# huangnengCSU/longcallR

Measured on AMD Instinct MI355X. Metric: candidate_sites_per_sec, higher is better.
Workload: dtype u8 in, u32 counts, f64 likelihoods, i64 fixed-point phase scores

## Files before the change

### include/lcr.h

```cpp
#ifndef LCR_H
#define LCR_H
#include <stddef.h>
#include <stdint.h>
#ifdef __cplusplus
extern "C" {
#endif

#define LCR_OK 0
#define LCR_E_ARG (-1)
#define LCR_E_CIGAR (-2)
#define LCR_E_DEVICE (-3)
#define LCR_E_STATE (-4)
#define LCR_E_NOMEM (-5)
#define LCR_W_HW_QUEUES 1

#define LCR_PLATFORM_HIFI 0
#define LCR_PLATFORM_ONT 1

#define LCR_MEM_HOST 0
#define LCR_MEM_DEVICE 1

typedef struct lcr_ctx lcr_ctx;


// ... 253 lines not shown
  uint32_t n_reads, n_h1, n_h2;
  uint32_t phase_set, n_phase_sets;
  uint32_t h1_absent, h1_present, h2_absent, h2_present;
} lcr_isoform;
typedef struct { int32_t n_regions, n_isoforms, n_chain, n_rows;
                 const lcr_isoform* iso; const int32_t* iso_region_off; const uint64_t* chain ; const int32_t* row_isoform;
                 const lcr_isoform* dev_iso; const uint64_t* dev_chain; const int32_t* dev_row_isoform; } lcr_isoform_list;
int lcr_isoforms(lcr_ctx*, const lcr_isoform_params*);
int lcr_get_isoforms(lcr_ctx*, lcr_isoform_list* out);
int lcr_isoforms_ms(lcr_ctx*, float* ms);

enum { LCR_ENDS_STRAND_TS = 0, LCR_ENDS_STRAND_READ = 1 };
typedef struct { uint32_t min_count, window, strand_mode, pad_; } lcr_end_params;
typedef struct {
  int32_t region; uint8_t strand, side, kind, pad_;
  int64_t peak0;
  int32_t min0, max0;
  uint32_t n_reads, n_h1, n_h2, n_peak;
  uint32_t phase_set, n_phase_sets;
  uint32_t h1_absent, h1_present, h2_absent, h2_present;
} lcr_end_site;
typedef struct { int32_t n_regions, n_sites, n_rows, n_part; int64_t n_assigned;
                 const lcr_end_site* site; const int32_t* site_region_off; const int32_t* row_site;
                 const lcr_end_site* dev_site; const int32_t* dev_row_site; } lcr_end_list;
int lcr_transcript_ends(lcr_ctx*, const lcr_end_params*);
int lcr_get_transcript_ends(lcr_ctx*, lcr_end_list* out);
int lcr_transcript_ends_ms(lcr_ctx*, float* ms);

typedef struct { int32_t n_genes, n_exons; const int64_t *span_start0, *span_end0; const int32_t* exon_off;
                 const int64_t *exon_start0, *exon_end0; } lcr_gene_annotation;
int lcr_assign_genes(lcr_ctx*, int32_t mem, const lcr_gene_annotation*);
int lcr_get_read_genes(lcr_ctx*, int32_t* n_reads, const int32_t** gene, const uint32_t** overlap, const int32_t** dev_gene);

typedef struct {
  int32_t region;
  uint32_t phase_set, n_phase_sets;
  uint32_t h1, h2;
  uint32_t n_sites;
  uint32_t h1_pat, h1_mat, h2_pat, h2_mat;
  int32_t gene;
  uint32_t pad_;
} lcr_ase_gene;
typedef struct { int32_t n_regions, n_pairs; const lcr_ase_gene* rec; const int32_t* pair_region_off; const lcr_ase_gene* dev_rec; } lcr_ase_gene_list;
int lcr_ase_genes(lcr_ctx*, const lcr_ase_params*, int32_t mem, int32_t n_sites, const int64_t* pos0, const uint8_t* pat, const uint8_t* mat);
int lcr_get_ase_genes(lcr_ctx*, lcr_ase_gene_list* out);

typedef struct {
  int32_t region; uint8_t motif; uint8_t pad_[3];
  int64_t start0;
  int32_t len; uint32_t n_reads;
  uint32_t phase_set, n_phase_sets;
  uint32_t h1_absent, h1_present, h2_absent, h2_present;
  int32_t gene;
  uint32_t pad2_;
} lcr_junction_gene;
typedef struct { int32_t n_regions, n_junctions; const lcr_junction_gene* junc; const int32_t* junc_region_off;
                 const lcr_junction_gene* dev_junc; float kernel_ms; } lcr_junction_gene_list;
int lcr_junctions_genes(lcr_ctx*, const lcr_junction_params*, int32_t mem, const lcr_gene_annotation*);
int lcr_get_junctions_genes(lcr_ctx*, lcr_junction_gene_list* out);

enum { LCR_ASJ_EXONS = 1, LCR_ASJ_DNA_FILTER = 2, LCR_ASJ_COVERAGE = 4 };
typedef struct { uint32_t min_count, min_junctions, flags; float min_phase_score;
                 int32_t n_dna, pad_; const int64_t* dna_pos0; } lcr_asj_params;
typedef struct { int32_t region, gene; int64_t start0; int32_t len; uint32_t n_reads; } lcr_exon_gene;
typedef struct { int32_t n_regions, n_junctions; const lcr_junction_gene* junc; const int32_t* junc_region_off;
                 const lcr_junction_gene* dev_junc;
                 int32_t n_exons, n_genes; const lcr_exon_gene* exon; const int32_t* exon_region_off; const lcr_exon_gene* dev_exon;
                 const int32_t* gene_reads; float kernel_ms; } lcr_asj_gene_list;
int lcr_asj_genes(lcr_ctx*, const lcr_asj_params*, int32_t mem, const lcr_gene_annotation*);
int lcr_get_asj_genes(lcr_ctx*, lcr_asj_gene_list* out);

typedef struct {
  int32_t n_regions, n_rows;
  const uint8_t* region_applied;
  const uint8_t* sampled;
  const uint8_t* dev_sampled;
} lcr_downsample_info;
int lcr_set_downsample(lcr_ctx*, uint32_t depth, uint64_t seed);
int lcr_set_downsample_rows(lcr_ctx*, int32_t mem, int32_t n_rows, const uint8_t* sampled);
int lcr_get_downsample(lcr_ctx*, lcr_downsample_info* out);

int lcr_get_ld_blocks(lcr_ctx*, int32_t region, int32_t* n_blocks, const int32_t** block_off, const int32_t** snp_idx);

int lcr_get_tie_census(lcr_ctx*, uint64_t out[8]);

typedef struct {
  int32_t n_regions;
  const int64_t* start0;
  const int32_t* len;
  const uint32_t* max_cov;
} lcr_region_list;
int lcr_discover_regions(lcr_ctx*, int32_t mem, int32_t n_reads, const int32_t* ref_start, const int32_t* ref_end,
                         int64_t contig_len, lcr_region_list* out);
int lcr_discover_regions_truncated(lcr_ctx*, int32_t mem, int32_t n_reads, const int32_t* ref_start, const int32_t* ref_end,
                                   int64_t contig_len, int32_t truncation, uint32_t truncation_coverage, lcr_region_list* out,
                                   int64_t* n_truncated);

typedef struct lcr_bam lcr_bam;
typedef struct {
  uint8_t min_mapq;
  int32_t min_read_length;
  float divergence;
} lcr_read_filter;
int lcr_bam_open(const char* path, int32_t n_threads, lcr_bam** out);
int lcr_bam_open_keep(const char* path, int32_t n_threads, int64_t keep_bytes, lcr_bam** out);
void lcr_bam_close(lcr_bam*);
const char* lcr_bam_last_error(const lcr_bam*);
int lcr_bam_refs(lcr_bam*, int32_t* n_ref, const char* const** names, const int64_t** lengths);
int lcr_bam_n_records(lcr_bam*, int64_t* n);
int lcr_bam_resident(lcr_bam*, int64_t* now, int64_t* peak);
int lcr_bam_spans(lcr_bam*, int32_t ref_id, const lcr_read_filter*, int32_t* n, const int32_t** ref_start,
                  const int32_t** ref_end);
int lcr_bam_batch(lcr_bam*, int32_t ref_id, const lcr_read_filter*, int32_t n_regions, const int64_t* start0,
                  const int32_t* len, lcr_reads* reads, const int32_t** read_begin, const uint64_t** name_off,
                  const char** names);
int lcr_bam_batch_packed(lcr_bam*, int32_t ref_id, const lcr_read_filter*, int32_t n_regions, const int64_t* start0,
                         const int32_t* len, lcr_reads_packed* reads, const int32_t** read_begin, const uint64_t** name_off,
                         const char** names);

typedef struct lcr_vcf lcr_vcf;
int lcr_vcf_open(const char* path, int32_t n_threads, lcr_vcf** out);
void lcr_vcf_close(lcr_vcf*);
const char* lcr_vcf_last_error(const lcr_vcf*);
int lcr_vcf_contigs(lcr_vcf*, int32_t* n, const char* const** names);
int lcr_vcf_contig(lcr_vcf*, const char* name, int32_t* n, const int64_t** pos0, const uint8_t** genotype, const float** qual);
int lcr_vcf_contig_alleles(lcr_vcf*, const char* name, int32_t* n, const uint8_t** ref, const uint8_t** alt, const uint8_t** phase);
int lcr_vcf_contig_phase_sets(lcr_vcf*, const char* name, int32_t* n, const uint32_t** ps);

int lcr_bam_write_phased(lcr_bam*, const char* out_path, int32_t n_regions, const int32_t* region_ref, const int64_t* start0,
                         const int32_t* len, int64_t n_tagged, const uint64_t* name_off, const char* names, const int32_t* hp,
                         const uint32_t* ps, int32_t level, int32_t n_threads);

int lcr_bam_write_reads(const char* out_path, const char* contig, int64_t contig_len, const lcr_reads* rd, int32_t level, int32_t n_threads);

int lcr_ctx_set_async_phase(lcr_ctx*, int on);

int lcr_ctx_set_lock_dir(lcr_ctx*, const char* dir);

int lcr_debug_set(lcr_ctx*, const char* key, int64_t value);

enum { LCR_K_SPANS = 0 , LCR_K_PILEUP, LCR_K_CAND_FILTER, LCR_K_CAND_HIST, LCR_K_CAND_GT,
       LCR_K_FRAG_COUNT, LCR_K_FRAG_FILL, LCR_K_PHASE,
       LCR_K_BIND ,
       LCR_K_BIND_TABLE ,
       LCR_K_CAND_IMPORT , LCR_K_JUNCTIONS ,
       LCR_K_ASE , LCR_NKERNELS };
enum { LCR_K_GENES = LCR_NKERNELS ,
       LCR_K_ASE_GENES ,
       LCR_NTIMERS };
int lcr_enable_timing(lcr_ctx*, int on);
int lcr_kernel_ms(lcr_ctx*, int kernel, float* ms);
int lcr_pileup_bytes(lcr_ctx*, int64_t* bytes);
int lcr_pileup_stage_bytes(lcr_ctx*, int64_t* bytes);

int lcr_release_cached_memory(void);
int lcr_set_cache_limits(int64_t device_bytes, int64_t host_bytes);

const char* lcr_version(void);

#ifdef __cplusplus
}
#endif
#endif
```

### longcallr_amd/_lib.py

```python
import ctypes as C
import os

from . import _abi

_HERE = os.path.dirname(os.path.abspath(__file__))
SO_PATH = os.environ.get("LCR_LIB") or os.path.join(_HERE, "liblcr.so")

SYMBOLS = [
    "lcr_params_preset", "lcr_ctx_create", "lcr_ctx_destroy", "lcr_last_error", "lcr_ctx_set_stream",
    "lcr_ctx_sync", "lcr_ctx_set_lock_dir", "lcr_ctx_set_async_phase", "lcr_debug_set", "lcr_load_batch", "lcr_load_batch_async", "lcr_bind_batch",
    "lcr_host_alloc", "lcr_host_free", "lcr_host_register", "lcr_host_unregister", "lcr_pileup", "lcr_get_columns", "lcr_candidates",
    "lcr_get_candidates", "lcr_get_candidates_device", "lcr_fragments", "lcr_get_fragmat", "lcr_phase", "lcr_get_phase_result", "lcr_get_read_records_device", "lcr_collect_phase", "lcr_get_ld_blocks", "lcr_get_tie_census",
    "lcr_enable_timing", "lcr_kernel_ms", "lcr_pileup_bytes", "lcr_pileup_stage_bytes", "lcr_discover_regions", "lcr_discover_regions_truncated", "lcr_version", "lcr_release_cached_memory", "lcr_set_cache_limits",
    "lcr_bam_open", "lcr_bam_open_keep", "lcr_bam_close", "lcr_bam_last_error", "lcr_bam_refs", "lcr_bam_n_records", "lcr_bam_resident", "lcr_bam_spans", "lcr_bam_batch", "lcr_bam_write_phased", "lcr_bam_write_reads",
    "lcr_set_downsample", "lcr_set_downsample_rows", "lcr_get_downsample",
    "lcr_junctions", "lcr_get_junctions", "lcr_ase", "lcr_get_ase", "lcr_vcf_contig_alleles",
    "lcr_assign_genes", "lcr_get_read_genes", "lcr_ase_genes", "lcr_get_ase_genes",
    "lcr_junctions_genes", "lcr_get_junctions_genes", "lcr_asj_genes", "lcr_get_asj_genes",
    "lcr_load_batch_packed", "lcr_load_batch_packed_async", "lcr_unpack_bases", "lcr_unpack_ms", "lcr_bam_batch_packed",
    "lcr_set_exon_mask", "lcr_exon_mask_ms", "lcr_import_candidates", "lcr_vcf_open", "lcr_vcf_close", "lcr_vcf_last_error", "lcr_vcf_contigs", "lcr_vcf_contig",
    "lcr_haplotag", "lcr_get_haplotag_sites", "lcr_haplotag_ms", "lcr_vcf_contig_phase_sets",
    "lcr_site_counts", "lcr_get_site_counts", "lcr_site_counts_ms",
    "lcr_hap_coverage", "lcr_get_hap_coverage", "lcr_hap_coverage_ms",
    "lcr_somatic", "lcr_get_somatic", "lcr_somatic_ms",
    "lcr_isoforms", "lcr_get_isoforms", "lcr_isoforms_ms",
    "lcr_transcript_ends", "lcr_get_transcript_ends", "lcr_transcript_ends_ms",
]

_lib = None


class LcrError(RuntimeError):
    pass


def load():
    global _lib
    if _lib is not None:
        return _lib
    if not os.path.exists(SO_PATH):
        raise LcrError("liblcr.so is missing: build it with `python -m longcallr_amd.build` "
                       "(hipcc --offload-arch=gfx950). There is no CPU fallback.")
    try:
        import torch
    except Exception:
        pass
    l = C.CDLL(SO_PATH)
    vp, i32 = C.c_void_p, C.c_int
    l.lcr_version.restype = C.c_char_p
    l.lcr_last_error.restype = C.c_char_p
    l.lcr_last_error.argtypes = [vp]
    l.lcr_params_preset.argtypes = [i32, C.POINTER(_abi.LcrParams)]
    l.lcr_ctx_create.argtypes = [i32, C.POINTER(vp)]
    l.lcr_ctx_destroy.argtypes = [vp]
    l.lcr_ctx_destroy.restype = None
    l.lcr_ctx_set_stream.argtypes = [vp, vp]
    l.lcr_ctx_sync.argtypes = [vp]
    l.lcr_ctx_set_lock_dir.argtypes = [vp, C.c_char_p]
    l.lcr_ctx_set_async_phase.argtypes = [vp, C.c_int32]
    l.lcr_debug_set.argtypes = [vp, C.c_char_p, C.c_int64]
    l.lcr_load_batch.argtypes = [vp, C.POINTER(_abi.LcrReads), C.POINTER(_abi.LcrRegions)]
    l.lcr_load_batch_async.argtypes = [vp, C.POINTER(_abi.LcrReads), C.POINTER(_abi.LcrRegions), C.c_int32]
    l.lcr_bind_batch.argtypes = [vp, C.c_int32]
    l.lcr_load_batch_packed.argtypes = [vp, C.POINTER(_abi.LcrReadsPacked), C.POINTER(_abi.LcrRegions)]
    l.lcr_load_batch_packed_async.argtypes = [vp, C.POINTER(_abi.LcrReadsPacked), C.POINTER(_abi.LcrRegions), C.c_int32]
    l.lcr_unpack_bases.argtypes = [vp, C.c_int32, vp, vp, vp, vp, C.c_int64, vp, C.c_int64]
    l.lcr_unpack_ms.argtypes = [vp, C.POINTER(C.c_float)]
    l.lcr_host_alloc.argtypes = [C.c_size_t, C.POINTER(C.c_void_p)]
    l.lcr_host_free.argtypes = [vp]
    l.lcr_host_free.restype = None
    l.lcr_host_register.argtypes = [vp, C.c_size_t]
    l.lcr_host_unregister.argtypes = [vp]
    for f in ("lcr_pileup", "lcr_candidates", "lcr_fragments", "lcr_phase"):
        getattr(l, f).argtypes = [vp, C.POINTER(_abi.LcrParams)]
    l.lcr_get_columns.argtypes = [vp, C.POINTER(_abi.LcrColumns)]
    l.lcr_get_candidates.argtypes = [vp, C.POINTER(_abi.LcrCandidateList)]
    l.lcr_get_candidates_device.argtypes = [vp, C.POINTER(vp), C.POINTER(i32)]
    l.lcr_get_read_records_device.argtypes = [vp, C.POINTER(vp), C.POINTER(i32)]
    l.lcr_get_fragmat.argtypes = [vp, C.POINTER(_abi.LcrFragmat)]
    l.lcr_get_phase_result.argtypes = [vp, C.POINTER(_abi.LcrPhaseResult)]
    l.lcr_collect_phase.argtypes = [vp, C.POINTER(_abi.LcrPhaseCollected)]
    l.lcr_release_cached_memory.argtypes = []
    l.lcr_set_cache_limits.argtypes = [C.c_int64, C.c_int64]
    l.lcr_get_tie_census.argtypes = [vp, C.POINTER(C.c_uint64)]
    l.lcr_get_ld_blocks.argtypes = [vp, C.c_int32, C.POINTER(C.c_int32), C.POINTER(C.POINTER(C.c_int32)), C.POINTER(C.POINTER(C.c_int32))]
    l.lcr_discover_regions.argtypes = [vp, C.c_int32, C.c_int32, vp, vp, C.c_int64, C.POINTER(_abi.LcrRegionList)]
    l.lcr_discover_regions_truncated.argtypes = [vp, C.c_int32, C.c_int32, vp, vp, C.c_int64, C.c_int32, C.c_uint32, C.POINTER(_abi.LcrRegionList),
                                                 C.POINTER(C.c_int64)]
    l.lcr_enable_timing.argtypes = [vp, i32]
    l.lcr_kernel_ms.argtypes = [vp, i32, C.POINTER(C.c_float)]
    l.lcr_pileup_bytes.argtypes = [vp, C.POINTER(C.c_int64)]
    l.lcr_pileup_stage_bytes.argtypes = [vp, C.POINTER(C.c_int64)]
    flt = C.POINTER(_abi.LcrReadFilter)
    l.lcr_bam_open.argtypes = [C.c_char_p, C.c_int32, C.POINTER(vp)]
    l.lcr_bam_open_keep.argtypes = [C.c_char_p, C.c_int32, C.c_int64, C.POINTER(vp)]
    l.lcr_bam_close.argtypes = [vp]
    l.lcr_bam_close.restype = None
    l.lcr_bam_last_error.argtypes = [vp]
    l.lcr_bam_last_error.restype = C.c_char_p
    l.lcr_bam_refs.argtypes = [vp, C.POINTER(C.c_int32), C.POINTER(C.POINTER(C.c_char_p)), C.POINTER(C.POINTER(C.c_int64))]
    l.lcr_bam_n_records.argtypes = [vp, C.POINTER(C.c_int64)]
    l.lcr_bam_resident.argtypes = [vp, C.POINTER(C.c_int64), C.POINTER(C.c_int64)]
    l.lcr_bam_spans.argtypes = [vp, C.c_int32, flt, C.POINTER(C.c_int32), C.POINTER(C.POINTER(C.c_int32)), C.POINTER(C.POINTER(C.c_int32))]
    l.lcr_bam_batch.argtypes = [vp, C.c_int32, flt, C.c_int32, vp, vp, C.POINTER(_abi.LcrReads), C.POINTER(C.POINTER(C.c_int32)),
                                C.POINTER(C.POINTER(C.c_uint64)), C.POINTER(C.c_char_p)]
    l.lcr_bam_batch_packed.argtypes = [vp, C.c_int32, flt, C.c_int32, vp, vp, C.POINTER(_abi.LcrReadsPacked), C.POINTER(C.POINTER(C.c_int32)),
                                       C.POINTER(C.POINTER(C.c_uint64)), C.POINTER(C.c_char_p)]
    l.lcr_bam_write_phased.argtypes = [vp, C.c_char_p, C.c_int32, vp, vp, vp, C.c_int64, vp, C.c_char_p, vp, vp, C.c_int32, C.c_int32]
    l.lcr_bam_write_reads.argtypes = [C.c_char_p, C.c_char_p, C.c_int64, C.POINTER(_abi.LcrReads), C.c_int32, C.c_int32]
    l.lcr_import_candidates.argtypes = [vp, C.POINTER(_abi.LcrParams), C.c_int32, C.c_int32, vp, vp, vp]
    l.lcr_set_exon_mask.argtypes = [vp, C.c_int32, vp, vp, vp]
    l.lcr_exon_mask_ms.argtypes = [vp, C.POINTER(C.c_float)]
    l.lcr_set_downsample.argtypes = [vp, C.c_uint32, C.c_uint64]
    l.lcr_set_downsample_rows.argtypes = [vp, C.c_int32, C.c_int32, vp]
    l.lcr_get_downsample.argtypes = [vp, C.POINTER(_abi.LcrDownsampleInfo)]
    l.lcr_junctions.argtypes = [vp, C.POINTER(_abi.LcrJunctionParams)]
    l.lcr_get_junctions.argtypes = [vp, C.POINTER(_abi.LcrJunctionList)]
    l.lcr_vcf_open.argtypes = [C.c_char_p, C.c_int32, C.POINTER(vp)]
    l.lcr_vcf_close.argtypes = [vp]
    l.lcr_vcf_close.restype = None
    l.lcr_vcf_last_error.argtypes = [vp]
    l.lcr_vcf_last_error.restype = C.c_char_p
    l.lcr_vcf_contigs.argtypes = [vp, C.POINTER(C.c_int32), C.POINTER(C.POINTER(C.c_char_p))]
    l.lcr_vcf_contig.argtypes = [vp, C.c_char_p, C.POINTER(C.c_int32), C.POINTER(vp), C.POINTER(vp), C.POINTER(vp)]
    l.lcr_ase.argtypes = [vp, C.POINTER(_abi.LcrAseParams), C.c_int32, C.c_int32, vp, vp, vp]
    l.lcr_get_ase.argtypes = [vp, C.POINTER(_abi.LcrAseList)]
    l.lcr_assign_genes.argtypes = [vp, C.c_int32, C.POINTER(_abi.LcrGeneAnnotation)]
    l.lcr_get_read_genes.argtypes = [vp, C.POINTER(C.c_int32), C.POINTER(vp), C.POINTER(vp), C.POINTER(vp)]
    l.lcr_ase_genes.argtypes = [vp, C.POINTER(_abi.LcrAseParams), C.c_int32, C.c_int32, vp, vp, vp]
    l.lcr_get_ase_genes.argtypes = [vp, C.POINTER(_abi.LcrAseGeneList)]
    l.lcr_junctions_genes.argtypes = [vp, C.POINTER(_abi.LcrJunctionParams), C.c_int32, C.POINTER(_abi.LcrGeneAnnotation)]
    l.lcr_get_junctions_genes.argtypes = [vp, C.POINTER(_abi.LcrJunctionGeneList)]
    l.lcr_asj_genes.argtypes = [vp, C.POINTER(_abi.LcrAsjParams), C.c_int32, C.POINTER(_abi.LcrGeneAnnotation)]
    l.lcr_get_asj_genes.argtypes = [vp, C.POINTER(_abi.LcrAsjGeneList)]
    l.lcr_vcf_contig_alleles.argtypes = [vp, C.c_char_p, C.POINTER(C.c_int32), C.POINTER(vp), C.POINTER(vp), C.POINTER(vp)]
    l.lcr_vcf_contig_phase_sets.argtypes = [vp, C.c_char_p, C.POINTER(C.c_int32), C.POINTER(vp)]
    l.lcr_haplotag.argtypes = [vp, C.POINTER(_abi.LcrParams), C.c_int32, C.c_int32, vp, vp, vp, vp]
    l.lcr_get_haplotag_sites.argtypes = [vp, C.POINTER(C.c_int32), C.POINTER(vp), C.POINTER(vp)]
    l.lcr_haplotag_ms.argtypes = [vp, C.POINTER(C.c_float)]
    l.lcr_site_counts.argtypes = [vp, C.POINTER(_abi.LcrSiteCountParams)]
    l.lcr_get_site_counts.argtypes = [vp, C.POINTER(C.c_int32), C.POINTER(vp), C.POINTER(vp)]
    l.lcr_site_counts_ms.argtypes = [vp, C.POINTER(C.c_float)]
    l.lcr_hap_coverage.argtypes = [vp]
    l.lcr_get_hap_coverage.argtypes = [vp, C.POINTER(_abi.LcrHapCovList)]
    l.lcr_hap_coverage_ms.argtypes = [vp, C.POINTER(C.c_float)]
    l.lcr_somatic.argtypes = [vp, C.POINTER(_abi.LcrSomaticParams)]
    l.lcr_get_somatic.argtypes = [vp, C.POINTER(C.c_int32), C.POINTER(vp), C.POINTER(vp)]
    l.lcr_somatic_ms.argtypes = [vp, C.POINTER(C.c_float)]
    l.lcr_isoforms.argtypes = [vp, C.POINTER(_abi.LcrIsoformParams)]
    l.lcr_get_isoforms.argtypes = [vp, C.POINTER(_abi.LcrIsoformList)]
    l.lcr_isoforms_ms.argtypes = [vp, C.POINTER(C.c_float)]
    l.lcr_transcript_ends.argtypes = [vp, C.POINTER(_abi.LcrEndParams)]
    l.lcr_get_transcript_ends.argtypes = [vp, C.POINTER(_abi.LcrEndList)]
    l.lcr_transcript_ends_ms.argtypes = [vp, C.POINTER(C.c_float)]
    _lib = l
    return l
```

### longcallr_amd/api.py

```python
import ctypes as C

import numpy as np

from . import _abi, _lib
from ._lib import LcrError


def _view(ptr, dtype, n):
    if n == 0 or not ptr:
        return np.zeros(0, dtype=dtype)
    buf = (C.c_char * (np.dtype(dtype).itemsize * n)).from_address(ptr)
    return np.frombuffer(buf, dtype=dtype, count=n).copy()


def _view_nocopy(ptr, dtype, n):
    if n == 0 or not ptr:
        return np.zeros(0, dtype=dtype)
    buf = (C.c_char * (np.dtype(dtype).itemsize * n)).from_address(ptr)
    return np.frombuffer(buf, dtype=dtype, count=n)


_DEBUG_ENV = {"LCR_PHASE_PROF": "phase_prof", "LCR_GRID_MIN_ENTRIES": "grid_min_entries",
              "LCR_GRID_GENERIC": "grid_generic", "LCR_GRID_SPEC_LANES": "grid_spec_lanes", "LCR_GRID_SPEC_BATCH": "grid_spec_batch", "LCR_POST_HALF": "post_half", "LCR_ENUM_FORCE_BIG": "enum_force_big",
              "LCR_ENUM_FORCE_STREAM": "enum_force_stream", "LCR_ENUM_ELIDE": "enum_elide", "LCR_HIST_TILES": "hist_tiles", "LCR_TIE_ARITH": "tie_arith", "LCR_CHAIN_TIES": "chain_ties", "LCR_K3_HITS": "k3_hits", "LCR_K3_LIST_BLOCKS": "k3_list_blocks", "LCR_FUSE_FILTER": "fuse_filter", "LCR_ASYNC_PHASE": "async_phase", "LCR_HOST_TRACE": "host_trace", "LCR_OWN_FILL": "own_fill", "LCR_REDO_LDS": "redo_lds", "LCR_SPEC_COMPACT": "spec_compact", "LCR_LEAN_PLANES": "lean_planes"}


class Engine:
    def __init__(self, device=0, params=None, timing=False):
        self.lib = _lib.load()
        h = C.c_void_p()
        rc = self.lib.lcr_ctx_create(device, C.byref(h))
        if rc != 0:
            raise LcrError("lcr_ctx_create(device=%d) failed with %d: no usable HIP device; "
                           "liblcr has no CPU fallback" % (device, rc))
        self.h = h
        self.device = device
        self.params = params if params is not None else _abi.make_params()
        self._sites = None
        self._keep = None
        self._n_regions = None
        self._mask_keep = None
        self.last_truncated_columns = 0
        if timing:
            self.lib.lcr_enable_timing(self.h, 1)
            if timing is not True:
                self.debug_set("timing_mask", sum(1 << int(k) for k in timing))
        import os
        for env, key in _DEBUG_ENV.items():
            v = os.environ.get(env)
            if v is not None:
                self.debug_set(key, int(v) if v.lstrip("-").isdigit() else 1)
        if os.environ.get("LCR_LOCK_DIR"):
            self._chk(self.lib.lcr_ctx_set_lock_dir(self.h, os.fsencode(os.environ["LCR_LOCK_DIR"])), "lcr_ctx_set_lock_dir")

    def debug_set(self, key, value):
        self._chk(self.lib.lcr_debug_set(self.h, key.encode(), int(value)), "lcr_debug_set")
        return self

    def close(self):
        if getattr(self, "h", None):
            self.lib.lcr_ctx_destroy(self.h)
            self.h = None

    __del__ = close

    def _chk(self, rc, what):
        if rc != 0:
            raise LcrError("%s failed (%d): %s" % (what, rc, self.lib.lcr_last_error(self.h).decode()))

    def set_stream(self, hip_stream_ptr):
        self._chk(self.lib.lcr_ctx_set_stream(self.h, C.c_void_p(hip_stream_ptr)), "lcr_ctx_set_stream")

    def sync(self):
        self._chk(self.lib.lcr_ctx_sync(self.h), "lcr_ctx_sync")
        self._sites = None
        self._mask_keep = None

    def set_async_phase(self, on=True):
        rc = self.lib.lcr_ctx_set_async_phase(self.h, 1 if on else 0)
        self.async_warning = self.lib.lcr_last_error(self.h).decode() if rc > 0 else None
        if rc < 0:
            self._chk(rc, "lcr_ctx_set_async_phase")
        return self

    def load_batch(self, batch):
        if isinstance(batch, (_abi.ReadBatch, _abi.PackedReadBatch)):
            reads, regions = batch.c_reads(), batch.c_regions()
            self._keep = (batch, reads, regions)
        else:
            reads, regions, keep = batch
            self._keep = (keep, reads, regions)
        if isinstance(reads, _abi.LcrReadsPacked):
            self._chk(self.lib.lcr_load_batch_packed(self.h, C.byref(reads), C.byref(regions)), "lcr_load_batch_packed")
        else:
            self._chk(self.lib.lcr_load_batch(self.h, C.byref(reads), C.byref(regions)), "lcr_load_batch")
        self._n_regions = int(regions.n_regions)
        return self

    def load_batch_async(self, batch, slot):
        reads, regions = batch.c_reads(), batch.c_regions()
        if not hasattr(self, "_keep_slot"):
            self._keep_slot = {}
        if isinstance(reads, _abi.LcrReadsPacked):
            self._chk(self.lib.lcr_load_batch_packed_async(self.h, C.byref(reads), C.byref(regions), int(slot)), "lcr_load_batch_packed_async")
        else:
            self._chk(self.lib.lcr_load_batch_async(self.h, C.byref(reads), C.byref(regions), int(slot)), "lcr_load_batch_async")
        self._keep_slot[int(slot)] = (batch, reads, regions)
        return self

    def unpack_bases(self, seq_len, seq_off, pack_off, seq4, bases_out):
        import torch
        want = (("seq_len", seq_len, (torch.int32,)), ("seq_off", seq_off, (torch.int64, torch.uint64)), ("pack_off", pack_off, (torch.int64, torch.uint64)),
                ("seq4", seq4, (torch.uint8,)), ("bases_out", bases_out, (torch.uint8,)))
        for name, t, dts in want:
            if not getattr(t, "is_cuda", False) or t.dtype not in dts or t.device.index != self.device or t.dim() != 1 or not t.is_contiguous():
                raise ValueError("unpack_bases: %s must be a contiguous 1-d %s tensor on device %d" % (name, dts[0], self.device))
        if not (seq_len.numel() == seq_off.numel() == pack_off.numel()):
            raise ValueError("seq_len, seq_off and pack_off must have the same length")
        torch.cuda.current_stream(self.device).synchronize()
        ptr = lambda t: C.c_void_p(t.data_ptr()) if t.numel() else None
        self._chk(self.lib.lcr_unpack_bases(self.h, int(seq_len.numel()), ptr(seq_len), ptr(seq_off), ptr(pack_off), ptr(seq4), int(seq4.numel()),
                                            ptr(bases_out), int(bases_out.numel())), "lcr_unpack_bases")
        return self

    def unpack_ms(self):
        ms = C.c_float()
        self._chk(self.lib.lcr_unpack_ms(self.h, C.byref(ms)), "lcr_unpack_ms")
        return float(ms.value)

    def bind_batch(self, slot):
        self._chk(self.lib.lcr_bind_batch(self.h, int(slot)), "lcr_bind_batch")
        self._n_regions = int(self._keep_slot[int(slot)][2].n_regions)
        return self

    def discover_regions(self, ref_start, ref_end, contig_len, truncation=False, truncation_coverage=200000):
        if not 0 <= int(truncation_coverage) < 1 << 32:
            raise ValueError("truncation_coverage must be in [0, 2^32), got %r" % (truncation_coverage,))
        rs = np.ascontiguousarray(ref_start, dtype=np.int32)
        re_ = np.ascontiguousarray(ref_end, dtype=np.int32)
        o = _abi.LcrRegionList()
        nt = C.c_int64(0)
        self._chk(self.lib.lcr_discover_regions_truncated(self.h, _abi.LCR_MEM_HOST, int(rs.size), rs.ctypes.data, re_.ctypes.data,
                                                          int(contig_len), 1 if truncation else 0, int(truncation_coverage), C.byref(o),
                                                          C.byref(nt)), "lcr_discover_regions_truncated")
        self.last_truncated_columns = int(nt.value)
        return list(zip(_view(o.start0, np.int64, o.n_regions).tolist(), _view(o.len, np.int32, o.n_regions).tolist(),
                        _view(o.max_cov, np.uint32, o.n_regions).tolist()))

    def fill_data_into_freq_vec(self):
        self._chk(self.lib.lcr_pileup(self.h, C.byref(self.params)), "lcr_pileup")
        return self

    def get_candidate_snps(self):
        self._chk(self.lib.lcr_candidates(self.h, C.byref(self.params)), "lcr_candidates")
        return self

    def import_external_candidates(self, pos0, genotype, qual):
        if any(getattr(t, "is_cuda", False) for t in (pos0, genotype, qual)):
            import torch
            ts = (pos0, genotype, qual)
            want = (torch.int64, torch.uint8, torch.float32)
            if not all(getattr(t, "is_cuda", False) for t in ts):
                raise ValueError("device sites: pos0, genotype and qual must all be device tensors")
            for name, t, dt in zip(("pos0", "genotype", "qual"), ts, want):
                if t.dtype != dt:
                    raise ValueError("device sites: %s must be %s, got %s" % (name, dt, t.dtype))
                if t.device.index != self.device:
                    raise ValueError("device sites: %s is on %s, the engine on device %d" % (name, t.device, self.device))
                if t.dim() != 1 or not t.is_contiguous():
                    raise ValueError("device sites: %s must be a contiguous 1-d tensor" % name)
            if len({t.numel() for t in ts}) != 1:
                raise ValueError("pos0, genotype and qual must have the same length")
            self._release_sites()
            torch.cuda.current_stream(self.device).synchronize()
            self._chk(self.lib.lcr_import_candidates(self.h, C.byref(self.params), _abi.LCR_MEM_DEVICE, int(pos0.numel()),
                                                     *[C.c_void_p(t.data_ptr()) for t in ts]), "lcr_import_candidates")
            self._sites = ts
# ... 217 lines not shown
            pat = np.ascontiguousarray(sites[1], dtype=np.uint8)
            mat = np.ascontiguousarray(sites[2], dtype=np.uint8)
            if not (pos.size == pat.size == mat.size):
                raise ValueError("pos0, pat and mat must have the same length")
            rc = fn(self.h, C.byref(p), _abi.LCR_MEM_HOST, int(pos.size), pos.ctypes.data, pat.ctypes.data, mat.ctypes.data)
        self._chk(rc, what)

    def assign_genes(self, genes):
        a, keep = self._annotation(genes)
        self._chk(self.lib.lcr_assign_genes(self.h, _abi.LCR_MEM_HOST, C.byref(a)), "lcr_assign_genes")
        return self

    @staticmethod
    def _annotation(genes):
        a = _abi.LcrGeneAnnotation()
        keep = []
        if genes is not None and len(genes.span_start0):
            for f, dt in (("span_start0", np.int64), ("span_end0", np.int64), ("exon_off", np.int32), ("exon_start0", np.int64), ("exon_end0", np.int64)):
                keep.append(np.ascontiguousarray(getattr(genes, f), dtype=dt))
                setattr(a, f, keep[-1].ctypes.data)
            a.n_genes, a.n_exons = int(keep[0].size), int(keep[3].size)
            if keep[1].size != a.n_genes or keep[2].size != a.n_genes + 1 or keep[4].size != a.n_exons:
                raise ValueError("annotation arrays: span_end0 needs n_genes, exon_off n_genes + 1, exon_end0 n_exons entries")
        return a, keep

    def read_genes(self):
        n, g, ov, dg = C.c_int32(), C.c_void_p(), C.c_void_p(), C.c_void_p()
        self._chk(self.lib.lcr_get_read_genes(self.h, C.byref(n), C.byref(g), C.byref(ov), C.byref(dg)), "lcr_get_read_genes")
        return _view(g.value, np.int32, n.value), _view(ov.value, np.uint32, n.value)

    def ase_genes(self, sites=None, min_baseq=13, min_phase_score=None):
        self._ase_call(self.lib.lcr_ase_genes, "lcr_ase_genes", sites, min_baseq, min_phase_score)
        o = _abi.LcrAseGeneList()
        self._chk(self.lib.lcr_get_ase_genes(self.h, C.byref(o)), "lcr_get_ase_genes")
        return _view(o.rec, _abi.AGENE_DTYPE, o.n_pairs), _view(o.pair_region_off, np.int32, o.n_regions + 1)

    def junctions_genes(self, genes, min_count=10, min_junctions=2):
        p = _abi.LcrJunctionParams(int(min_count), int(min_junctions))
        a, keep = self._annotation(genes)
        self._chk(self.lib.lcr_junctions_genes(self.h, C.byref(p), _abi.LCR_MEM_HOST, C.byref(a)), "lcr_junctions_genes")
        o = _abi.LcrJunctionGeneList()
        self._chk(self.lib.lcr_get_junctions_genes(self.h, C.byref(o)), "lcr_get_junctions_genes")
        self.last_junctions_genes_ms = float(o.kernel_ms)
        return _view(o.junc, _abi.JUNC_GENE_DTYPE, o.n_junctions), _view(o.junc_region_off, np.int32, o.n_regions + 1)

    def asj_genes(self, genes, min_count=10, min_junctions=2, exons=False, dna_pos0=None, coverage=False, min_phase_score=None):
        flags = (_abi.LCR_ASJ_EXONS if exons else 0) | (_abi.LCR_ASJ_DNA_FILTER if dna_pos0 is not None else 0) | (_abi.LCR_ASJ_COVERAGE if coverage else 0)
        p = _abi.LcrAsjParams(int(min_count), int(min_junctions), flags, float(self.params.min_phase_score if min_phase_score is None else min_phase_score))
        dna = None
        if dna_pos0 is not None:
            dna = np.ascontiguousarray(dna_pos0, dtype=np.int64)
            p.n_dna, p.dna_pos0 = int(dna.size), (dna.ctypes.data if dna.size else None)
        a, keep = self._annotation(genes)
        self._chk(self.lib.lcr_asj_genes(self.h, C.byref(p), _abi.LCR_MEM_HOST, C.byref(a)), "lcr_asj_genes")
        o = _abi.LcrAsjGeneList()
        self._chk(self.lib.lcr_get_asj_genes(self.h, C.byref(o)), "lcr_get_asj_genes")
        return {"junc": _view(o.junc, _abi.JUNC_GENE_DTYPE, o.n_junctions), "junc_region_off": _view(o.junc_region_off, np.int32, o.n_regions + 1),
                "exon": _view(o.exon, _abi.EXON_GENE_DTYPE, o.n_exons), "exon_region_off": _view(o.exon_region_off, np.int32, o.n_regions + 1),
                "gene_reads": _view(o.gene_reads, np.int32, o.n_genes) if o.gene_reads else None, "kernel_ms": float(o.kernel_ms)}

    def set_downsample(self, depth, seed=2025):
        self._chk(self.lib.lcr_set_downsample(self.h, int(depth), int(seed)), "lcr_set_downsample")
        return self

    def set_downsample_rows(self, sampled):
        m = np.ascontiguousarray(sampled, dtype=np.uint8)
        self._chk(self.lib.lcr_set_downsample_rows(self.h, _abi.LCR_MEM_HOST, int(m.size), m.ctypes.data), "lcr_set_downsample_rows")
        return self

    def downsample_info(self):
        o = _abi.LcrDownsampleInfo()
        self._chk(self.lib.lcr_get_downsample(self.h, C.byref(o)), "lcr_get_downsample")
        return dict(applied=_view(o.region_applied, np.uint8, o.n_regions),
                    sampled=_view(o.sampled, np.uint8, o.n_rows) if o.sampled else None, dev_sampled=int(o.dev_sampled or 0))

    def run_all(self):
        return self.fill_data_into_freq_vec().get_candidate_snps().get_fragments().phase()

    def columns(self):
        o = _abi.LcrColumns()
        self._chk(self.lib.lcr_get_columns(self.h, C.byref(o)), "lcr_get_columns")
        return _view(o.planes, np.uint32, _abi.NPLANES * o.n_cols).reshape(_abi.NPLANES, o.n_cols)

    def candidates(self):
        o = _abi.LcrCandidateList()
        self._chk(self.lib.lcr_get_candidates(self.h, C.byref(o)), "lcr_get_candidates")
        self._sites = None
        return (_view(o.cand, _abi.CAND_DTYPE, o.n_cand), _view(o.region_off, np.int32, o.n_regions + 1))

    def candidates_device(self):
        ptr, n = C.c_void_p(), C.c_int32()
        self._chk(self.lib.lcr_get_candidates_device(self.h, C.byref(ptr), C.byref(n)), "lcr_get_candidates_device")
        return int(ptr.value or 0), int(n.value)

    def read_records_device(self):
        ptr, n = C.c_void_p(), C.c_int32()
        self._chk(self.lib.lcr_get_read_records_device(self.h, C.byref(ptr), C.byref(n)), "lcr_get_read_records_device")
        return int(ptr.value or 0), int(n.value)

    def fragmat(self):
        o = _abi.LcrFragmat()
        self._chk(self.lib.lcr_get_fragmat(self.h, C.byref(o)), "lcr_get_fragmat")
        return dict(
            row_region_off=_view(o.row_region_off, np.int32, o.n_regions + 1),
            row_ptr=_view(o.row_ptr, np.int64, o.n_rows + 1), row_read=_view(o.row_read, np.int32, o.n_rows),
            col=_view(o.col, np.int32, o.nnz), val=_view(o.val, np.uint8, o.nnz),
            row_for_phasing=_view(o.row_for_phasing, np.uint8, o.n_rows),
            row_links=_view(o.row_links, np.uint32, o.n_rows))

    def phase_result(self):
        o = _abi.LcrPhaseResult()
        self._chk(self.lib.lcr_get_phase_result(self.h, C.byref(o)), "lcr_get_phase_result")
        return dict(haplotag=_view(o.haplotag, np.int8, o.n_rows), assignment=_view(o.assignment, np.uint8, o.n_rows),
                    phase_set=_view(o.phase_set, np.uint32, o.n_rows),
                    objective=_view(o.objective, np.float64, o.n_regions))

    def collect_phase(self, copy=False):
        o = _abi.LcrPhaseCollected()
        self._chk(self.lib.lcr_collect_phase(self.h, C.byref(o)), "lcr_collect_phase")
        v = _view if copy else _view_nocopy
        return dict(cand=v(o.cand, _abi.CAND_DTYPE, o.n_cand), cand_region_off=v(o.cand_region_off, np.int32, o.n_regions + 1),
                    row_region_off=v(o.row_region_off, np.int32, o.n_regions + 1),
                    haplotag=v(o.haplotag, np.int8, o.n_rows), assignment=v(o.assignment, np.uint8, o.n_rows),
                    phase_set=v(o.phase_set, np.uint32, o.n_rows), objective=v(o.objective, np.float64, o.n_regions),
                    dev_cand=(int(o.dev_cand or 0), int(o.n_cand)), dev_read_rec=(int(o.dev_read_rec or 0), int(o.n_rows)))

    def ld_blocks(self, region):
        n, off, idx = C.c_int32(), C.POINTER(C.c_int32)(), C.POINTER(C.c_int32)()
        self._chk(self.lib.lcr_get_ld_blocks(self.h, int(region), C.byref(n), C.byref(off), C.byref(idx)), "lcr_get_ld_blocks")
        return [[idx[k] for k in range(off[b], off[b + 1])] for b in range(n.value)]

    TIE_FIELDS = ("sigma_f64", "sigma_flips", "delta_unresolved", "step_unresolved", "best_f64", "best_unresolved", "sigma_unresolved", "delta_step_f64")

    def tie_census(self):
        out = (C.c_uint64 * 8)()
        self._chk(self.lib.lcr_get_tie_census(self.h, out), "lcr_get_tie_census")
        return dict(zip(self.TIE_FIELDS, [int(x) for x in out]))

    def kernel_ms(self, k):
        ms = C.c_float()
        self._chk(self.lib.lcr_kernel_ms(self.h, k, C.byref(ms)), "lcr_kernel_ms")
        return float(ms.value)

    def pileup_bytes(self):
        b = C.c_int64()
        self._chk(self.lib.lcr_pileup_bytes(self.h, C.byref(b)), "lcr_pileup_bytes")
        return int(b.value)

    def pileup_stage_bytes(self):
        b = C.c_int64()
        self._chk(self.lib.lcr_pileup_stage_bytes(self.h, C.byref(b)), "lcr_pileup_stage_bytes")
        return int(b.value)


def host_register(*arrays):
    lib = _lib.load()
    done = []
    for a in arrays:
        if a is None or a.nbytes == 0:
            continue
        if lib.lcr_host_register(C.c_void_p(a.ctypes.data), a.nbytes) != 0:
            host_unregister(done)
            raise LcrError("lcr_host_register failed")
        done.append(a)
    return done


def host_unregister(arrays):
    lib = _lib.load()
    for a in arrays:
        lib.lcr_host_unregister(C.c_void_p(a.ctypes.data))
```

### longcallr_amd/csrc/k0_ops.hip

```cpp
#include <algorithm>
#include <climits>

#include "lcr_dev.h"

#ifndef K0_THREADS
#define K0_THREADS 256
#endif
#ifndef K0_OPT
#define K0_OPT 4
#endif
#ifndef K0_ABL
#define K0_ABL 0
#endif
#define K0_NW (K0_THREADS / 64)
#define K0_WIN K0_THREADS
#define K0_ACC 64
#ifndef K0_HCAP
#define K0_HCAP 160
#endif


__device__ __forceinline__ int wave_incl_max(int v) {
  v = max(v, __builtin_amdgcn_update_dpp(0, v, 0x111, 0xf, 0xf, false));
  v = max(v, __builtin_amdgcn_update_dpp(0, v, 0x112, 0xf, 0xf, false));
  v = max(v, __builtin_amdgcn_update_dpp(0, v, 0x114, 0xf, 0xf, false));
  v = max(v, __builtin_amdgcn_update_dpp(0, v, 0x118, 0xf, 0xf, false));
  v = max(v, __builtin_amdgcn_update_dpp(0, v, 0x142, 0xa, 0xf, false));
  v = max(v, __builtin_amdgcn_update_dpp(0, v, 0x143, 0xc, 0xf, false));
  return v;
}


__global__ void __launch_bounds__(LCR_BLOCK) k0_cig_check(const uint64_t* __restrict__ cig_off, const uint32_t* __restrict__ n_cig,
                                                           int32_t nr, int64_t n_cigar, int32_t* out) {
  const int r = blockIdx.x * blockDim.x + threadIdx.x;
  if (r + 1 < nr && cig_off[r + 1] != cig_off[r] + n_cig[r]) out[1] = 1;
  if (r < nr && (cig_off[r] > (uint64_t)n_cigar || (uint64_t)n_cig[r] > (uint64_t)n_cigar - cig_off[r])) out[2] = 1;
  if (r == 0) {
    uint64_t* g = reinterpret_cast<uint64_t*>(out + 4);
    g[0] = cig_off[0]; g[1] = cig_off[nr - 1] + n_cig[nr - 1];
  }
}
void launch_k0_cig_check(const uint64_t* cig_off, const uint32_t* n_cig, int32_t nr, int64_t n_cigar, int32_t* out, hipStream_t s) {
  if (nr > 0) hipLaunchKernelGGL(k0_cig_check, dim3((nr + LCR_BLOCK - 1) / LCR_BLOCK), dim3(LCR_BLOCK), 0, s, cig_off, n_cig, nr, n_cigar, out);
}
__global__ void __launch_bounds__(LCR_BLOCK) k0_cig_compact(const uint32_t* __restrict__ cigar, const uint64_t* __restrict__ cig_off,
                                                             const uint32_t* __restrict__ n_cig, const int32_t* __restrict__ new_off,
                                                             int32_t nr, uint32_t* __restrict__ out, uint64_t* __restrict__ out_off) {
  const int r = (int)((blockIdx.x * blockDim.x + threadIdx.x) >> 6), lane = threadIdx.x & 63;
  if (r >= nr) return;
  const uint32_t* src = cigar + cig_off[r];
  uint32_t* dst = out + new_off[r];
  for (uint32_t i = lane; i < n_cig[r]; i += 64) dst[i] = src[i];
  if (lane == 0) out_off[r] = (uint64_t)new_off[r];
}
void launch_k0_cig_compact(const uint32_t* cigar, const uint64_t* cig_off, const uint32_t* n_cig, const int32_t* new_off, int32_t nr,
                           uint32_t* out, uint64_t* out_off, hipStream_t s) {
  if (nr > 0) hipLaunchKernelGGL(k0_cig_compact, dim3((unsigned)(((int64_t)nr * 64 + LCR_BLOCK - 1) / LCR_BLOCK)), dim3(LCR_BLOCK), 0, s,
                                 cigar, cig_off, n_cig, new_off, nr, out, out_off);
}

__global__ void __launch_bounds__(LCR_BLOCK) k0_block_reads(const ReadBin* __restrict__ rbin, int32_t nr, uint64_t cig0, int32_t opb,
                                                             int32_t n_blocks, int32_t* __restrict__ blk_first_read) {
  const int r = blockIdx.x * blockDim.x + threadIdx.x;
  if (r >= nr) return;
  if (r == 0) blk_first_read[n_blocks] = nr - 1;
  const uint64_t cb = rbin[r].cig_off - cig0, ce = cb + (uint32_t)rbin[r].n_cig;
  for (uint64_t k = (cb + opb - 1) / opb; k * opb < ce; k++) blk_first_read[k] = r;
}
void launch_k0_block_reads(const ReadBin* rbin, int32_t nr, uint64_t cig0, int32_t opb, int32_t n_blocks, int32_t* blk_first_read, hipStream_t s) {
  if (nr > 0) hipLaunchKernelGGL(k0_block_reads, dim3((nr + LCR_BLOCK - 1) / LCR_BLOCK), dim3(LCR_BLOCK), 0, s, rbin, nr, cig0, opb, n_blocks, blk_first_read);
}

struct K0Hdr {
  int32_t refbase;
  int32_t qbase;
  int32_t qlo, qhi;
  int32_t vec, ftile;
  int32_t cend;
  uint32_t hi;
  uint64_t seq_off;
  int32_t reb, rel_pos;
};

__device__ __forceinline__ void wave_lds_sync() {
  __builtin_amdgcn_fence(__ATOMIC_RELEASE, "wavefront");
  __builtin_amdgcn_wave_barrier();
  __builtin_amdgcn_fence(__ATOMIC_ACQUIRE, "wavefront");
}

template <int OPT>
__global__ void __launch_bounds__(K0_THREADS)
k0_ops(BatchView b, const ReadBin* __restrict__ rbin, const int32_t* __restrict__ blk_first_read, uint64_t cig0, uint32_t n_ops,
       int ont, int D, int32_t n_tiles, int32_t* __restrict__ tile_fill, int32_t* __restrict__ tile_nchunks, int32_t* __restrict__ tile_ndiff,
       K0Ctl* __restrict__ ctl, unsigned int* __restrict__ acct, unsigned int pool_sub, unsigned long long* __restrict__ recs,
       unsigned int desc_sub, uint32_t* __restrict__ desc_tile, uint2* __restrict__ desc_val, int2* __restrict__ read_scan) {
  constexpr int OPB = OPT * K0_THREADS, WOPS = OPT * 64;
  __shared__ __attribute__((aligned(8))) uint16_t ridh[OPB];
  __shared__ K0Hdr hdr[K0_HCAP];
  __shared__ int ws_ref[K0_NW], ws_q[K0_NW], ws_rid[K0_NW];
  __shared__ int cnt[K0_WIN], cur[K0_WIN];
  __shared__ unsigned int s_base[3];
  __shared__ int runbase[OPB];
  __shared__ int s_carry[2], s_acc[2];

  const int tid = threadIdx.x, lane = tid & 63, wv = tid >> 6;
  const uint32_t j0 = blockIdx.x * (uint32_t)OPB;
  if (j0 >= n_ops) return;
  const uint32_t jend = min(j0 + (uint32_t)OPB, n_ops);
  const bool last_block = jend == n_ops;
  const uint32_t* __restrict__ cg = b.cigar + cig0;

  uint32_t w[OPT];
  {
    const uint32_t j = j0 + OPT * tid;
    if (OPT == 4 && j + 4 <= jend) {
      const uint4 v = *reinterpret_cast<const uint4*>(cg + j);
      w[0] = v.x; w[1] = v.y; w[2] = v.z; w[3] = v.w;
    } else {
#pragma unroll
      for (int k = 0; k < OPT; k++) w[k] = j + k < jend ? cg[j + k] : 0x4u;
    }
  }
  const int r_lo = blk_first_read[blockIdx.x];
  const int n_blk_reads = blk_first_read[blockIdx.x + 1] - r_lo + 1;
#pragma unroll
  for (int k = 0; k < OPT; k++) ridh[k * K0_THREADS + tid] = 0;
  cnt[tid] = 0;
  if (tid == 0) { s_acc[0] = 0; s_acc[1] = 0; }
  __syncthreads();

  auto load_hdr = [&](int r, uint64_t* cb_out, int* ncig_out) {
    const ReadBin h = rbin[r];
    K0Hdr x;
    x.refbase = h.rel_pos; x.qbase = h.lead > 0 ? h.lead : 0;
    x.qlo = ont ? h.lead + D : -(1 << 30); x.qhi = ont ? h.reb - D + 1 : (1 << 30);
    x.vec = h.vec; x.ftile = h.ftile; x.seq_off = h.seq_off; x.reb = h.reb; x.rel_pos = h.rel_pos;
    const int strand = h.flags & 1, ts = (h.flags >> 1) & 3;
    const uint32_t tscls = ts == 0 ? 0u : ((strand == 0) == (ts == 1) ? 1u : 2u);
    x.hi = ((uint32_t)strand << 28) | (tscls << 29);
    const uint64_t cb = h.cig_off - cig0;
    x.cend = (int32_t)min<int64_t>((int64_t)cb + h.n_cig - (int64_t)j0, INT_MAX);
    *cb_out = cb; *ncig_out = h.n_cig;
    return x;
  };
  auto settle_empty = [&](int r, const K0Hdr& x) {
    b.read_rend[r] = x.rel_pos;
    if (x.qbase != x.reb) atomicExch(&ctl->error, 2);
  };
  for (int rr = tid; rr < n_blk_reads; rr += K0_THREADS) {
    uint64_t cb; int ncig;
    const K0Hdr x = load_hdr(r_lo + rr, &cb, &ncig);
    if (rr == 0 || cb < (uint64_t)jend || (cb == (uint64_t)jend && (last_block || ncig == 0))) {
      if (rr < K0_HCAP) hdr[rr] = x;
      if (rr > 0) { if (ncig > 0) ridh[cb - j0] = (uint16_t)rr; else settle_empty(r_lo + rr, x); }
    }
  }
  if (blockIdx.x == 0)
    for (int r = tid; r < r_lo; r += K0_THREADS) { uint64_t cb; int ncig; const K0Hdr x = load_hdr(r, &cb, &ncig); settle_empty(r, x); }
  if (wv == 0) {
    const uint64_t cb0 = rbin[r_lo].cig_off - cig0;
    int cr = 0, cq = 0;
    for (uint64_t j = cb0 + lane; j < (uint64_t)j0; j += 64) {
      const uint32_t x = cg[j];
      const int op = x & 15, len = (int)(x >> 4);
      const bool m = op == 0 || op == 7 || op == 8;
      cr += (m || op == 2 || op == 3) ? len : 0;
      cq += (m || op == 1) ? len : 0;
    }
    cr = wave_incl_scan(cr); cq = wave_incl_scan(cq);
    if (lane == 63) { s_carry[0] = cr; s_carry[1] = cq; }
  }
  __syncthreads();

  if (K0_ABL == 1) return;
  int dr[OPT], dq[OPT], xr[OPT], xq[OPT], rid[OPT], mark[OPT];
  {
    bool bad_op = false;
    int tr = 0, tq = 0, tm = 0;
    const uint2 mk = *reinterpret_cast<const uint2*>(&ridh[OPT * tid]);
#pragma unroll
    for (int k = 0; k < OPT; k++) {
      const int op = w[k] & 15, len = (int)(w[k] >> 4);
      const bool m = op == 0 || op == 7 || op == 8;
      if (!(m || (op >= 1 && op <= 5))) bad_op = true;
      dr[k] = (m || op == 2 || op == 3) ? len : 0;
      dq[k] = (m || op == 1) ? len : 0;
      mark[k] = OPT == 4 ? (int)(((k < 2 ? mk.x : mk.y) >> (16 * (k & 1))) & 0xffffu) : (int)ridh[OPT * tid + k];
      xr[k] = tr; xq[k] = tq;
      tr += dr[k]; tq += dq[k];
      tm = max(tm, mark[k]); rid[k] = tm;
    }
    if (bad_op) atomicExch(&ctl->error, 1);
    const int ir = wave_incl_scan(tr), iq = wave_incl_scan(tq), im = wave_incl_max(tm);
    if (lane == 63) { ws_ref[wv] = ir; ws_q[wv] = iq; ws_rid[wv] = im; }
    __syncthreads();
    int br = ir - tr, bq = iq - tq, bm = __shfl_up(im, 1, 64);
    if (lane == 0) bm = 0;
    for (int i = 0; i < wv; i++) { br += ws_ref[i]; bq += ws_q[i]; bm = max(bm, ws_rid[i]); }
#pragma unroll
    for (int k = 0; k < OPT; k++) {
      xr[k] += br; xq[k] += bq; rid[k] = max(rid[k], bm);
      if (mark[k] != 0) {
        if (mark[k] < K0_HCAP) { hdr[mark[k]].refbase -= xr[k]; hdr[mark[k]].qbase -= xq[k]; }
        else read_scan[r_lo + mark[k]] = make_int2(xr[k], xq[k]);
      }
    }
    if (tid == 0) { hdr[0].refbase += s_carry[0]; hdr[0].qbase += s_carry[1]; }
  }
  __syncthreads();

  if (K0_ABL == 2) { if (xr[0] + xq[1] + rid[2] == 0x7fffffff) ctl->error = 9; return; }
  int a[OPT], e[OPT], tb[OPT], kind[OPT];
  unsigned int rlo[OPT], rhi[OPT];
  unsigned int my_items = 0;
  const int win0 = hdr[0].ftile + (int)((unsigned int)max(hdr[0].rel_pos - 1, 0) / (unsigned int)LCR_TILE);
#pragma unroll
  for (int k = 0; k < OPT; k++) {
    const int p = OPT * tid + k;
    const bool act = j0 + p < jend;
    K0Hdr H;
    if (rid[k] < K0_HCAP) H = hdr[rid[k]];
    else {
      uint64_t cb; int ncig;
      H = load_hdr(r_lo + rid[k], &cb, &ncig);
      const int2 sb = read_scan[r_lo + rid[k]];
      H.refbase -= sb.x; H.qbase -= sb.y;
    }
    const int op = w[k] & 15, len = (int)(w[k] >> 4);
    const int rs = H.refbase + xr[k];
    const int qs = H.qbase + xq[k];
    const bool m = act && (op == 0 || op == 7 || op == 8), d = act && op == 2, ins = act && op == 1, isn = act && op == 3;
    int aa = max(rs, 0), ee = min(rs + len, H.vec);
    if (m) { aa = max(aa, rs + (H.qlo - qs)); ee = min(ee, rs + (H.qhi - qs)); }
    int kd = ((m || d || isn) && len > 0 && ee > aa) ? (m ? 1 : d ? 2 : 4) : 0;
    if (ins && len > 0 && rs >= 1 && rs < H.vec) { kd = 3; aa = rs - 1; ee = rs; }
    kind[k] = kd; a[k] = aa; e[k] = ee; tb[k] = H.ftile;
    if (kd == 1) {
      const unsigned long long o0 = H.seq_off + (unsigned long long)(long long)(qs - rs);
      rlo[k] = (unsigned int)o0; rhi[k] = ((unsigned int)(o0 >> 32) & 0xffu) | H.hi;
    } else {
      rlo[k] = kd == 2 ? (unsigned int)REC_KIND_D : kd == 3 ? (unsigned int)REC_KIND_I : (unsigned int)REC_KIND_N;
      rhi[k] = 0xffu;
    }
    if (kd) my_items++;
    if (act && p == H.cend - 1) {
      b.read_rend[r_lo + rid[k]] = rs + dr[k];
      if (qs + dq[k] != H.reb) atomicExch(&ctl->error, 2);
    }
    if (kd == 4) {
      const int ta = H.ftile + (int)((unsigned int)aa / (unsigned int)LCR_TILE), te = H.ftile + (int)((unsigned int)(ee - 1) / (unsigned int)LCR_TILE);
      if (te > ta + 1) { atomicAdd(&tile_ndiff[ta + 1], 1); atomicAdd(&tile_ndiff[te], -1); }
    }
  }

  if (K0_ABL == 3) { int x = 0; for (int k = 0; k < OPT; k++) x += a[k] + e[k] + tb[k] + kind[k] + (int)rlo[k] + (int)rhi[k]; if (x == 0x7fffffff) ctl->error = 9; return; }
  auto make_rec = [&](int k, int t) -> unsigned long long {
    const int c0 = (t - tb[k]) * LCR_TILE;
    const int c_lo = max(a[k], c0), c_hi = min(e[k], c0 + LCR_TILE);
    unsigned int lo = rlo[k], hi = rhi[k] | ((unsigned int)(c_lo - c0) << 8) | ((unsigned int)(c_hi - c_lo - 1) << 18);
    if (kind[k] == 1) {
      const unsigned int s = lo + (unsigned int)c_lo;
      hi = (hi & ~0xffu) | (((hi & 0xffu) + (s < lo ? 1u : 0u)) & 0xffu);
      lo = s;
    }
    return ((unsigned long long)hi << 32) | lo;
  };
  auto first_tile = [&](int k) { return tb[k] + (int)((unsigned int)a[k] / (unsigned int)LCR_TILE); };
  auto last_tile = [&](int k) { return tb[k] + (int)((unsigned int)(e[k] - 1) / (unsigned int)LCR_TILE); };
  auto next_tile = [&](int k, int t, int te) { return kind[k] == 4 ? te : t + 1; };

  int key[OPT], rank[OPT], hpos[OPT];
  bool is_last[OPT];
  {
#pragma unroll
    for (int k = 0; k < OPT; k++) {
      const int tp = kind[k] ? first_tile(k) - win0 : -1;
      key[k] = (tp >= 0 && tp < K0_WIN) ? tp : -1;
    }
    int pk = __shfl_up(key[OPT - 1], 1, 64);
    if (lane == 0) pk = -2;
    bool head[OPT];
    int hp = 0;
#pragma unroll
    for (int k = 0; k < OPT; k++) {
      head[k] = key[k] != (k == 0 ? pk : key[k - 1]);
      if (head[k]) hp = OPT * lane + k + 1;
      hpos[k] = hp;
    }
    const int ih = wave_incl_max(hp);
    int bh = __shfl_up(ih, 1, 64);
    if (lane == 0) bh = 0;
    const int nh = __shfl_down(head[0] ? 1 : 0, 1, 64);
#pragma unroll
    for (int k = 0; k < OPT; k++) {
      hpos[k] = max(hpos[k], bh) - 1;
      rank[k] = OPT * lane + k - hpos[k];
      is_last[k] = k + 1 < OPT ? head[k + 1] : (lane == 63 || nh != 0);
      if (is_last[k] && key[k] >= 0) atomicAdd(&cnt[key[k]], rank[k] + 1);
      if (kind[k]) {
        const int te = last_tile(k);
        for (int t = first_tile(k); t < te;) {
          t = next_tile(k, t, te);
          const int wi = t - win0;
          if (wi >= 0 && wi < K0_WIN) atomicAdd(&cnt[wi], 1);
        }
      }
    }
  }
  __syncthreads();

  if (K0_ABL == 4) { int x = 0; for (int k = 0; k < OPT; k++) x += rank[k] + hpos[k] + (is_last[k] ? 1 : 0); if (x == 0x7fffffff) ctl->error = 9; return; }
  unsigned int my_recs = 0;
  const unsigned int shard = blockIdx.x % K0_ACC;
  {
    static_assert(K0_WIN == K0_THREADS, "one window counter per thread");
    const int c = cnt[tid];
    const int c16 = (c + 15) & ~15;
    const int ic = wave_incl_scan(c16);
    const unsigned long long nzb = __ballot(c > 0);
    if (lane == 63) ws_ref[wv] = ic;
    if (lane == 0) ws_q[wv] = __popcll(nzb);
    __syncthreads();
    int before = 0, dbefore = 0, total = 0, dtotal = 0;
    for (int i = 0; i < K0_NW; i++) { if (i < wv) { before += ws_ref[i]; dbefore += ws_q[i]; } total += ws_ref[i]; dtotal += ws_q[i]; }
    if (tid == 0 && total > 0) {
      unsigned int* sh = acct + 32 * shard;
      const unsigned int at = atomicAdd(&sh[2], (unsigned int)total);
      const unsigned int dt = atomicAdd(&sh[3], (unsigned int)dtotal);
      const bool fits = at + (unsigned int)total <= pool_sub && dt + (unsigned int)dtotal <= desc_sub;
      if (!fits) atomicExch(&ctl->error, 3);
      s_base[0] = shard * pool_sub + at; s_base[1] = shard * desc_sub + dt; s_base[2] = fits ? 1u : 0u;
    }
    cur[tid] = before + ic - c16;
    my_recs += (unsigned int)c;
    __syncthreads();
    if (c > 0 && s_base[2]) {
      const int tile = win0 + tid;
      const unsigned int di = s_base[1] + (unsigned int)dbefore + (unsigned int)__popcll(nzb & ((1ull << lane) - 1ull));
      desc_tile[di] = (uint32_t)tile; desc_val[di] = make_uint2(s_base[0] + (unsigned int)(before + ic - c16), (unsigned int)c);
      atomicAdd(&tile_fill[tile], c);
      atomicAdd(&tile_nchunks[tile], c16 >> 4);
    }
  }
  const unsigned int blk_at = s_base[0];
  const bool blk_fits = s_base[2] != 0;

  auto put = [&](int slot, unsigned long long rec) { if (blk_fits) recs[blk_at + (unsigned int)slot] = rec; };
  int* rbw = runbase + wv * WOPS;
#pragma unroll
  for (int k = 0; k < OPT; k++)
    if (is_last[k] && key[k] >= 0) rbw[hpos[k]] = atomicAdd(&cur[key[k]], rank[k] + 1);
  wave_lds_sync();
  bool overflow = false;
#pragma unroll
  for (int k = 0; k < OPT; k++) {
    if (key[k] >= 0) put(rbw[hpos[k]] + rank[k], make_rec(k, first_tile(k)));
    else if (kind[k]) overflow = true;
    if (kind[k]) {
      const int te = last_tile(k);
      for (int t = first_tile(k); t < te;) {
        t = next_tile(k, t, te);
        const int wi = t - win0;
        if (wi >= 0 && wi < K0_WIN) put(atomicAdd(&cur[wi], 1), make_rec(k, t));
        else overflow = true;
      }
    }
  }
  if (overflow) {
#pragma unroll
    for (int k = 0; k < OPT; k++) {
      if (!kind[k]) continue;
      const int te = last_tile(k);
      for (int t = first_tile(k);; t = next_tile(k, t, te)) {
        if (t - win0 < 0 || t - win0 >= K0_WIN) {
          unsigned int* sh = acct + 32 * shard;
          const unsigned int at = atomicAdd(&sh[2], 1u), di = atomicAdd(&sh[3], 1u);
          if (at >= pool_sub || di >= desc_sub) atomicExch(&ctl->error, 3);
          else {
            recs[shard * pool_sub + at] = make_rec(k, t);
            desc_tile[shard * desc_sub + di] = (uint32_t)t; desc_val[shard * desc_sub + di] = make_uint2(shard * pool_sub + at, 1u);
            atomicAdd(&tile_fill[t], 1);
            atomicAdd(&tile_nchunks[t], 1);
          }
          my_recs++;
        }
        if (t >= te) break;
      }
    }
  }
  my_items = (unsigned int)wave_incl_scan((int)my_items);
  my_recs = (unsigned int)wave_incl_scan((int)my_recs);
  if (lane == 63) { atomicAdd(&s_acc[0], (int)my_items); atomicAdd(&s_acc[1], (int)my_recs); }
  __syncthreads();
  if (tid == 0) {
    unsigned int* acc = acct + 32 * shard;
    if (s_acc[0]) atomicAdd(&acc[0], (unsigned int)s_acc[0]);
    if (s_acc[1]) atomicAdd(&acc[1], (unsigned int)s_acc[1]);
  }
}

__global__ void __launch_bounds__(LCR_BLOCK) k0_empty_reads(BatchView b, const ReadBin* __restrict__ rbin, K0Ctl* __restrict__ ctl) {
  const int r = blockIdx.x * blockDim.x + threadIdx.x;
  if (r >= b.n_reads) return;
  b.read_rend[r] = rbin[r].rel_pos;
  if ((rbin[r].lead > 0 ? rbin[r].lead : 0) != rbin[r].reb) atomicExch(&ctl->error, 2);
}

int launch_k0_opb() { return K0_OPT * K0_THREADS; }
int launch_k0_acct_words() { return 32 * K0_ACC; }
int launch_k0_acct_slots() { return K0_ACC; }

__global__ void __launch_bounds__(LCR_BLOCK) k0_desc_bin(const K0Ctl* __restrict__ ctl, const unsigned int* __restrict__ acct, unsigned int desc_sub,
                                                          const uint32_t* __restrict__ desc_tile, const uint2* __restrict__ desc_val,
                                                          const int32_t* __restrict__ chunk_off, int32_t* __restrict__ cursor, uint2* __restrict__ sorted) {
  if (ctl->error != 0) return;
  const unsigned int shard = blockIdx.x % K0_ACC, per = gridDim.x / K0_ACC;
  const unsigned int n = min(acct[32 * shard + 3], desc_sub);
  for (unsigned int i = (blockIdx.x / K0_ACC) * LCR_BLOCK + threadIdx.x; i < n; i += per * LCR_BLOCK) {
    const uint32_t t = desc_tile[shard * desc_sub + i];
    const uint2 d = desc_val[shard * desc_sub + i];
    const int ne = (int)((d.y + 15u) >> 4);
    uint2* dst = sorted + chunk_off[t] + atomicAdd(&cursor[t], ne);
    for (int e = 0; e < ne; e++) dst[e] = make_uint2(d.x + 16u * (unsigned int)e, min(16u, d.y - 16u * (unsigned int)e));
  }
}
void launch_k0_desc_bin(const K0Ctl* ctl, const unsigned int* acct, unsigned int desc_sub, const uint32_t* desc_tile, const void* desc_val,
                        const int32_t* chunk_off, int32_t* cursor, void* sorted, int32_t n_blocks_hint, hipStream_t s) {
  const int per = std::max(1, std::min((n_blocks_hint + K0_ACC - 1) / K0_ACC, 32));
  hipLaunchKernelGGL(k0_desc_bin, dim3(per * K0_ACC), dim3(LCR_BLOCK), 0, s, ctl, acct, desc_sub, desc_tile, (const uint2*)desc_val,
                     chunk_off, cursor, (uint2*)sorted);
}

void launch_k0_ops(const BatchView& b, const ReadBin* rb, const int32_t* blk_first_read, uint64_t cig0, uint32_t n_ops, int ont, int D,
                   int32_t n_tiles, int32_t* tile_fill, int32_t* tile_nchunks, int32_t* tile_ndiff, K0Ctl* ctl, unsigned int* acct,
                   unsigned int pool_sub, unsigned long long* recs, unsigned int desc_sub, uint32_t* desc_tile, void* desc_val, void* read_scan,
                   hipStream_t s) {
  if (b.n_reads == 0) return;
  if (n_ops == 0) { hipLaunchKernelGGL(k0_empty_reads, dim3((b.n_reads + LCR_BLOCK - 1) / LCR_BLOCK), dim3(LCR_BLOCK), 0, s, b, rb, ctl); return; }
  const int opb = launch_k0_opb();
  hipLaunchKernelGGL(k0_ops<K0_OPT>, dim3((n_ops + opb - 1) / opb), dim3(K0_THREADS), 0, s, b, rb, blk_first_read, cig0, n_ops, ont, D, n_tiles,
                     tile_fill, tile_nchunks, tile_ndiff, ctl, acct, pool_sub, recs, desc_sub, desc_tile, (uint2*)desc_val, (int2*)read_scan);
}
```

### longcallr_amd/csrc/k1_pileup.hip

```cpp
#include <algorithm>
#include <climits>

#include "lcr_dev.h"
#include "k2_eval.h"

#ifdef LCR_K1_ABLATE
#define K1_ABL LCR_K1_ABLATE
#else
#define K1_ABL 0
#endif
#ifndef K1_THREADS
#define K1_THREADS LCR_TILE
#endif
#define K1_WAVES (K1_THREADS / 64)
#define K1_CPT (LCR_TILE / K1_THREADS)
#define K1_RPB 2
#define K1_PMAP (8 * K1_THREADS)
#ifndef K1_NT_STORES
#define K1_NT_STORES 0
#endif
#ifndef K1_PIF
#define K1_PIF 4
#endif

// ... 105 lines not shown
    const int n = g < ng ? (max(len[g], 0) + LCR_TILE - 1) / LCR_TILE : 0;
    const int incl = wave_incl_scan(n);
    if (lane == 63) wsum[wave] = incl;
    __syncthreads();
    int before = base_s;
    for (int w = 0; w < wave; w++) before += wsum[w];
    if (g < ng) first_tile[g + 1] = before + incl;
    __syncthreads();
    if (tid == 1023) base_s = before + incl;
    __syncthreads();
  }
}
void launch_k0_bind_a(const int64_t* start0, const int32_t* len, const int64_t* col_off, const int32_t* read_begin, int32_t ng,
                      int32_t* first_tile, int64_t* h_start0, int32_t* h_len, int64_t* h_col_off, int32_t* h_read_begin,
                      const uint64_t* cig_off, const uint32_t* n_cig, int32_t nr, int64_t n_cigar, int32_t* out, hipStream_t s) {
  hipLaunchKernelGGL(k0_bind_a, dim3(1 + (nr + 1023) / 1024), dim3(1024), 0, s, start0, len, col_off, read_begin, ng, first_tile, h_start0, h_len,
                     h_col_off, h_read_begin, cig_off, n_cig, nr, n_cigar, out);
}

__device__ __forceinline__ int last_le(const int32_t* __restrict__ a, int n, int x) {
  int lo = 0, hi = n;
  while (hi - lo > 1) { const int mid = (lo + hi) >> 1; if (a[mid] <= x) lo = mid; else hi = mid; }
  return lo;
}
__global__ void __launch_bounds__(LCR_BLOCK) k0_bind_b(BatchView b, ReadBin* __restrict__ rbin, int32_t* order_flag, int32_t* __restrict__ read_region,
                                                        int32_t n_tiles, int32_t* __restrict__ tile_region, int32_t* __restrict__ tile_col0,
                                                        uint64_t cig0, int32_t opb, int32_t n_blocks, int32_t* __restrict__ blk_first_read) {
  const int i = blockIdx.x * LCR_BLOCK + threadIdx.x;
  if (i >= b.n_reads) {
    const int t = i - b.n_reads;
    if (t < n_tiles) { const int g = last_le(b.region_first_tile, b.n_regions, t); tile_region[t] = g; tile_col0[t] = (t - b.region_first_tile[g]) * LCR_TILE; }
    return;
  }
  const int r = i;
  const int g = last_le(b.read_begin, b.n_regions, r);
  read_region[r] = g;
  const int32_t pos = b.pos[r];
  if (r > b.read_begin[g] && pos < b.pos[r - 1]) *order_flag = 1;
  ReadBin h;
  h.rel_pos = (int32_t)((int64_t)pos - b.start0[g]);
  h.vec = b.len[g]; h.ftile = b.region_first_tile[g]; h.n_cig = (int32_t)b.n_cig[r];
  h.gbase = b.col_off[g] + g;
  h.seq_off = b.seq_off[r]; h.cig_off = b.cig_off[r];
  h.lead = b.lead[r]; h.reb = b.seq_len[r] - b.trail[r];
  h.flags = b.flags[r]; h.pad_ = 0; h.pad2_ = 0;
  rbin[r] = h;
  if (r == 0) blk_first_read[n_blocks] = b.n_reads - 1;
  const uint64_t cb = h.cig_off - cig0, ce = cb + (uint32_t)h.n_cig;
  for (uint64_t k = (cb + opb - 1) / opb; k * opb < ce; k++) blk_first_read[k] = r;
}
void launch_k0_bind_b(const BatchView& b, ReadBin* rbin, int32_t* order_flag, int32_t* read_region, int32_t n_tiles, int32_t* tile_region,
                      int32_t* tile_col0, uint64_t cig0, int32_t opb, int32_t n_blocks, int32_t* blk_first_read, hipStream_t s) {
  const int64_t n = (int64_t)b.n_reads + n_tiles;
  if (n == 0) return;
  hipLaunchKernelGGL(k0_bind_b, dim3((unsigned)((n + LCR_BLOCK - 1) / LCR_BLOCK)), dim3(LCR_BLOCK), 0, s, b, rbin, order_flag, read_region, n_tiles,
                     tile_region, tile_col0, cig0, opb, n_blocks, blk_first_read);
}

enum {
  P_DIFF_DEPTH_F = 0,
  P_DIFF_DEPTH_R,
  P_DIFF_TS0,
  P_DIFF_TS1,
  P_DIFF_D,
  P_DIFF_N,
  P_NI,
  P_MM_F,
  P_MM_R = P_MM_F + 4,
  P_NPL = P_MM_R + 4
};
#define TSTRIDE (LCR_TILE + 1)
#define REF_PAD 16

__device__ __forceinline__ int block_incl_scan(int v, int* wsum ) {
  const int lane = threadIdx.x & 63, w = threadIdx.x >> 6;
  int s = wave_incl_scan(v);
  if (lane == 63) wsum[w] = s;
  __syncthreads();
  int add = 0;
  for (int i = 0; i < w; i++) add += wsum[i];
  return s + add;
}

struct K1Stage { Survivor* sv; int2* key; int32_t cap; int32_t* n_staged; };
template <bool LEAN>
__global__ void __launch_bounds__(K1_THREADS)
k1_pileup(BatchView b, DevParams prm, const int32_t* __restrict__ tile_region, const int32_t* __restrict__ tile_col0,
          int64_t n_cols, const int32_t* __restrict__ tile_fill, const int32_t* __restrict__ ent_off, const uint2* __restrict__ ents,
          const unsigned long long* __restrict__ recs,
          const int32_t* __restrict__ tile_nbase, uint32_t* __restrict__ planes, const int32_t* __restrict__ order,
          const int32_t* __restrict__ n_full, BinomTable bt, uint8_t* __restrict__ flt_flags, int32_t* __restrict__ flt_count, K1Stage stg) {
  if ((int)blockIdx.x >= *n_full) return;
  const int tile = order[blockIdx.x];
  __shared__ uint32_t pl[P_NPL * TSTRIDE];
  __shared__ __attribute__((aligned(16))) uint8_t refl[REF_PAD + LCR_TILE + 32];
  __shared__ unsigned long long rec_s[K1_RPB * K1_THREADS];
  __shared__ int pstart[K1_RPB * K1_THREADS + 1];
  __shared__ uint16_t pown[K1_PMAP];
  __shared__ int wsum[K1_WAVES];

  const int tid = threadIdx.x;
  const int g = tile_region[tile];
  const int tc0 = tile_col0[tile];
  const int vec = b.len[g];
  const int tlen = min(LCR_TILE, vec - tc0);
  const int64_t gcol0 = b.col_off[g] + tc0;
  if (*b.error_flag != 0) return;
  __shared__ uint32_t vge[17], vlt[17];
  if (tid >= 64 && tid < 64 + 34) {
    const int v = (tid - 64) % 17;
    uint32_t m = 0;
    for (int j = 0; j < 4; j++)
      for (int kk = 0; kk < 4; kk++)
        if (tid - 64 < 17 ? 4 * j + kk >= v : 4 * j + kk < v) m |= 1u << (8 * kk + j);
    if (tid - 64 < 17) vge[v] = m; else vlt[v] = m;
  }
  for (int i = tid; i < P_NPL * TSTRIDE; i += K1_THREADS) pl[i] = 0;
  for (int i = tid; i < REF_PAD + LCR_TILE + 32; i += K1_THREADS) {
    const int col = i - REF_PAD;
    uint8_t R = (col >= 0 && col < tlen) ? b.ref[gcol0 + col] : 0;
    refl[i] = (R == 'A' || R == 'C' || R == 'G' || R == 'T') ? R : 0xFF;
  }
  __syncthreads();
  const uint32_t* rl32 = reinterpret_cast<const uint32_t*>(refl);

  const int e0 = ent_off[tile];
  const int n_slots = (ent_off[tile + 1] - e0) * 16;
  static_assert(K1_RPB == 2, "a thread's two slots lie in one entry");
  auto load_recs = [&](int j, unsigned long long* out) -> int {
    out[0] = 0ull; out[1] = 0ull;
    int has = 0;
    if (j < n_slots) {
      const uint2 en = ents[e0 + (j >> 4)];
      const unsigned int k = (unsigned int)j & 15u;
      if (k < en.y) { out[0] = recs[en.x + k]; has |= 1; }
      if (k + 1 < en.y) { out[1] = recs[en.x + k + 1]; has |= 2; }
    }
    return has;
  };
  unsigned long long rec_nx[K1_RPB];
  int has_nx = load_recs(tid * K1_RPB, rec_nx);
  for (int rbase = 0; rbase < n_slots && K1_ABL != 3; rbase += K1_RPB * K1_THREADS) {
    unsigned long long rec_cur[K1_RPB];
#pragma unroll
    for (int x = 0; x < K1_RPB; x++) rec_cur[x] = rec_nx[x];
    const int has_cur = has_nx;
    has_nx = load_recs(rbase + K1_RPB * K1_THREADS + tid * K1_RPB, rec_nx);
    int npc[K1_RPB], nsum = 0;
#pragma unroll
    for (int x = 0; x < K1_RPB; x++) {
      const int slot = tid * K1_RPB + x;
      const unsigned long long rec = rec_cur[x];
      const bool hasrec = (has_cur >> x) & 1;
      const unsigned long long off = rec & REC_OFF_MASK;
      const int col0 = (int)((rec >> 40) & 1023u), len = (int)((rec >> 50) & 1023u) + 1;
      int npieces = 0;
      if (hasrec) {
        if (off == REC_KIND_D) {
          atomicAdd(&pl[P_DIFF_D * TSTRIDE + col0], 1u);
          atomicAdd(&pl[P_DIFF_D * TSTRIDE + col0 + len], 0xFFFFFFFFu);
        } else if (off == REC_KIND_I) {
          atomicAdd(&pl[P_NI * TSTRIDE + col0], 1u);
        } else if (off == REC_KIND_N) {
          atomicAdd(&pl[P_DIFF_N * TSTRIDE + col0], 1u);
          atomicAdd(&pl[P_DIFF_N * TSTRIDE + col0 + len], 0xFFFFFFFFu);
        } else {
          const int strand = (int)((rec >> 60) & 1u), tscls = (int)((rec >> 61) & 3u);
          uint32_t* dp = pl + (strand ? P_DIFF_DEPTH_R : P_DIFF_DEPTH_F) * TSTRIDE;
          atomicAdd(&dp[col0], 1u);
          atomicAdd(&dp[col0 + len], 0xFFFFFFFFu);
          if (tscls) {
            uint32_t* tp = pl + (tscls == 2 ? P_DIFF_TS1 : P_DIFF_TS0) * TSTRIDE;
            atomicAdd(&tp[col0], 1u);
            atomicAdd(&tp[col0 + len], 0xFFFFFFFFu);
          }
          npieces = (len + 15) >> 4;
        }
      }
      rec_s[slot] = rec;
      npc[x] = K1_ABL == 1 ? 0 : npieces;
      nsum += npc[x];
    }
    int run = block_incl_scan(nsum, wsum) - nsum;
    int P = 0;
#pragma unroll
    for (int i = 0; i < K1_WAVES; i++) P += wsum[i];
    const int pstride = (P + K1_PMAP - 1) / K1_PMAP;
    if (tid == 0) pstart[0] = 0;
#pragma unroll
    for (int x = 0; x < K1_RPB; x++) {
      const int first = run;
      run += npc[x];
      pstart[tid * K1_RPB + x + 1] = run;
      if (pstride == 1) for (int q = first; q < run; q++) pown[q] = (uint16_t)(tid * K1_RPB + x);
      else if (pstride > 1) for (int k = (first + pstride - 1) / pstride; k * pstride < run; k++) pown[k] = (uint16_t)(tid * K1_RPB + x);
    }
    __syncthreads();
    struct Piece { uint4 v; int colA, k_lo, k_hi, strand; bool ok; };
    auto fetch = [&](int p) -> Piece {
      Piece q;
      q.ok = p < P;
      if (!q.ok) { q.v = make_uint4(0, 0, 0, 0); q.colA = 0; q.k_lo = q.k_hi = 0; q.strand = 0; return q; }
      int lo;
      if (pstride == 1) lo = pown[p];
      else { lo = pown[p / pstride]; while (pstart[lo + 1] <= p) lo++; }
      const unsigned long long rc = rec_s[lo];
      const uint32_t rhi = (uint32_t)(rc >> 32);
      const long long soff = (long long)(rc & REC_OFF_MASK);
      const int scol = (int)((rhi >> 8) & 1023u), slen = (int)((rhi >> 18) & 1023u) + 1;
      q.strand = (int)((rhi >> 28) & 1u);
      const int d16 = 16 * (p - pstart[lo]);
      const long long A = soff + d16;
      q.k_lo = 0; q.k_hi = min(16, slen - d16);
      q.colA = scol + d16;
      if (A + 16 <= b.n_bases) q.v = *reinterpret_cast<const uint4*>(b.bases + A);
      else {
        uint32_t t[4] = {0, 0, 0, 0};
        for (int x = 0; x < 16; x++)
          if (A + x < b.n_bases) t[x >> 2] |= (uint32_t)b.bases[A + x] << (8 * (x & 3));
        q.v = make_uint4(t[0], t[1], t[2], t[3]);
      }
      return q;
    };
    auto tally = [&](const Piece& q) {
      if (!q.ok) return;
      const int ci = q.colA + REF_PAD, di = ci >> 2;
      const uint32_t sh = (uint32_t)(ci & 3);
      const uint32_t r0 = rl32[di], r1 = rl32[di + 1], r2 = rl32[di + 2], r3 = rl32[di + 3], r4 = rl32[di + 4];
      const uint32_t x0 = q.v.x ^ __builtin_amdgcn_alignbyte(r1, r0, sh), x1 = q.v.y ^ __builtin_amdgcn_alignbyte(r2, r1, sh);
      const uint32_t x2 = q.v.z ^ __builtin_amdgcn_alignbyte(r3, r2, sh), x3 = q.v.w ^ __builtin_amdgcn_alignbyte(r4, r3, sh);
      auto nzf = [](uint32_t x) -> uint32_t { return (x | ((x & 0x7f7f7f7fu) + 0x7f7f7f7fu)) & 0x80808080u; };
      uint32_t mm = (nzf(x0) >> 7) | (nzf(x1) >> 6) | (nzf(x2) >> 5) | (nzf(x3) >> 4);
      mm &= vlt[q.k_hi];
      if (K1_ABL == 5) mm = 0;
      uint32_t* dp = pl + (q.strand ? P_DIFF_DEPTH_R : P_DIFF_DEPTH_F) * TSTRIDE + q.colA;
      uint32_t* mp = pl + (q.strand ? P_MM_R : P_MM_F) * TSTRIDE + q.colA;
      while (mm) {
        const uint32_t pb = (uint32_t)__builtin_ctz(mm), jd = pb & 3u, kb = pb >> 3;
        mm &= mm - 1;
        const uint32_t lo = (jd & 2u) ? q.v.z : q.v.x, hi = (jd & 2u) ? q.v.w : q.v.y;
        const uint32_t base = __builtin_amdgcn_perm(hi, lo, 0x0c0c0c00u | ((jd & 1u) << 2) | kb);
        const uint32_t dcol = 4u * jd + kb;
        const uint32_t h = (base >> 1) & 3u;
        const bool acgt = (base & 0xDFu) == __builtin_amdgcn_perm(0u, 0x47544341u , 0x0c0c0c00u | h);
        if (acgt) atomicAdd(mp + h * TSTRIDE + dcol, 1u);
        else { atomicAdd(dp + dcol, 0xFFFFFFFFu); atomicAdd(dp + dcol + 1, 1u); }
      }
    };
    for (int p = tid; p < P; p += K1_PIF * K1_THREADS) {
      Piece q[K1_PIF];
#pragma unroll
      for (int x = 0; x < K1_PIF; x++) q[x] = fetch(p + x * K1_THREADS);
#pragma unroll
      for (int x = 0; x < K1_PIF; x++) tally(q[x]);
    }
    __syncthreads();
  }
  __syncthreads();

  {
    constexpr int NP = P_DIFF_N - P_DIFF_DEPTH_F + 1;
    static_assert(NP == 6, "six difference arrays");
    __shared__ int wsum5[NP][K1_WAVES];
    const int lane = tid & 63, w = tid >> 6;
    int v[NP][K1_CPT], incl[NP];
#pragma unroll
    for (int p = 0; p < NP; p++) {
      const uint32_t* d = pl + (P_DIFF_DEPTH_F + p) * TSTRIDE;
      int run = 0;
#pragma unroll
      for (int x = 0; x < K1_CPT; x++) { run += (int)d[tid * K1_CPT + x]; v[p][x] = run; }
      incl[p] = wave_incl_scan(run);
      if (lane == 63) wsum5[p][w] = incl[p];
      incl[p] -= run;
    }
    __syncthreads();
#pragma unroll
    for (int p = 0; p < NP; p++) {
      int add = incl[p];
      for (int i = 0; i < w; i++) add += wsum5[p][i];
      uint32_t* d = pl + (P_DIFF_DEPTH_F + p) * TSTRIDE;
#pragma unroll
      for (int x = 0; x < K1_CPT; x++) d[tid * K1_CPT + x] = (uint32_t)(add + v[p][x]);
    }
    __syncthreads();
  }

  const uint32_t nbase = (uint32_t)tile_nbase[tile];
  static_assert(K1_CPT == 1, "the fused filter counts one column per thread");
  int n_pass = 0;
  Survivor sv;
  for (int col = tid; col < tlen; col += K1_THREADS) {
    const uint8_t R = refl[REF_PAD + col];
    const int ri = R == 'A' ? 0 : R == 'C' ? 1 : R == 'G' ? 2 : R == 'T' ? 3 : -1;
    uint32_t f[4], rv[4];
    uint32_t sf = 0, sr = 0;
#pragma unroll
    for (int k = 0; k < 4; k++) {
      const int hk = k < 2 ? k : 5 - k;
      f[k] = pl[(P_MM_F + hk) * TSTRIDE + col]; rv[k] = pl[(P_MM_R + hk) * TSTRIDE + col];
      sf += f[k]; sr += rv[k];
    }
    if (ri >= 0) {
      const uint32_t mf = pl[P_DIFF_DEPTH_F * TSTRIDE + col] - sf, mr = pl[P_DIFF_DEPTH_R * TSTRIDE + col] - sr;
#pragma unroll
      for (int k = 0; k < 4; k++) if (k == ri) { f[k] = mf; rv[k] = mr; }
    }
    const int64_t o = gcol0 + col;
    if (!LEAN) {
#pragma unroll
      for (int k = 0; k < 4; k++) {
        planes[(int64_t)(LCR_PL_A + k) * n_cols + o] = f[k] + rv[k];
        planes[(int64_t)(LCR_PL_FWD_A + k) * n_cols + o] = f[k];
      }
      planes[(int64_t)LCR_PL_N * n_cols + o] = nbase + pl[P_DIFF_N * TSTRIDE + col];
      planes[(int64_t)LCR_PL_D * n_cols + o] = pl[P_DIFF_D * TSTRIDE + col];
      planes[(int64_t)LCR_PL_NI * n_cols + o] = pl[P_NI * TSTRIDE + col];
      planes[(int64_t)LCR_PL_TS_FWD * n_cols + o] = pl[P_DIFF_TS0 * TSTRIDE + col];
      planes[(int64_t)LCR_PL_TS_REV * n_cols + o] = pl[P_DIFF_TS1 * TSTRIDE + col];
    }
    if (LEAN || flt_flags) {
      uint32_t cnt[4];
#pragma unroll
      for (int k = 0; k < 4; k++) cnt[k] = f[k] + rv[k];
      const ColEval ev = eval_counts(cnt, R, prm, bt, b.exon_mask, o, [&]() { return pl[P_DIFF_D * TSTRIDE + col]; }, [&]() { return nbase + pl[P_DIFF_N * TSTRIDE + col]; },
                                     [&](int k) { return f[k]; });
      if (!LEAN) flt_flags[o] = ev.pass ? 1 : 0;
      n_pass += ev.pass ? 1 : 0;
      if (LEAN && ev.pass) {
        sv.gcol = o; sv.region = g; sv.col = tc0 + col;
        sv.ref_base = ev.ref_base; sv.allele1 = ev.allele1; sv.allele2 = ev.allele2; sv.n_alt = ev.n_alt;
        sv.cnt1 = ev.cnt1; sv.cnt2 = ev.cnt2; sv.depth = ev.depth; sv.af1 = ev.af1; sv.af2 = ev.af2;
        sv.ts_fwd = pl[P_DIFF_TS0 * TSTRIDE + col]; sv.ts_rev = pl[P_DIFF_TS1 * TSTRIDE + col];
      }
    }
  }
  if (LEAN) {
    __shared__ int stage_base;
    const int lane = tid & 63, w = tid >> 6;
    const unsigned long long bal = __ballot(n_pass != 0);
    if (lane == 0) wsum[w] = __popcll(bal);
    __syncthreads();
    int before = 0, total = 0;
#pragma unroll
    for (int i = 0; i < K1_WAVES; i++) { before += i < w ? wsum[i] : 0; total += wsum[i]; }
    if (tid == 0) {
      flt_count[tile] = total;
      if (total > 0) stage_base = atomicAdd(stg.n_staged, total);
    }
    if (total > 0) {
      __syncthreads();
      const int rank = before + __popcll(bal & ((1ull << lane) - 1ull));
      const int slot = stage_base + rank;
      if (n_pass != 0 && slot >= 0 && slot < stg.cap) { stg.sv[slot] = sv; stg.key[slot] = make_int2(tile, rank); }
    }
  } else if (flt_flags) {
    const int total = __syncthreads_count(n_pass);
    if (tid == 0) flt_count[tile] = total;
  }
}

__global__ void __launch_bounds__(128) k1_empty_tiles(BatchView b, const int32_t* __restrict__ tile_region, const int32_t* __restrict__ tile_col0,
                                                       int64_t n_cols, const int32_t* __restrict__ tile_nbase, uint32_t* __restrict__ planes,
// ... 430 lines not shown
```

### longcallr_amd/csrc/k2_candidates.hip

```cpp
#include "lcr_dev.h"
#include "k2_eval.h"

#define SCAN_ITEMS 4
#define SCAN_TILE (LCR_BLOCK * SCAN_ITEMS)

__device__ __forceinline__ int wave_incl_scan_i(int v, int lane) {
#pragma unroll
  for (int d = 1; d < 64; d <<= 1) {
    int t = __shfl_up(v, d, 64);
    if (lane >= d) v += t;
  }
  return v;
}
__device__ __forceinline__ long long wave_incl_scan_ll(long long v, int lane) {
#pragma unroll
  for (int d = 1; d < 64; d <<= 1) {
    long long t = __shfl_up(v, d, 64);
    if (lane >= d) v += t;
  }
  return v;
}

template <typename OutT>
__global__ void __launch_bounds__(LCR_BLOCK) scan_phase1(const int32_t* __restrict__ in, OutT* __restrict__ out, int32_t n,
// ... 155 lines not shown

__global__ void __launch_bounds__(LCR_BLOCK)
k2_compact(BatchView b, DevParams prm, BinomTable bt, const int32_t* __restrict__ tile_region,
           const int32_t* __restrict__ tile_col0, int64_t n_cols, const uint32_t* __restrict__ planes,
           const uint8_t* __restrict__ flags, const int32_t* __restrict__ tile_count, const int32_t* __restrict__ tile_off,
           Survivor* __restrict__ out, int32_t out_cap ) {
  __shared__ int wsum[4];
  if (tile_count[blockIdx.x] == 0) return;
  const int g = tile_region[blockIdx.x], tc0 = tile_col0[blockIdx.x];
  const int tlen = min(LCR_TILE, b.len[g] - tc0);
  const int64_t gcol0 = b.col_off[g] + tc0;
  const int tid = threadIdx.x, lane = tid & 63, w = tid >> 6;
  int base = tile_off[blockIdx.x];
  int f[4], c = 0;
#pragma unroll
  for (int k = 0; k < 4; k++) { int col = tid * 4 + k; f[k] = (col < tlen) ? flags[gcol0 + col] : 0; c += f[k]; }
  int incl = wave_incl_scan_i(c, lane);
  if (lane == 63) wsum[w] = incl;
  __syncthreads();
  int add = 0;
  for (int i = 0; i < w; i++) add += wsum[i];
  int rank = base + incl - c + add;
#pragma unroll
  for (int k = 0; k < 4; k++) {
    if (!f[k]) continue;
    const int col = tid * 4 + k;
    ColEval ev = eval_column(planes, n_cols, gcol0 + col, b.ref[gcol0 + col], prm, bt, b.exon_mask);
    Survivor sv;
    sv.gcol = gcol0 + col; sv.region = g; sv.col = tc0 + col;
    sv.ref_base = ev.ref_base; sv.allele1 = ev.allele1; sv.allele2 = ev.allele2; sv.n_alt = ev.n_alt;
    sv.cnt1 = ev.cnt1; sv.cnt2 = ev.cnt2; sv.depth = ev.depth; sv.af1 = ev.af1; sv.af2 = ev.af2;
    sv.ts_fwd = planes[(int64_t)LCR_PL_TS_FWD * n_cols + gcol0 + col];
    sv.ts_rev = planes[(int64_t)LCR_PL_TS_REV * n_cols + gcol0 + col];
    if (rank < out_cap) out[rank] = sv;
    rank++;
  }
}

__global__ void __launch_bounds__(LCR_BLOCK)
k2_place(const uint4* __restrict__ stage, const int2* __restrict__ key, const int32_t* __restrict__ n_staged, int32_t stage_cap,
         const int32_t* __restrict__ tile_off, uint4* __restrict__ out, int32_t out_cap) {
  static_assert(sizeof(Survivor) == 48, "a survivor record is three 16-byte words");
  const int i = blockIdx.x * LCR_BLOCK + threadIdx.x;
  if (i >= min(*n_staged, stage_cap)) return;
  const int2 k = key[i];
  const int dst = tile_off[k.x] + k.y;
  if (dst < 0 || dst >= out_cap) return;
  const uint4 a = stage[3 * (size_t)i], b = stage[3 * (size_t)i + 1], c = stage[3 * (size_t)i + 2];
  out[3 * (size_t)dst] = a; out[3 * (size_t)dst + 1] = b; out[3 * (size_t)dst + 2] = c;
}


__global__ void __launch_bounds__(LCR_BLOCK)
k2_hist(BatchView b, DevParams prm, const ReadBin* __restrict__ rbin, const Survivor* __restrict__ sv,
        const int32_t* __restrict__ tile_off, int32_t n_tiles, int32_t n_sv, uint32_t* __restrict__ hist, int32_t* __restrict__ hit_cnt, uint2* __restrict__ hit_list,
        int32_t* __restrict__ ovf_cnt, int32_t* __restrict__ ovf_list) {
  const int r = (blockIdx.x * LCR_BLOCK + threadIdx.x) >> 4;
  const bool live = r < b.n_reads;
  const int rr = live ? r : 0;
  const ReadBin h = rbin[rr];
  const int rend = b.read_rend[rr];
  const uint8_t* __restrict__ seq = b.bases + h.seq_off;
  const uint8_t* __restrict__ qual = b.quals + h.seq_off;
  const int l16 = threadIdx.x & 15, rbase = threadIdx.x & 48;
  const int key = h.rel_pos > 0 ? h.rel_pos : 0, rend_c = min(rend, h.vec);
  const bool span = live && rend_c > key;
  const int t0 = h.ftile + (int)((unsigned int)key / (unsigned int)LCR_TILE), t1 = h.ftile + (int)((unsigned int)(max(rend_c, 1) - 1) / (unsigned int)LCR_TILE) + 1;
  uint32_t pre[4];
  {
    const uint32_t* __restrict__ cg = b.cigar + h.cig_off;
#pragma unroll
    for (int k = 0; k < 4; k++) pre[k] = (span && (uint32_t)(16 * k + l16) < (uint32_t)h.n_cig) ? cg[16 * k + l16] : 0u;
  }
  const int s_lo = span ? tile_off[t0] : 0, s_hi = span ? (t1 < n_tiles ? tile_off[t1] : n_sv) : 0;
  int nh = 0;
  uint2* const hl = hit_cnt ? hit_list + (size_t)rr * LCR_HITS : nullptr;
  int cur, s_end;
  auto site_col = [&](int i) { return sv[i].col; };
  row16_find_sites(span && s_lo < s_hi, h, rend, s_lo, s_hi, site_col, &cur, &s_end);
  row16_walk_range(b, h, cur, s_end, pre, site_col,
    [&](int cur_s, int c, bool hit) {
      uint8_t base = 0, rq = 0;
      if (hit) { base = seq[c]; rq = qual[c]; }
      if (hl) {
        const unsigned int hm = (unsigned int)(__ballot(hit) >> rbase) & 0xffffu;
        const int at = nh + __popc(hm & ((1u << l16) - 1u));
        if (hit && at < LCR_HITS) hl[at] = make_uint2((uint32_t)cur_s, (uint32_t)base | ((uint32_t)rq << 8));
        nh += __popc(hm);
      }
      if (!hit) return;
      const uint8_t bq = rq < 30 ? rq : 30;
      bool masked = false;
      if (in_end_zone(c, h.lead, h.reb, prm.dist_to_end))
        masked = prm.ont ? true : polya_masked(seq, b.seq_len[rr], c, prm.polya_len, sv[cur_s].ref_base);
      const int bi = base_code(base);
      if (!masked && bi >= 0) atomicAdd(&hist[((int64_t)cur_s * 4 + bi) * 31 + bq], 1u);
    });
  if (hl && live && l16 == 0) {
    hit_cnt[r] = nh;
    if (nh > LCR_HITS) ovf_list[atomicAdd(ovf_cnt, 1)] = r;
  }
}

void launch_k2_hist(const BatchView& b, const DevParams& p, const ReadBin* rbin, const Survivor* sv,
                    const int32_t* tile_off, int32_t n_tiles, int32_t n_sv, uint32_t* hist, int32_t* hit_cnt, void* hit_list, int32_t* ovf_cnt, int32_t* ovf_list, hipStream_t s) {
  if (b.n_reads == 0) return;
  const int per = LCR_BLOCK / 16;
  hipLaunchKernelGGL(k2_hist, dim3((b.n_reads + per - 1) / per), dim3(LCR_BLOCK), 0, s, b, p, rbin, sv, tile_off, n_tiles, n_sv, hist, hit_cnt, (uint2*)hit_list,
                     ovf_cnt, ovf_list);
}

#ifndef HT_SLOTS
#define HT_SLOTS 256
#endif
#ifndef HT_SPLIT
#define HT_SPLIT 32
#endif
#ifndef HT_BLOCK
#define HT_BLOCK 512
#endif
__global__ void __launch_bounds__(HT_BLOCK)
k2_hist_tiles(BatchView b, const int32_t* __restrict__ tile_col0, const int32_t* __restrict__ tile_count, const int32_t* __restrict__ tile_off,
              const Survivor* __restrict__ sv, const int32_t* __restrict__ ent_off, const uint2* __restrict__ ents,
              const unsigned long long* __restrict__ recs, uint32_t* __restrict__ hist) {
  const int tile = blockIdx.x / HT_SPLIT, part = blockIdx.x % HT_SPLIT, cnt = tile_count[tile];
  if (cnt == 0) return;
  __shared__ uint32_t hp[HT_SLOTS * 62];
  __shared__ uint16_t slot_of[LCR_TILE];
  constexpr int HT_LANES = 8;
  const int tid = threadIdx.x, grp = tid / HT_LANES, ln = tid % HT_LANES;
  const int s0 = tile_off[tile], tc0 = tile_col0[tile];
  const int e0 = ent_off[tile];
  const int n_ent = ent_off[tile + 1] - e0;
  const int j_lo = 16 * (int)((int64_t)n_ent * part / HT_SPLIT), j_hi = 16 * (int)((int64_t)n_ent * (part + 1) / HT_SPLIT);
  if (j_lo >= j_hi) return;
  for (int p0 = 0; p0 < cnt; p0 += HT_SLOTS) {
    const int pc = min(HT_SLOTS, cnt - p0);
    for (int i = tid; i < LCR_TILE; i += HT_BLOCK) slot_of[i] = 0xFFFFu;
    for (int i = tid; i < pc * 62; i += HT_BLOCK) hp[i] = 0u;
    __syncthreads();
    for (int i = tid; i < pc; i += HT_BLOCK) slot_of[sv[s0 + p0 + i].col - tc0] = (uint16_t)i;
    __syncthreads();
    const int c_lo = sv[s0 + p0].col - tc0, c_hi = sv[s0 + p0 + pc - 1].col - tc0;
    auto fetch = [&](int j) -> unsigned long long {
      if (j >= j_hi) return ~0ull;
      const uint2 en = ents[e0 + (j >> 4)];
      return ((unsigned int)j & 15u) < en.y ? recs[en.x + ((unsigned int)j & 15u)] : ~0ull;
    };
    unsigned long long nx = fetch(j_lo + grp), nx2 = fetch(j_lo + grp + HT_BLOCK / HT_LANES);
    for (int j = j_lo + grp; j < j_hi; j += HT_BLOCK / HT_LANES) {
      const unsigned long long rec = nx;
      nx = nx2;
      nx2 = fetch(j + 2 * (HT_BLOCK / HT_LANES));
      const unsigned long long off = rec & REC_OFF_MASK;
      const bool live = off < REC_KIND_N;
      const int col0 = (int)((rec >> 40) & 1023u), len = (int)((rec >> 50) & 1023u) + 1;
      const int d_lo = max(0, c_lo - col0), d_hi = live ? min(len - 1, c_hi - col0) : -1;
      auto tally = [&](int dd, bool in, uint32_t base, uint32_t qual) {
        const uint32_t slot = slot_of[min(col0 + max(dd, 0), LCR_TILE - 1)];
        const uint32_t u = (base & 0xDFu) - 65u;
        const bool acgt = u < 20u && ((0x80045u >> u) & 1u);
        const uint32_t k = ((base & 0xDFu) >> 1) & 3u, bi = k ^ (k >> 1);
        const uint32_t q = min(qual, 30u);
        const uint32_t idx = slot * 124u + bi * 31u + q;
        if (in && acgt && slot != 0xFFFFu) atomicAdd(&hp[idx >> 1], 1u << (16 * (idx & 1u)));
      };
      for (int d0 = d_lo + 4 * ln; d0 <= d_hi; d0 += 4 * HT_LANES) {
        const unsigned long long at = off + (unsigned long long)d0;
        uint32_t bw, qw;
        if (at + 4 <= (unsigned long long)b.n_bases) {
          bw = *reinterpret_cast<const uint32_t*>(b.bases + at); qw = *reinterpret_cast<const uint32_t*>(b.quals + at);
        } else {
          bw = 0; qw = 0;
          for (int t = 0; t < 4; t++) if (at + t < (unsigned long long)b.n_bases) { bw |= (uint32_t)b.bases[at + t] << (8 * t); qw |= (uint32_t)b.quals[at + t] << (8 * t); }
        }
#pragma unroll
        for (int t = 0; t < 4; t++) tally(d0 + t, d0 + t <= d_hi, (bw >> (8 * t)) & 0xFFu, (qw >> (8 * t)) & 0xFFu);
      }
    }
    __syncthreads();
    uint32_t* out = hist + (int64_t)(s0 + p0) * 124;
    for (int i = tid; i < pc * 124; i += HT_BLOCK) {
      const uint32_t v = (hp[i >> 1] >> (16 * (i & 1))) & 0xffffu;
      if (v) atomicAdd(&out[i], v);
    }
    __syncthreads();
  }
}

void launch_k2_hist_tiles(const BatchView& b, const int32_t* tile_col0, int32_t n_tiles, const int32_t* tile_count,
                          const int32_t* tile_off, const Survivor* sv, const int32_t* ent_off, const void* ents, const unsigned long long* recs,
                          uint32_t* hist , hipStream_t s) {
  if (n_tiles == 0) return;
  hipLaunchKernelGGL(k2_hist_tiles, dim3((unsigned)n_tiles * HT_SPLIT), dim3(HT_BLOCK), 0, s, b, tile_col0, tile_count, tile_off, sv, ent_off,
                     (const uint2*)ents, recs, hist);
}

struct GtConst {
  double le[31], l1e[31];
  double log10_2;
  double log_prior[3];
};
static GtConst make_gt_const() {
  GtConst c;
  for (int q = 0; q <= 30; q++) {
    double e = pow(0.1, (double)q / 10.0);
    c.le[q] = log10(e);
    c.l1e[q] = log10(1.0 - e);
  }
  c.log10_2 = log10(2.0);
  const double theta = 0.001;
  c.log_prior[0] = log10(theta / 2.0); c.log_prior[1] = log10(theta); c.log_prior[2] = log10(1.0 - 1.5 * theta);
  return c;
}

__device__ __forceinline__ bool gt_survivor(const DevParams& prm, const GtConst& gc, const Survivor& v, const uint32_t* h,
                                            const int64_t* __restrict__ start0, lcr_candidate& c) {
  const int ri = base_code(v.ref_base);
  {
    int ai = -1; uint32_t ac = 0;
    if (v.allele1 != v.ref_base) { ai = base_code(v.allele1); ac = v.cnt1; }
    else if (v.allele2 != v.ref_base) { ai = base_code(v.allele2); ac = v.cnt2; }
    if (ai >= 0) {
      uint32_t pass = 0;
      for (uint32_t q = prm.min_baseq; q <= 30; q++) pass += h[ai * 31 + q];
      if (ac > 0 && pass < 2) return false;
    }
  }
  double l0 = 0.0, l2 = 0.0;
  uint32_t num_reads = 0;
  for (int q = 0; q <= 30; q++) {
    const uint32_t hm = h[ri * 31 + q];
    uint32_t hx = 0;
#pragma unroll
    for (int bq = 0; bq < 4; bq++) if (bq != ri) hx += h[bq * 31 + q];
    num_reads += hm + hx;
    if (hm) { l0 += (double)hm * gc.le[q]; l2 += (double)hm * gc.l1e[q]; }
    if (hx) { l0 += (double)hx * gc.l1e[q]; l2 += (double)hx * gc.le[q]; }
  }
  double loglik[3] = {l0, 0.0, l2};
  loglik[1] -= (double)num_reads * gc.log10_2;
  double logprob[3] = {loglik[0] + gc.log_prior[0], loglik[1] + gc.log_prior[1], loglik[2] + gc.log_prior[2]};
  const double mlp = fmax(fmax(logprob[0], logprob[1]), logprob[2]);
  double vp[3] = {pow(10.0, logprob[0] - mlp), pow(10.0, logprob[1] - mlp), pow(10.0, logprob[2] - mlp)};
  const double svp = vp[0] + vp[1] + vp[2];
  vp[2] = vp[2] / svp;
  const double variant_quality = -10.0 * log10(fmax(10e-301, vp[2]));
  const double ml = fmax(fmax(loglik[0], loglik[1]), loglik[2]);
  double gl[3] = {pow(10.0, loglik[0] - ml), pow(10.0, loglik[1] - ml), pow(10.0, loglik[2] - ml)};
  const double sgl = gl[0] + gl[1] + gl[2];
  double gp[3] = {gl[0] / sgl, gl[1] / sgl, gl[2] / sgl};
  double ph[3] = {-10.0 * log10(gp[0]), -10.0 * log10(gp[1]), -10.0 * log10(gp[2])};
  for (int i = 1; i < 3; i++) {
    double x = ph[i];
    int j = i;
    while (j > 0 && x < ph[j - 1]) { ph[j] = ph[j - 1]; j--; }
    ph[j] = x;
  }
  const double genotype_quality = ph[1] - ph[0];

  c.pos = start0[v.region] + v.col;
  c.region = v.region;
  c.ref_base = v.ref_base; c.allele1 = v.allele1; c.allele2 = v.allele2; c.n_alt = v.n_alt;
  c.cnt1 = v.cnt1; c.cnt2 = v.cnt2; c.depth = v.depth; c.af1 = v.af1; c.af2 = v.af2;
  c.haplotype = 0; c.phase_set = 0; c.phase_score = 0.0;
  for (int k = 0; k < 3; k++) { c.loglik[k] = loglik[k]; c.gt_prob[k] = gp[k]; }
  c.qual = variant_quality; c.gq = genotype_quality;
  if (gp[0] > gp[1] && gp[0] > gp[2]) { c.variant_type = 2; c.genotype = -1; }
  else if (gp[1] > gp[0] && gp[1] > gp[2]) { c.variant_type = 1; c.genotype = 0; }
  else { c.variant_type = 0; c.genotype = 1; }
  c.flags = 0;
  if (variant_quality < (double)prm.min_qual) return false;
  uint8_t ref_allele_base, alt0; float altf0, altf1 = 0.0f;
  if (v.allele1 == v.ref_base) { ref_allele_base = v.allele1; alt0 = v.allele2; altf0 = v.af2; }
  else if (v.allele2 == v.ref_base) { ref_allele_base = v.allele2; alt0 = v.allele1; altf0 = v.af1; }
  else { ref_allele_base = v.ref_base; alt0 = v.allele1; altf0 = v.af1; altf1 = v.af2; }
  const int fwd_t = (int)v.ts_fwd, rev_t = (int)v.ts_rev;
  bool kept = false;
  if (ref_allele_base == 'A' && alt0 == 'G' && (fwd_t > rev_t * 2 || (fwd_t == 0 && rev_t == 0)) && c.variant_type != 2) {
    c.flags = LCR_F_RNA_EDIT; kept = true;
  } else if (ref_allele_base == 'T' && alt0 == 'C' && (rev_t > fwd_t * 2 || (fwd_t == 0 && rev_t == 0)) && c.variant_type != 2) {
    c.flags = LCR_F_RNA_EDIT; kept = true;
  } else if (v.n_alt == 1 && altf0 < prm.min_af) {
    c.flags = LCR_F_CAND_SOMATIC; kept = true;
  } else if (c.variant_type == 2) {
    if (v.n_alt == 2 && altf0 >= prm.min_af && altf1 >= prm.min_af) { c.variant_type = 3; c.genotype = -1; }
    c.flags = LCR_F_HOM | LCR_F_FOR_PHASING; kept = true;
  } else if (c.variant_type == 1) {
    if (v.n_alt == 2) { c.variant_type = 3; c.genotype = -1; c.flags = LCR_F_HOM | LCR_F_FOR_PHASING; }
    else c.flags = LCR_F_HET | LCR_F_FOR_PHASING;
    kept = true;
  }
  return kept;
}

#define GT_ROWS 64
#define GT_STRIDE 125
#define GT_REC_STRIDE 36
__global__ void __launch_bounds__(GT_ROWS)
k2_gt(DevParams prm, GtConst gc, const Survivor* __restrict__ sv, int32_t n_sv, const uint32_t* __restrict__ hist,
      const int64_t* __restrict__ start0, lcr_candidate* __restrict__ out, int32_t* __restrict__ keep) {
  static_assert(sizeof(lcr_candidate) == 128 && GT_REC_STRIDE * 4 >= (int)sizeof(lcr_candidate) && GT_REC_STRIDE % 4 == 0, "a staged record is eight aligned 16-byte words");
  static_assert(GT_ROWS * GT_REC_STRIDE <= GT_ROWS * GT_STRIDE, "the staged records fit where the rows were");
  __shared__ __attribute__((aligned(16))) uint32_t lds[GT_ROWS * GT_STRIDE];
  const int lane = threadIdx.x;
  const int s0 = blockIdx.x * GT_ROWS, s = s0 + lane;
  const int rows = min(GT_ROWS, n_sv - s0);
  const int n4 = rows * 31;
  const uint4* __restrict__ src = reinterpret_cast<const uint4*>(hist + (int64_t)s0 * 124);
// ... 129 lines not shown
```

### longcallr_amd/csrc/lcr_api.hip

```cpp
#include <chrono>
#include <cmath>
#include <cstdlib>
#include <map>
#include <mutex>

#include "lcr_ctx.h"

namespace {
struct BlockCache {
  std::mutex mu;
  std::multimap<size_t, void*> blocks[2][16];
  size_t held[2][16] = {};
  size_t limit[2] = {(size_t)24 << 30, (size_t)2 << 30};
};
BlockCache& block_cache() { static BlockCache* c = new BlockCache(); return *c; }
}
void* lcr_cache_take(int host, size_t want, size_t* cap) {
  int dev = 0;
  if (hipGetDevice(&dev) != hipSuccess || dev < 0 || dev >= 16) return nullptr;
  BlockCache& bc = block_cache();
  std::lock_guard<std::mutex> g(bc.mu);
  auto& m = bc.blocks[host ? 1 : 0][dev];
  auto it = m.lower_bound(want);
  if (it == m.end() || it->first > 2 * want + (1u << 20)) return nullptr;
// ... 56 lines not shown
  if (!m) return hipSuccess;
  const unsigned blocks = (unsigned)std::max<size_t>(1, std::min<size_t>((most + 255) / 256, 1024));
  hipLaunchKernelGGL(lcr_fill_multi_kernel, dim3(blocks, (unsigned)m), dim3(256), 0, s, r);
  return hipGetLastError();
}

hipError_t lcr_fill_async(void* p, int byte, size_t bytes, hipStream_t s) {
  if (!bytes) return hipSuccess;
  if (!g_lcr_own_fill) return hipMemsetAsync(p, byte, bytes, s);
  const size_t mis = (size_t)((uintptr_t)p & 15), head = std::min(bytes, mis ? 16 - mis : 0), n16 = (bytes - head) / 16, tail = bytes - head - 16 * n16;
  const uint32_t b = (uint32_t)(byte & 255), word = b | (b << 8) | (b << 16) | (b << 24);
  const unsigned blocks = (unsigned)std::max<size_t>(1, std::min<size_t>((n16 + 255) / 256, 2048));
  hipLaunchKernelGGL(lcr_fill_kernel, dim3(blocks), dim3(256), 0, s, (uint8_t*)p, word, head, n16, tail);
  return hipGetLastError();
}

int g_lcr_host_trace = 0;
namespace {
struct HtMark { const char* tag; std::chrono::steady_clock::time_point t; };
thread_local std::vector<HtMark> g_ht;
}
void lcr_host_trace_mark(const char* tag) { g_ht.push_back({tag, std::chrono::steady_clock::now()}); }
void lcr_host_trace_flush() {
  if (g_ht.empty()) return;
  std::string line = "[host]";
  char buf[96];
  for (const HtMark& m : g_ht) { snprintf(buf, sizeof buf, " %s %.1f", m.tag, std::chrono::duration<double, std::micro>(m.t - g_ht[0].t).count()); line += buf; }
  fprintf(stderr, "%s\n", line.c_str());
  g_ht.clear();
}

extern "C" {

const char* lcr_version(void) { return "liblcr 0.1 (gfx950)"; }

int lcr_release_cached_memory(void) {
  BlockCache& bc = block_cache();
  std::lock_guard<std::mutex> g(bc.mu);
  int cur = 0;
  (void)hipGetDevice(&cur);
  for (int dev = 0; dev < 16; dev++) {
    if (bc.blocks[0][dev].empty() && bc.blocks[1][dev].empty()) continue;
    (void)hipSetDevice(dev);
    for (auto& kv : bc.blocks[0][dev]) (void)hipFree(kv.second);
    for (auto& kv : bc.blocks[1][dev]) (void)hipHostFree(kv.second);
    bc.blocks[0][dev].clear(); bc.blocks[1][dev].clear();
    bc.held[0][dev] = bc.held[1][dev] = 0;
  }
  (void)hipSetDevice(cur);
  return LCR_OK;
}
int lcr_set_cache_limits(int64_t device_bytes, int64_t host_bytes) {
  if (device_bytes < 0 || host_bytes < 0) return LCR_E_ARG;
  BlockCache& bc = block_cache();
  std::lock_guard<std::mutex> g(bc.mu);
  bc.limit[0] = (size_t)device_bytes; bc.limit[1] = (size_t)host_bytes;
  return LCR_OK;
}

int lcr_params_preset(int preset, lcr_params* o) {
  if (!o || preset < 0 || preset > 3) return LCR_E_ARG;
  memset(o, 0, sizeof *o);
  const bool ont = preset >= 2;
  o->platform = ont ? LCR_PLATFORM_ONT : LCR_PLATFORM_HIFI;
  o->min_baseq = 10; o->dist_to_end = ont ? 20 : 40; o->polya_len = 5;
  o->min_depth = ont ? 10 : 6; o->max_depth = 50000; o->min_qual = 2;
  o->dense_win = 100; o->min_dense_cnt = 5; o->low_cnt_cut = 10; o->min_linkers = 1; o->max_enum_snps = 10;
  o->ld_weight_threshold = 1;
  o->use_strand_bias = (preset == 0 || preset == 2) ? 1 : 0;
  o->min_af = ont ? 0.20f : 0.15f; o->min_af_intron = 0.0f; o->low_frac_cut = 0.05f;
  o->min_phase_score = ont ? 13.0f : 11.0f;
  o->read_assign_cutoff = 0.0; o->seed = 2025;
  return LCR_OK;
}

int lcr_ctx_create(int device, lcr_ctx** out) {
  if (!out) return LCR_E_ARG;
  int n = 0;
  if (hipGetDeviceCount(&n) != hipSuccess || n <= 0 || device < 0 || device >= n) return LCR_E_DEVICE;
  if (hipSetDevice(device) != hipSuccess) return LCR_E_DEVICE;
  lcr_ctx* c = new lcr_ctx();
  c->device = device;
  if (hipStreamCreateWithFlags(&c->stream, hipStreamNonBlocking) != hipSuccess) { delete c; return LCR_E_DEVICE; }
  c->own_stream = true;
  for (int k = 0; k < LCR_NTIMERS; k++)
    for (int j = 0; j < 2; j++)
      if (hipEventCreate(&c->ev[k][j]) != hipSuccess) { lcr_ctx_destroy(c); return LCR_E_DEVICE; }
  for (hipEvent_t* e : {&c->ev_ctl, &c->ev_sv, &c->ev_cand, &c->ev_nnz, &c->ev_imp, &c->ev_genes})
    if (hipEventCreateWithFlags(e, hipEventDisableTiming) != hipSuccess) { lcr_ctx_destroy(c); return LCR_E_DEVICE; }
  for (CallState* st : c->post_calls()) {
    if (hipEventCreateWithFlags(&st->ev, hipEventDisableTiming) != hipSuccess) { lcr_ctx_destroy(c); return LCR_E_DEVICE; }
    for (hipEvent_t& e : st->ev_t) if (hipEventCreate(&e) != hipSuccess) { lcr_ctx_destroy(c); return LCR_E_DEVICE; }
  }
  *out = c;
  return LCR_OK;
}

void lcr_ctx_destroy(lcr_ctx* c) {
  if (!c) return;
  (void)hipSetDevice(c->device);
  (void)c->phase.settle(nullptr);
  for (hipStream_t q : {c->phase.main_q, c->phase.side, c->phase.aux}) if (q) (void)hipStreamSynchronize(q);
  (void)hipStreamSynchronize(c->stream);
  if (c->up_stream) (void)hipStreamSynchronize(c->up_stream);
  for (auto& u : c->up) if (u.ev) (void)hipEventDestroy(u.ev);
  if (c->up_stream) (void)hipStreamDestroy(c->up_stream);
  for (hipEvent_t e : {c->ev_nnz, c->ev_cand, c->ev_sv, c->ev_ctl, c->ev_imp, c->ev_genes}) if (e) (void)hipEventDestroy(e);
  for (CallState* st : c->post_calls()) for (hipEvent_t e : {st->ev, st->ev_t[0], st->ev_t[1]}) if (e) (void)hipEventDestroy(e);
  for (int k = 0; k < 2 * lcr_ctx::UP_LANES; k++) if (c->ev_up[k]) (void)hipEventDestroy(c->ev_up[k]);
  for (hipEvent_t e : c->ev_mask_t) if (e) (void)hipEventDestroy(e);
  for (hipEvent_t e : c->ev_unpack_t) if (e) (void)hipEventDestroy(e);
  c->phase.release();
  for (int k = 0; k < LCR_NTIMERS; k++) for (int j = 0; j < 2; j++) if (c->ev[k][j]) (void)hipEventDestroy(c->ev[k][j]);
  if (c->own_stream && c->stream) (void)hipStreamDestroy(c->stream);
  delete c;
}

const char* lcr_last_error(const lcr_ctx* c) { return c ? c->err.c_str() : "null ctx"; }

int lcr_ctx_set_stream(lcr_ctx* c, void* s) {
  if (!c) return LCR_E_ARG;
  (void)hipSetDevice(c->device);
  { int rc = phase_settle(c); if (rc) return rc; }
  if (c->own_stream && c->stream) { (void)hipStreamSynchronize(c->stream); (void)hipStreamDestroy(c->stream); }
  if (s) { c->stream = (hipStream_t)s; c->own_stream = false; }
  else { HIPCHK(c, hipStreamCreateWithFlags(&c->stream, hipStreamNonBlocking)); c->own_stream = true; }
  return LCR_OK;
}

int lcr_ctx_sync(lcr_ctx* c) {
  if (!c) return LCR_E_ARG;
  HIPCHK(c, hipSetDevice(c->device));
  { int rc = phase_settle(c); if (rc) return rc; }
  HIPCHK(c, hipStreamSynchronize(c->stream));
  return LCR_OK;
}

int lcr_enable_timing(lcr_ctx* c, int on) { if (!c) return LCR_E_ARG; c->timing = on != 0; return LCR_OK; }

int lcr_kernel_ms(lcr_ctx* c, int k, float* ms) {
  if (!c || !ms || k < 0 || k >= LCR_NTIMERS) return LCR_E_ARG;
  if (!c->ev_valid[k]) return LCR_E_STATE;
  HIPCHK(c, hipEventSynchronize(c->ev[k][1]));
  HIPCHK(c, hipEventElapsedTime(ms, c->ev[k][0], c->ev[k][1]));
  return LCR_OK;
}

int lcr_pileup_bytes(lcr_ctx* c, int64_t* bytes) {
  if (!c || !bytes) return LCR_E_ARG;
  int64_t staged = 0;
  const int rc = pile_staged_bytes(c, &staged);
  *bytes = c->pileup_bytes + staged;
  return rc;
}

int lcr_pileup_stage_bytes(lcr_ctx* c, int64_t* bytes) {
  if (!c || !bytes) return LCR_E_ARG;
  int64_t staged = 0;
  const int rc = pile_staged_bytes(c, &staged);
  *bytes = c->stage_bytes + staged;
  return rc;
}

int lcr_phase(lcr_ctx* c, const lcr_params* p) {
  if (!c || !p) return LCR_E_ARG;
  if (c->stage < ST_FRAGGED) { c->err = "lcr_phase before lcr_fragments"; return LCR_E_STATE; }
  if (c->cand_used) { c->err = "lcr_phase after lcr_phase: the phase stage has rewritten the candidate records; run the candidate stage again"; return LCR_E_STATE; }
  if (p->ld_weight_threshold != 1) { c->err = "ld_weight_threshold must be 1: SNPFrag::phase is only ever called with 1 (thread.rs:166)"; return LCR_E_ARG; }
  const bool ds_on = c->ds_rows_set || c->ds_depth > 0;
  if (ds_on && !(p->read_assign_cutoff > 0.0)) { c->err = "down-sampling needs read_assign_cutoff > 0: the last read assignment must not depend on the sign of an unsampled row's haplotag"; return LCR_E_ARG; }
  HIPCHK(c, hipSetDevice(c->device));
  { int rc = frag_settle(c); if (rc) return rc; }
  PhaseInputs in;
  in.ds_depth = c->ds_depth; in.ds_seed = c->ds_seed; in.ds_rows = c->ds_rows_set ? c->ds_rows.data() : nullptr;
  c->ds_rows_set = false;
  in.n_regions = c->bv.n_regions; in.n_rows = c->n_rows; in.nnz = c->nnz;
  in.row_region_off = c->h_row_region_off.data(); in.cand_region_off = c->h_cand_off.data();
  in.region_start0 = c->h_start0.data();
  in.region_e_off = c->h_nnz.as<int64_t>();
  in.d_row_ptr = c->row_ptr.as<int64_t>(); in.d_col = c->col.as<int32_t>(); in.d_val = c->val.as<uint8_t>();
  in.d_row_links = c->row_links.as<uint32_t>();
  in.cand = &c->h_cand;
  in.d_cand = c->d_cand.as<lcr_candidate>(); in.d_cand_off = c->d_cand_off.as<int32_t>();
  in.d_row_region_off = c->row_region_off.as<int32_t>(); in.d_start0 = c->bv.start0;
  Timer t(c, LCR_K_PHASE);
  c->cand_used = true;
  int rc = c->phase.run(in, *p, c->stream, &c->err);
  if (rc) {
    if (c->phase.q_first) (void)hipStreamSynchronize(c->phase.q_first);
    if (c->phase.side) (void)hipStreamSynchronize(c->phase.side);
    if (c->phase.aux) (void)hipStreamSynchronize(c->phase.aux);
    return rc;
  }
  c->stage = ST_PHASED;
  c->res_valid = true; c->res_ng = c->bv.n_regions;
  c->phase_slot = c->bound_slot >= 0 ? c->bound_slot : (c->bound_host ? -2 : -1);
  return LCR_OK;
}

int lcr_set_downsample(lcr_ctx* c, uint32_t depth, uint64_t seed) {
  if (!c) return LCR_E_ARG;
  c->ds_depth = depth; c->ds_seed = seed;
  return LCR_OK;
}

int lcr_set_downsample_rows(lcr_ctx* c, int32_t mem, int32_t n_rows, const uint8_t* sampled) {
  if (!c || (mem != LCR_MEM_HOST && mem != LCR_MEM_DEVICE)) return LCR_E_ARG;
  if (c->stage < ST_FRAGGED || c->cand_used) { c->err = "lcr_set_downsample_rows names the rows of a fragment stage: call it between lcr_fragments and lcr_phase"; return LCR_E_STATE; }
  if (n_rows != c->n_rows || (n_rows > 0 && !sampled)) { c->err = "lcr_set_downsample_rows: one byte per fragment row of lcr_get_fragmat"; return LCR_E_ARG; }
  c->ds_rows.resize((size_t)n_rows);
  if (n_rows > 0) {
    if (mem == LCR_MEM_HOST) memcpy(c->ds_rows.data(), sampled, (size_t)n_rows);
    else { HIPCHK(c, hipSetDevice(c->device)); HIPCHK(c, hipMemcpy(c->ds_rows.data(), sampled, (size_t)n_rows, hipMemcpyDeviceToHost)); }
  }
  for (uint8_t& b : c->ds_rows) b = b ? 1 : 0;
  c->ds_rows_set = true;
  return LCR_OK;
}

int lcr_get_downsample(lcr_ctx* c, lcr_downsample_info* out) {
  if (!c || !out) return LCR_E_ARG;
  if (!c->res_valid) { c->err = "lcr_get_downsample: no phase results (call it after lcr_phase and before the next candidate stage)"; return LCR_E_STATE; }
  HIPCHK(c, hipSetDevice(c->device));
  { int rc = phase_settle(c); if (rc) return rc; }
  out->n_regions = c->phase.ds_ng; out->n_rows = c->phase.ds_nrow;
  out->region_applied = c->phase.ds_applied.data();
  out->sampled = c->phase.ds_any ? c->phase.h_sampled.as<uint8_t>() : nullptr;
  out->dev_sampled = c->phase.ds_any ? c->phase.d_sampled.as<uint8_t>() : nullptr;
  return LCR_OK;
}

int lcr_discover_regions(lcr_ctx* c, int32_t mem, int32_t n_reads, const int32_t* ref_start, const int32_t* ref_end,
                         int64_t contig_len, lcr_region_list* out) {
  return lcr_discover_regions_truncated(c, mem, n_reads, ref_start, ref_end, contig_len, 0, 0, out, nullptr);
}

int lcr_discover_regions_truncated(lcr_ctx* c, int32_t mem, int32_t n_reads, const int32_t* ref_start, const int32_t* ref_end,
                                   int64_t contig_len, int32_t truncation, uint32_t truncation_coverage, lcr_region_list* out, int64_t* n_truncated) {
  if (!c || !out || n_reads < 0 || contig_len < 0 || contig_len > 0x7FFFFFF0ll) return LCR_E_ARG;
  if (n_truncated) *n_truncated = 0;
  const uint32_t cap = truncation ? truncation_coverage : UINT32_MAX;
  HIPCHK(c, hipSetDevice(c->device));
  c->rl_start0.clear(); c->rl_len.clear(); c->rl_max.clear();
  out->n_regions = 0; out->start0 = nullptr; out->len = nullptr; out->max_cov = nullptr;
  if (n_reads == 0 || contig_len == 0) return LCR_OK;
  const int32_t *d_s = ref_start, *d_e = ref_end;
  if (mem == LCR_MEM_HOST) {
    HIPCHK(c, c->rd_start.reserve((size_t)n_reads * 4)); HIPCHK(c, c->rd_end.reserve((size_t)n_reads * 4));
    { int rc2 = upload_bytes(c, c->rd_start.p, ref_start, (size_t)n_reads * 4); if (rc2) return rc2; rc2 = upload_bytes(c, c->rd_end.p, ref_end, (size_t)n_reads * 4); if (rc2) return rc2; }
    d_s = c->rd_start.as<int32_t>(); d_e = c->rd_end.as<int32_t>();
  }
  int64_t w_lo = contig_len, w_hi = 0;
  if (mem == LCR_MEM_HOST) {
    for (int32_t r = 0; r < n_reads; r++) {
      const int64_t s = ref_start[r], e = std::min<int64_t>(ref_end[r], contig_len);
      if (s >= 0 && s < e) { w_lo = std::min(w_lo, s); w_hi = std::max(w_hi, e); }
    }
  } else {
    HIPCHK(c, c->rd_cnt.reserve(16));
    int32_t init[2] = {INT_MAX, 0}, got[2] = {INT_MAX, 0};
    HIPCHK(c, hipMemcpyAsync(c->rd_cnt.p, init, 8, hipMemcpyHostToDevice, c->stream));
    launch_k5_span_window(d_s, d_e, n_reads, contig_len, c->rd_cnt.as<int32_t>(), c->stream);
    HIPCHK(c, hipMemcpyAsync(got, c->rd_cnt.p, 8, hipMemcpyDeviceToHost, c->stream));
    HIPCHK(c, hipStreamSynchronize(c->stream));
    if (got[1] > 0) { w_lo = got[0]; w_hi = got[1]; }
  }
  if (w_hi <= w_lo) return LCR_OK;
  const int64_t full_len = contig_len;
  contig_len = w_hi - w_lo;
  const size_t nd = (size_t)contig_len + 2;
  HIPCHK(c, c->rd_diff.reserve(nd * 4)); HIPCHK(c, c->rd_ex.reserve((nd + 1) * 4));
  HIPCHK(c, hipMemsetAsync(c->rd_diff.p, 0, nd * 4, c->stream));
  launch_k5_span_diff(d_s, d_e, n_reads, full_len, w_lo, c->rd_diff.as<uint32_t>(), c->stream);
  launch_scan_i32(c->scan_tmp, (const int32_t*)c->rd_diff.p, c->rd_ex.as<int32_t>(), (int32_t)nd, nullptr, c->stream);
  const int32_t nb = (int32_t)((contig_len + 1023) / 1024);
  HIPCHK(c, c->rd_cnt.reserve(((size_t)nb + 1) * 4)); HIPCHK(c, c->rd_off.reserve(((size_t)nb + 2) * 4));
  uint32_t* d_trunc = truncation ? c->rd_off.as<uint32_t>() + nb + 1 : nullptr;
  if (d_trunc) HIPCHK(c, hipMemsetAsync(d_trunc, 0, 4, c->stream));
  launch_k5_bounds(false, c->rd_ex.as<int32_t>(), contig_len, cap, nb, c->rd_cnt.as<int32_t>(), nullptr, nullptr, nullptr, nullptr, 0, d_trunc, c->stream);
  launch_scan_i32(c->scan_tmp, c->rd_cnt.as<int32_t>(), c->rd_off.as<int32_t>(), nb, c->rd_off.as<int32_t>() + nb, c->stream);
  int32_t tot[2] = {0, 0};
  HIPCHK(c, hipMemcpyAsync(tot, c->rd_off.as<int32_t>() + nb, d_trunc ? 8 : 4, hipMemcpyDeviceToHost, c->stream));
  HIPCHK(c, hipStreamSynchronize(c->stream));
  HIPCHK(c, hipGetLastError());
  const int32_t n_isl = tot[0];
  if (n_truncated) *n_truncated = (int64_t)(uint32_t)tot[1];
  if (n_isl == 0) return LCR_OK;
  const int32_t n_keys = 2 * n_isl + 1;
  HIPCHK(c, c->rd_s.reserve((size_t)n_isl * 4)); HIPCHK(c, c->rd_e.reserve((size_t)n_isl * 4)); HIPCHK(c, c->rd_max.reserve((size_t)n_keys * 4));
  HIPCHK(c, hipMemsetAsync(c->rd_max.p, 0, (size_t)n_keys * 4, c->stream));
  launch_k5_bounds(true, c->rd_ex.as<int32_t>(), contig_len, cap, nb, nullptr, c->rd_off.as<int32_t>(), c->rd_s.as<int32_t>(), c->rd_e.as<int32_t>(),
                   c->rd_max.as<uint32_t>(), n_keys, nullptr, c->stream);
  std::vector<int32_t> hs(n_isl), he(n_isl);
  std::vector<uint32_t> hm(n_keys);
  HIPCHK(c, hipMemcpyAsync(hs.data(), c->rd_s.p, (size_t)n_isl * 4, hipMemcpyDeviceToHost, c->stream));
  HIPCHK(c, hipMemcpyAsync(he.data(), c->rd_e.p, (size_t)n_isl * 4, hipMemcpyDeviceToHost, c->stream));
  HIPCHK(c, hipMemcpyAsync(hm.data(), c->rd_max.p, (size_t)n_keys * 4, hipMemcpyDeviceToHost, c->stream));
  HIPCHK(c, hipStreamSynchronize(c->stream));
  HIPCHK(c, hipGetLastError());
  uint32_t running = 0;
  int64_t pend = -1;
  for (int i = 0; i < n_isl; i++) {
    hs[i] += (int32_t)w_lo; he[i] += (int32_t)w_lo;
    running = std::max(running, std::max(hm[2 * i], hm[2 * i + 1]));
    if (pend < 0) pend = hs[i];
    if ((int64_t)he[i] > pend) {
      c->rl_start0.push_back(pend); c->rl_len.push_back((int32_t)(he[i] - pend + 1)); c->rl_max.push_back(running);
      pend = -1; running = 0;
    }
  }
  out->n_regions = (int32_t)c->rl_start0.size();
  out->start0 = c->rl_start0.data(); out->len = c->rl_len.data(); out->max_cov = c->rl_max.data();
  return LCR_OK;
}

int lcr_get_phase_result(lcr_ctx* c, lcr_phase_result* out) {
  if (!c || !out) return LCR_E_ARG;
  if (c->stage < ST_PHASED) { c->err = "lcr_get_phase_result before lcr_phase"; return LCR_E_STATE; }
  { int rc = phase_settle(c); if (rc) return rc; }
  out->n_rows = c->n_rows; out->n_regions = c->bv.n_regions;
  out->haplotag = c->phase.r_haplotag; out->assignment = c->phase.r_assignment;
  out->phase_set = c->phase.r_phase_set; out->objective = c->phase.objective.data();
  return LCR_OK;
}

int lcr_get_read_records_device(lcr_ctx* c, const lcr_read_record** dev_rec, int32_t* n_rows) {
  if (!c || !dev_rec || !n_rows) return LCR_E_ARG;
  if (c->stage < ST_PHASED) { c->err = "lcr_get_read_records_device before lcr_phase"; return LCR_E_STATE; }
  HIPCHK(c, hipSetDevice(c->device));
  { int rc = phase_settle(c); if (rc) return rc; }
  static_assert(sizeof(lcr_read_record) == 12, "lcr_read_record is 12 bytes");
  *dev_rec = c->phase.d_read_rec.as<lcr_read_record>();
  *n_rows = c->n_rows;
  return LCR_OK;
}

int lcr_collect_phase(lcr_ctx* c, lcr_phase_collected* out) {
  if (!c || !out) return LCR_E_ARG;
  if (!c->res_valid) { c->err = "lcr_collect_phase: no phase results (call it after lcr_phase and before the next lcr_candidates)"; return LCR_E_STATE; }
  HIPCHK(c, hipSetDevice(c->device));
  { int rc = phase_settle(c); if (rc) return rc; }
  out->n_regions = c->res_ng; out->n_rows = c->n_rows; out->n_cand = (int32_t)c->h_cand.size(); out->pad_ = 0;
  out->cand = c->h_cand.data(); out->cand_region_off = c->h_cand_off.data(); out->row_region_off = c->h_row_region_off.data();
  out->haplotag = c->phase.r_haplotag; out->assignment = c->phase.r_assignment; out->phase_set = c->phase.r_phase_set;
  out->objective = c->phase.objective.data();
  out->dev_cand = c->d_cand.as<lcr_candidate>(); out->dev_read_rec = c->phase.d_read_rec.as<lcr_read_record>();
  return LCR_OK;
}

int lcr_ctx_set_async_phase(lcr_ctx* c, int on) {
  if (!c) return LCR_E_ARG;
  HIPCHK(c, hipSetDevice(c->device));
  { int rc = phase_settle(c); if (rc) return rc; }
  c->phase.dbg.async_phase = on != 0;
  if (on) {
    const char* q = getenv("GPU_MAX_HW_QUEUES");
    if (!q || atoi(q) < 8) {
      c->err = "asynchronous phase stage: GPU_MAX_HW_QUEUES is unset or below 8 in this process's environment -- the HIP runtime then shares hardware queues "
               "between the stage's streams (results are the same, the overlap is lost); export GPU_MAX_HW_QUEUES=8 before the process starts";
      return LCR_W_HW_QUEUES;
    }
  }
  return LCR_OK;
}

int lcr_ctx_set_lock_dir(lcr_ctx* c, const char* dir) {
  if (!c || !dir) return LCR_E_ARG;
  c->phase.lock_dir = dir;
  return LCR_OK;
}

int lcr_debug_set(lcr_ctx* c, const char* key, int64_t value) {
  if (!c || !key) return LCR_E_ARG;
  PhaseDebug& d = c->phase.dbg;
  const std::string k(key);
  if (k == "phase_prof") d.prof = (int)value;
  else if (k == "grid_min_entries") d.grid_min = value;
  else if (k == "grid_generic") d.grid_generic = (int)value;
  else if (k == "post_half") d.post_half = (int)value;
  else if (k == "enum_force_big") d.enum_force_big = (int)value;
  else if (k == "enum_force_stream") d.enum_force_stream = (int)value;
  else if (k == "enum_elide") d.enum_elide = value != 0;
  else if (k == "async_phase") d.async_phase = value != 0;
  else if (k == "host_trace") g_lcr_host_trace = value != 0;
  else if (k == "own_fill") g_lcr_own_fill = value != 0;
  else if (k == "fill_selftest") {
    HIPCHK(c, hipSetDevice(c->device));
    const size_t N = 4096;
    DevBuf buf;
    struct Drain { hipStream_t s; ~Drain() { (void)hipStreamSynchronize(s); } } drain{c->stream};
    HIPCHK(c, buf.reserve(4 * N));
    std::vector<uint8_t> host(4 * N), want(4 * N);
    for (size_t off = 0; off < 18; off++)
      for (size_t len : {(size_t)0, (size_t)1, (size_t)15, (size_t)16, (size_t)17, (size_t)255, (size_t)1000 + off, (size_t)2049}) {
        HIPCHK(c, hipMemsetAsync(buf.p, 0xAB, 4 * N, c->stream));
        std::fill(want.begin(), want.end(), (uint8_t)0xAB);
        uint8_t* base = buf.as<uint8_t>();
        HIPCHK(c, lcr_fill_async(base + off, 0x5C, len, c->stream));
        std::fill(want.begin() + off, want.begin() + off + len, (uint8_t)0x5C);
        void* const ptrs[4] = {base + N + off, base + 2 * N + 3, nullptr, base + 3 * N + off};
        const int vals[4] = {0x80, 0, 7, 0xFF};
        const size_t sizes[4] = {len, 33, 0, len / 2};
        HIPCHK(c, lcr_fill_multi_async(4, ptrs, vals, sizes, c->stream));
        std::fill(want.begin() + N + off, want.begin() + N + off + len, (uint8_t)0x80);
        std::fill(want.begin() + 2 * N + 3, want.begin() + 2 * N + 3 + 33, (uint8_t)0);
        std::fill(want.begin() + 3 * N + off, want.begin() + 3 * N + off + len / 2, (uint8_t)0xFF);
        HIPCHK(c, hipMemcpyAsync(host.data(), buf.p, 4 * N, hipMemcpyDeviceToHost, c->stream));
        HIPCHK(c, hipStreamSynchronize(c->stream));
        if (host != want) { c->err = "fill_selftest: a fill kernel wrote other bytes than asked (offset " + std::to_string(off) + ", length " + std::to_string(len) + ")"; return LCR_E_DEVICE; }
      }
  }
  else if (k == "chain_ties") d.chain_ties = value != 0;
  else if (k == "redo_lds") d.redo_lds = (int)std::max<int64_t>(0, std::min<int64_t>(value, 128 * 1024));
  else if (k == "tie_arith") d.tie_arith = (int)std::max<int64_t>(0, std::min<int64_t>(value, 3));
  else if (k == "timing_mask") c->timing_mask = (uint32_t)value;
  else if (k == "hist_tiles") c->dbg_hist_tiles = value > 0 ? 1 : value < 0 ? -1 : 0;
  else if (k == "k3_hits") c->dbg_k3_hits = value != 0;
  else if (k == "k3_list_blocks") c->dbg_k3_list_blocks = (int)std::max<int64_t>(0, std::min<int64_t>(value, 65536));
  else if (k == "fuse_filter") c->dbg_fuse_filter = value != 0;
  else if (k == "spec_compact") c->dbg_spec_compact = value != 0;
  else if (k == "lean_planes") c->dbg_lean_planes = value != 0;
  else if (k == "poison_planes") c->dbg_poison_planes = value != 0;
  else if (k == "iso_hash_bits") c->dbg_iso_hash_bits = (int)std::max<int64_t>(0, std::min<int64_t>(value, 64));
  else if (k == "ends_hash_bits") c->dbg_ends_hash_bits = (int)std::max<int64_t>(0, std::min<int64_t>(value, 32));
  else if (k == "grid_spec_batch") d.spec_batch = (int)value;
  else if (k == "grid_spec_lanes") d.spec_lanes = (int)std::max<int64_t>(1, std::min<int64_t>(value, 16));
  else { c->err = "lcr_debug_set: unknown key " + k; return LCR_E_ARG; }
  return LCR_OK;
}

int lcr_get_ld_blocks(lcr_ctx* c, int32_t region, int32_t* n_blocks, const int32_t** block_off, const int32_t** snp_idx) {
  if (!c || !n_blocks || !block_off || !snp_idx) return LCR_E_ARG;
  if (c->stage < ST_PHASED) { c->err = "lcr_get_ld_blocks before lcr_phase"; return LCR_E_STATE; }
  if (region < 0 || region >= c->bv.n_regions) { c->err = "lcr_get_ld_blocks: no such region"; return LCR_E_ARG; }
  { int rc = phase_settle(c); if (rc) return rc; }
  PhaseInputs in;
  in.n_regions = c->bv.n_regions;
  in.cand_region_off = c->h_cand_off.data();
  const int rc = c->phase.ld_blocks(in, region, &c->ld_off, &c->ld_snps, c->stream, &c->err);
  if (rc != LCR_OK) return rc;
  *n_blocks = (int32_t)c->ld_off.size() - 1; *block_off = c->ld_off.data(); *snp_idx = c->ld_snps.data();
  return LCR_OK;
}

int lcr_get_tie_census(lcr_ctx* c, uint64_t out[8]) {
  if (!c || !out) return LCR_E_ARG;
  if (c->stage < ST_PHASED) { c->err = "lcr_get_tie_census before lcr_phase"; return LCR_E_STATE; }
  { int rc = phase_settle(c); if (rc) return rc; }
  for (int i = 0; i < 8; i++) out[i] = i < TIE_NCTR ? (uint64_t)c->phase.tie_census[i] : 0;
  return LCR_OK;
}

}
```

### longcallr_amd/csrc/lcr_ctx.h

```cpp
#pragma once
#include <algorithm>
#include <array>
#include <cstring>

#include "lcr_dev.h"
#include "lcr_phase_host.h"

enum Stage { ST_NONE, ST_LOADED, ST_PILED, ST_CALLED, ST_FRAGGED, ST_PHASED };

struct CallState {
  bool valid = false;
  bool timed = false;
  hipEvent_t ev = nullptr;
  hipEvent_t ev_t[2] = {};
};

struct ColSegs { DevBuf cnt, off, seg; };

struct AnnotationCopy { DevBuf span_s, span_e, exon_off, exon_s, exon_e; };

struct SlotTable {
  int32_t n_slots = 0;
  DevBuf tbl_key, tbl_cnt, flag, koff;
  DevBuf ck, cc, cp;
  DevBuf off;
};

struct GeneJunctions {
  CallState st;
  int32_t n = 0, ng = 0;
  AnnotationCopy ann;
  DevBuf part, nocc, part_off, occ_off, cnt, pair_off, read_pair, row_slot, pregion, pgene, prow0, prows, pocc, tsz, tbl_off, rows, keys, jpair;
  SlotTable t;
  DevBuf d_junc;
  HostBuf h_junc, h_off;
  HostBuf h_ctl;
  HostBuf h_bad;
  int32_t *d_off = nullptr, *d_ctl = nullptr;
  K9Pairs pairs() const {
    return {read_pair.as<int32_t>(), row_slot.as<int32_t>(), pregion.as<int32_t>(), pgene.as<int32_t>(), prow0.as<int32_t>(), prows.as<int32_t>(), pocc.as<int32_t>()};
  }
};

struct AsjModes {
  int32_t nx = 0, n_genes = 0;
  bool cov = false;
  DevBuf dna;
  DevBuf nblk, blk_off, pblk, xtsz, xtbl_off, d_exon;
  SlotTable x;
  DevBuf sup, sup_uniq, sup_n, cov_n;
  HostBuf h_exon, h_xoff, h_cov;
};

struct lcr_ctx {
  int device = 0;
  hipStream_t stream = nullptr;
  bool own_stream = false;
  std::string err;
  Stage stage = ST_NONE;

  BatchView bv{};
  int64_t n_cols = 0, n_bases = 0, n_cigar = 0;
  int32_t n_tiles = 0;
  std::vector<int64_t> h_start0, h_col_off;
  std::vector<int32_t> h_len, h_read_begin, h_region_first_tile;
  DevBuf in_[16];
  struct UploadSlot { DevBuf buf[16]; DevBuf seq4, pack_off;
                      hipEvent_t ev = nullptr; bool filled = false; lcr_reads rd{}; lcr_regions rg{}; } up[2];
  hipStream_t up_stream = nullptr;
  int bound_slot = -1;
  bool bound_host = false;
  DevBuf in_seq4, in_pack_off, unpacked;
  HostBuf h_unpack_bad;
  hipEvent_t ev_unpack_t[2] = {};
  bool unpack_timed = false;
  DevBuf scan_tmp, read_region, read_bin, read_rend, tile_region, tile_col0, first_tile, k0_tile_fill, k0_items, tile_nbase, tile_order;
  DevBuf desc_tile, desc_val, chunks, chunk_off;
  DevBuf blk_first_read, read_scan, cig_compact, cig_off_new, cig_new_off32;
  uint64_t cig0 = 0;
  uint32_t n_ops = 0;
  int64_t n_items = 0;

  bool planes_dense = false;
  bool planes_tallied = false;
  int dbg_poison_planes = 0;
  int dbg_lean_planes = 1;
  DevBuf planes;
  bool sv_staged = false;
  int32_t sv_stage_cap = 0;
  int64_t sv_stage_n = -1;
  DevBuf sv_stage, sv_stage_key;
  DevParams dp{};
  int32_t pile_platform = -1; uint32_t pile_dist_to_end = 0;
  float sor_thr = -1.f;
  HostBuf h_planes;
  HostBuf h_nnz;
  DevBuf region_e_off, frag_tmp_col, frag_tmp_val;
  hipEvent_t ev_ctl = nullptr, ev_sv = nullptr, ev_cand = nullptr, ev_nnz = nullptr, ev_imp = nullptr;
  int32_t sv_cap_guess = 0;
  bool nnz_pending = false, cand_pending = false;
  HostBuf h_order;
  static constexpr int UP_LANES = 4;
  HostBuf h_up[2 * UP_LANES]; hipEvent_t ev_up[2 * UP_LANES] = {}; bool up_busy[2 * UP_LANES] = {};
  HostBuf h_stage[4];

  bool cand_used = false;
  DevBuf flags, tile_count, tile_off, total, survivors, sv_region_off, hist, cand_tmp, keep;
  DevBuf hit_cnt, hit_list, ovf_list;
  bool hits_valid = false; int32_t hits_n_sv = 0;
  int dbg_hist_tiles = 0;
  int dbg_spec_compact = 1;
  int dbg_fuse_filter = 1;
  bool flt_fused = false;
  DevParams flt_dp{};
  uint64_t mask_gen = 0, flt_mask_gen = 0;
  DevBuf exon_plane, ex_off, ex_s, ex_e;
  hipEvent_t ev_mask_t[2] = {};
  bool mask_timed = false;
  int dbg_k3_hits = 1;
  int dbg_k3_list_blocks = 0;
  std::vector<lcr_candidate> h_cand;
  std::vector<int32_t> h_cand_off;
  DevBuf d_cand, d_cand_off;
  DevBuf imp_pos, imp_gt, imp_q, imp_cnt;
  HostBuf h_imp_bad;

  uint32_t min_linkers = 1;
  int32_t n_rows = 0;
  int64_t nnz = 0;
  std::vector<int32_t> h_row_region_off;
  DevBuf region_rows, row_region_off, row_cnt, row_links, row_ptr, col, val;
  HostBuf h_row_ptr, h_row_read, h_col, h_val, h_row_fp, h_row_links;

  bool res_valid = false;
  int32_t res_ng = 0;
  int phase_slot = -1;
  PhaseHost phase;
  std::vector<int32_t> ld_off, ld_snps;
  uint32_t ds_depth = 0; uint64_t ds_seed = 0;
  std::vector<uint8_t> ds_rows; bool ds_rows_set = false;

  CallState hap;
  bool hap_pending = false;
  int32_t hap_ncand = 0;
  DevBuf ht_pos, ht_h1, ht_h2, ht_ps, ht_site, ht_site_ps, d_hsite;
  HostBuf h_hsite, h_hap_bad;

  CallState junc;
  int32_t junc_n = 0, junc_ng = 0;
  DevBuf j_part, j_npair, j_part_off, j_pair_off, j_tsz, j_tbl_off, j_rows, j_keys, j_tbl_key, j_tbl_cnt, j_flag, j_koff, j_ck, j_cc, j_cg, j_off, d_junc;
  HostBuf h_junc_ctl, h_junc, h_junc_off;

  CallState ase;
  int32_t ase_ng = 0;
  DevBuf a_pos, a_pat, a_mat, a_tag, a_site, d_ase;
  HostBuf h_ase, h_ase_bad;

  ColSegs colsegs;
  CallState sc;
  int32_t sc_ncand = 0;
  DevBuf d_sc;
  HostBuf h_sc;
  CallState som;
  int32_t som_ncand = 0;
  DevBuf d_som;
  HostBuf h_som;

  CallState hc;
  int32_t hc_ng = 0, hc_n = 0;
  DevBuf hc_planes, hc_nseg, hc_off, hc_send, d_hc_seg, d_hc_reg;
  HostBuf h_hc_seg, h_hc_off, h_hc_reg;

  CallState iso;
  int32_t iso_ng = 0, iso_n = 0, iso_nchain = 0, iso_nrows = 0;
  int dbg_iso_hash_bits = 64;
  DevBuf iso_part, iso_npair, iso_part_off, iso_pair_off, iso_tsz, iso_tbl_off;
  DevBuf iso_rows, iso_keys, iso_hash, iso_row_slot;
  DevBuf iso_tbl_rep, iso_tbl_cnt, iso_flag, iso_koff, iso_plen, iso_poff;
  DevBuf iso_off, iso_pbase, iso_cslot, iso_crank;
  DevBuf d_iso, d_iso_chain, d_iso_row;
  HostBuf h_iso_ctl, h_iso, h_iso_off, h_iso_chain, h_iso_row;

  CallState ends;
  int32_t ends_ng = 0, ends_n = 0, ends_nrows = 0, ends_npart = 0;
  int dbg_ends_hash_bits = 32;
  DevBuf e_part, e_part_off, e_tsz, e_tbl_off;
  DevBuf e_rows;
  DevBuf e_tbl_key, e_tbl_cnt, e_slot, e_flag, e_koff;
  DevBuf e_off, e_cslot, e_crank, e_nasg;
  DevBuf d_end, d_end_row;
  HostBuf h_end_ctl, h_end, h_end_off, h_end_row;

  bool genes_valid = false;
  int32_t genes_nr = 0, genes_n_genes = 0;
  AnnotationCopy g_ann;
  DevBuf g_pmax, d_gene, d_gene_ov;
  HostBuf h_gene, h_gene_ov, h_gene_bad;
  hipEvent_t ev_genes = nullptr;
  CallState agene;
  int32_t agene_ng = 0, agene_n = 0;
  DevBuf ag_pos, ag_pat, ag_mat, ag_cnt, ag_off, ag_tag, ag_site, ag_site_ps, d_agene;
  HostBuf h_agene, h_agene_off, h_agene_ctl, h_agene_bad;

  GeneJunctions jgene, ajgene;
  AsjModes asj;

  std::array<CallState*, 11> post_calls() { return {&hap, &junc, &ase, &agene, &sc, &hc, &som, &iso, &ends, &jgene.st, &ajgene.st}; }

  DevBuf rd_start, rd_end, rd_diff, rd_ex, rd_cnt, rd_off, rd_s, rd_e, rd_max;
  std::vector<int64_t> rl_start0;
  std::vector<int32_t> rl_len;
  std::vector<uint32_t> rl_max;

  bool timing = false;
  uint32_t timing_mask = 0;
  hipEvent_t ev[LCR_NTIMERS][2] = {};
  bool ev_valid[LCR_NTIMERS] = {};
  int64_t pileup_bytes = 0, stage_bytes = 0;
  bool pile_lean = false;
};

inline void rewind_to(lcr_ctx* c, Stage to) {
  if (c->stage > to) c->stage = to;
  if (to < ST_PILED) {
    c->planes_dense = false;
    c->planes_tallied = false;
    c->sv_staged = false;
    c->flt_fused = false;
  }
  if (to < ST_LOADED) c->bv.exon_mask = nullptr;
  if (to < ST_CALLED) {
    c->hits_valid = false;
    c->cand_used = false;
  }
// ... 108 lines not shown
```

### longcallr_amd/csrc/lcr_dev.h

```cpp
#pragma once
#include <hip/hip_runtime.h>
#include <climits>
#include <cstddef>
#include <stdint.h>

#include <string>
#include <vector>

#include "../../include/lcr.h"

#ifndef LCR_TILE
#define LCR_TILE 256
#endif
#define LCR_BLOCK 256
#define LCR_WAVE 64

struct BatchView {
  int32_t n_reads, n_regions;
  int64_t n_bases;
  const int32_t* pos;
  const int32_t* seq_len;
  const int32_t* lead;
  const int32_t* trail;
  const uint8_t* flags;
  const uint64_t* seq_off;
  const uint64_t* cig_off;
  const uint32_t* n_cig;
  const uint8_t* bases;
  const uint8_t* quals;
  const uint32_t* cigar;
  const int64_t* start0;
  const int32_t* len;
  const int64_t* col_off;
  const int32_t* read_begin;
  const uint8_t* ref;
  const int32_t* region_first_tile;
  const int32_t* read_region;
  int32_t* error_flag;
  int32_t* read_rend;
  const uint32_t* exon_mask;
};

struct ReadBin {
  int32_t rel_pos;
  int32_t vec;
  int32_t ftile;
  int32_t n_cig;
  int64_t gbase;
  uint64_t seq_off, cig_off;
  int32_t lead, reb;
  int32_t flags, pad_;
  int64_t pad2_;
};
static_assert(sizeof(ReadBin) == 64, "ReadBin must be 64 bytes");

struct DevParams {
  int32_t ont;
  int32_t dist_to_end, polya_len;
  uint32_t min_baseq, min_depth, max_depth, min_qual, low_cnt_cut, min_linkers;
  int32_t use_strand_bias;
  float min_af, min_af_intron, low_frac_cut;
  float sor_threshold;
  int32_t dbg;
};

#define REC_OFF_MASK 0xFFFFFFFFFFull
#define REC_KIND_D 0xFFFFFFFFFFull
#define REC_KIND_I 0xFFFFFFFFFEull
#define REC_KIND_N 0xFFFFFFFFFDull

struct Survivor {
  int64_t gcol;
  int32_t region;
  int32_t col;
  uint8_t ref_base, allele1, allele2, n_alt;
  uint32_t cnt1, cnt2, depth;
  uint32_t ts_fwd, ts_rev;
  float af1, af2;
};

#define HIPCHK(ctx, expr)                                                              \
  do {                                                                                 \
    hipError_t e_ = (expr);                                                            \
    if (e_ != hipSuccess) {                                                            \
      (ctx)->err = std::string(#expr) + ": " + hipGetErrorString(e_);                  \
      return LCR_E_DEVICE;                                                             \
    }                                                                                  \
  } while (0)

void* lcr_cache_take(int host, size_t want, size_t* cap);
bool lcr_cache_put(int host, void* p, size_t cap);

extern int g_lcr_host_trace;
void lcr_host_trace_mark(const char* tag);
void lcr_host_trace_flush();
#define HT(tag) do { if (g_lcr_host_trace) lcr_host_trace_mark(tag); } while (0)

extern int g_lcr_own_fill;
hipError_t lcr_fill_async(void* p, int byte, size_t bytes, hipStream_t s);
hipError_t lcr_fill_multi_async(int n , void* const* ptrs, const int* bytes_val, const size_t* sizes, hipStream_t s);

struct DevBuf {
  void* p = nullptr;
  size_t cap = 0;
  DevBuf() = default;
  DevBuf(const DevBuf&) = delete; DevBuf& operator=(const DevBuf&) = delete;
  ~DevBuf() { if (p && !lcr_cache_put(0, p, cap)) (void)hipFree(p); }
  hipError_t reserve(size_t bytes) {
    if (bytes <= cap) return hipSuccess;
    if (p) { (void)hipDeviceSynchronize(); if (!lcr_cache_put(0, p, cap)) (void)hipFree(p); }
    p = nullptr;
    cap = 0;
    size_t want = bytes + bytes / 8 + 256;
    if ((p = lcr_cache_take(0, want, &cap)) != nullptr) return hipSuccess;
    hipError_t e = hipMalloc(&p, want);
    if (e == hipSuccess) cap = want; else p = nullptr;
    return e;
  }
  template <class T> T* as() const { return reinterpret_cast<T*>(p); }
};
struct HostBuf {
  void* p = nullptr;
  size_t cap = 0;
  HostBuf() = default;
  HostBuf(const HostBuf&) = delete; HostBuf& operator=(const HostBuf&) = delete;
  ~HostBuf() { if (p && !lcr_cache_put(1, p, cap)) (void)hipHostFree(p); }
  hipError_t reserve(size_t bytes) {
    if (bytes <= cap) return hipSuccess;
    if (p) { (void)hipDeviceSynchronize(); if (!lcr_cache_put(1, p, cap)) (void)hipHostFree(p); }
    p = nullptr;
    cap = 0;
    size_t want = bytes + bytes / 8 + 256;
    if ((p = lcr_cache_take(1, want, &cap)) != nullptr) return hipSuccess;
    hipError_t e = hipHostMalloc(&p, want, hipHostMallocDefault);
    if (e == hipSuccess) cap = want; else p = nullptr;
    return e;
  }
  template <class T> T* as() const { return reinterpret_cast<T*>(p); }
  template <class T> hipError_t dev(T** out) const { return hipHostGetDevicePointer((void**)out, p, 0); }
};

struct PhaseLutDev {
  int64_t fe[31], f1e[31];
  int64_t f_homref, f_homvar, f_het0, f_log2;
};

struct K0Ctl {
  unsigned int pool_top, n_items, n_recs;
  int32_t error;
  unsigned int desc_top;
  unsigned int empty_cols;
  unsigned int pad_[2];
};
static_assert(sizeof(K0Ctl) == 32, "K0Ctl is eight words: the host fetches it with one 32-byte copy");
static_assert(offsetof(K0Ctl, error) == 12, "BatchView::error_flag is word 3 of K0Ctl");

void launch_k0_region_setup(const int64_t* start0, const int32_t* len, const int64_t* col_off, const int32_t* read_begin, int32_t ng,
                            int32_t* first_tile, int64_t* h_start0, int32_t* h_len, int64_t* h_col_off, int32_t* h_read_begin,
                            hipStream_t s);
void launch_k0_tiles(const int32_t* first_tile, int32_t n_regions, int32_t* tile_region, int32_t* tile_col0, hipStream_t s);
void launch_k0_read_region(const BatchView& b, int32_t* read_region, hipStream_t s);
void launch_k0_tiles_read_region(const BatchView& b, const int32_t* first_tile, int32_t* tile_region, int32_t* tile_col0, int32_t* read_region, hipStream_t s);
void launch_k0_pack(const BatchView& b, ReadBin* out, int32_t* order_flag , hipStream_t s);
void launch_k0_bind_a(const int64_t* start0, const int32_t* len, const int64_t* col_off, const int32_t* read_begin, int32_t ng,
                      int32_t* first_tile, int64_t* h_start0, int32_t* h_len, int64_t* h_col_off, int32_t* h_read_begin,
                      const uint64_t* cig_off, const uint32_t* n_cig, int32_t nr, int64_t n_cigar, int32_t* out, hipStream_t s);
void launch_k0_bind_b(const BatchView& b, ReadBin* rbin, int32_t* order_flag, int32_t* read_region, int32_t n_tiles, int32_t* tile_region,
                      int32_t* tile_col0, uint64_t cig0, int32_t opb, int32_t n_blocks, int32_t* blk_first_read, hipStream_t s);
void launch_k0_unpack(int32_t nr, const int32_t* seq_len, const uint64_t* seq_off, const uint64_t* pack_off, const uint8_t* seq4, int64_t n_pack,
                      uint8_t* out, int64_t n_bases, int32_t* bad , hipStream_t s);
void launch_k0_cig_check(const uint64_t* cig_off, const uint32_t* n_cig, int32_t nr, int64_t n_cigar, int32_t* out, hipStream_t s);
void launch_k0_cig_compact(const uint32_t* cigar, const uint64_t* cig_off, const uint32_t* n_cig, const int32_t* new_off, int32_t nr,
                           uint32_t* out, uint64_t* out_off, hipStream_t s);
int launch_k0_opb();
void launch_k0_block_reads(const ReadBin* rbin, int32_t nr, uint64_t cig0, int32_t opb, int32_t n_blocks, int32_t* blk_first_read, hipStream_t s);
void launch_k0_ops(const BatchView& b, const ReadBin* rb, const int32_t* blk_first_read, uint64_t cig0, uint32_t n_ops, int ont, int D,
                   int32_t n_tiles, int32_t* tile_fill, int32_t* tile_nchunks, int32_t* tile_ndiff, K0Ctl* ctl, unsigned int* acct ,
                   unsigned int pool_sub , unsigned long long* recs, unsigned int desc_sub, uint32_t* desc_tile, void* desc_val ,
                   void* read_scan , hipStream_t s);
int launch_k0_acct_words();
int launch_k0_acct_slots();
void launch_k0_desc_bin(const K0Ctl* ctl, const unsigned int* acct, unsigned int desc_sub, const uint32_t* desc_tile, const void* desc_val,
                        const int32_t* chunk_off, int32_t* cursor , void* sorted , int32_t n_blocks_hint,
                        hipStream_t s);
size_t launch_k1_tiles_tmp_words(int32_t n_tiles);
struct PileScratch {
  size_t ctl;
  size_t ndiff;
  size_t nch;
  size_t cur;
  size_t acct;
  size_t tmp;
  size_t words;
};
inline PileScratch pile_scratch(int32_t n_tiles) {
  const size_t nt = (size_t)n_tiles;
  PileScratch L{};
  L.ctl = nt + 1; L.ndiff = nt + 16; L.nch = L.ndiff + nt + 8; L.cur = L.nch + nt + 8; L.acct = L.cur + nt + 8;
  L.tmp = L.acct + launch_k0_acct_words();
  L.words = (L.tmp + launch_k1_tiles_tmp_words(n_tiles) + 63) & ~(size_t)63;
  return L;
}
void launch_k1_tiles_a(int32_t n_tiles, const int32_t* tile_fill, const int32_t* tile_ndiff, const int32_t* tile_nent, int32_t* tmp ,
                       const unsigned int* acct, int32_t n_acct, K0Ctl* ctl, K0Ctl* host_ctl ,
                       const int32_t* tile_region, const int32_t* tile_col0, const int32_t* region_len , hipStream_t s);
void launch_k1_tiles_b(int32_t n_tiles, const int32_t* tile_fill, const int32_t* tile_ndiff, const int32_t* tile_nent, int32_t* tmp,
                       int32_t* tile_nbase, int32_t* ent_off, int32_t* order, int32_t* flt_count , hipStream_t s);
void launch_k1_pileup(const BatchView& b, const DevParams& p, const int32_t* tile_region, const int32_t* tile_col0,
                      int32_t n_tiles, int64_t n_cols, const int32_t* tile_fill, const int32_t* chunk_off, const void* chunks,
                      const unsigned long long* recs, const int32_t* tile_nbase, uint32_t* planes, const int32_t* order,
                      const int32_t* tiles_tmp , hipStream_t s,
                      uint8_t* flt_flags , int32_t* flt_count );
#define K1_TMP_NFULL 80
#define K1_TMP_STAGED 83
void launch_k1_pileup_lean(const BatchView& b, const DevParams& p, const int32_t* tile_region, const int32_t* tile_col0,
                           int32_t n_tiles, int64_t n_cols, const int32_t* tile_fill, const int32_t* chunk_off, const void* chunks,
                           const unsigned long long* recs, const int32_t* tile_nbase, const int32_t* order, int32_t* tiles_tmp , hipStream_t s,
                           int32_t* flt_count, Survivor* stage, void* stage_key, int32_t stage_cap);
void launch_k2_place(const Survivor* stage, const void* stage_key, const int32_t* n_staged, int32_t stage_cap, const int32_t* tile_off,
                     Survivor* out, int32_t out_cap, hipStream_t s);
void launch_k1_empty_tiles(const BatchView& b, const int32_t* tile_region, const int32_t* tile_col0, int32_t n_tiles, int64_t n_cols,
                           const int32_t* tile_nbase, uint32_t* planes, const int32_t* order, const int32_t* tiles_tmp, hipStream_t s);
void launch_k1_zonefix(const BatchView& b, const ReadBin* rbin, int D, int L, int64_t n_cols, uint32_t* planes, hipStream_t s);
void launch_k2_filter(const BatchView& b, const DevParams& p, const int32_t* tile_region, const int32_t* tile_col0,
                      int32_t n_tiles, int64_t n_cols, const uint32_t* planes, const int32_t* tile_fill, uint8_t* flags,
                      int32_t* tile_count, hipStream_t s);
void launch_gather_i32(const int32_t* src, const int32_t* idx, int32_t n, int32_t n_src, const int32_t* total, int32_t* out, hipStream_t s,
                       int32_t* host_out = nullptr );
void launch_scan_i32(DevBuf& tmp, const int32_t* in, int32_t* out_excl, int32_t n, int32_t* total, hipStream_t s);
void launch_k2_compact(const BatchView& b, const DevParams& p, const int32_t* tile_region, const int32_t* tile_col0,
                       int32_t n_tiles, int64_t n_cols, const uint32_t* planes, const uint8_t* flags,
                       const int32_t* tile_count, const int32_t* tile_off, Survivor* out, int32_t out_cap, hipStream_t s);
float lcr_device_sor_threshold(hipStream_t s);
#define LCR_HITS 16
void launch_k2_hist(const BatchView& b, const DevParams& p, const ReadBin* rbin, const Survivor* sv, const int32_t* tile_off , int32_t n_tiles, int32_t n_sv,
                    uint32_t* hist , int32_t* hit_cnt , void* hit_list ,
                    int32_t* ovf_cnt , int32_t* ovf_list , hipStream_t s);
void launch_k2_hist_tiles(const BatchView& b, const int32_t* tile_col0, int32_t n_tiles, const int32_t* tile_count,
                          const int32_t* tile_off, const Survivor* sv, const int32_t* ent_off, const void* ents, const unsigned long long* recs,
                          uint32_t* hist, hipStream_t s);
void launch_k2_gt(const DevParams& p, const Survivor* sv, int32_t n_sv, const uint32_t* hist, const int64_t* start0,
                  lcr_candidate* out, int32_t* keep, hipStream_t s);
void launch_k2_finish(DevBuf& scan_tmp, const lcr_candidate* tmp, const int32_t* keep, int32_t n_sv, const int32_t* sv_region_off,
                      int32_t n_regions, int32_t* pos, int32_t* idx, lcr_candidate* out, int32_t* cand_off, uint32_t dense_win,
                      uint32_t min_dense_cnt, hipStream_t s, lcr_candidate* h_cand = nullptr, int32_t* h_off = nullptr);
void launch_k2_import_count(const BatchView& b, const int64_t* pos0, const uint8_t* gt, const float* qual, int32_t n_sites, int32_t* count , hipStream_t s);
void launch_k2_import_emit(const BatchView& b, int64_t n_cols, const uint32_t* planes, const int32_t* tile_fill , const int64_t* pos0, const uint8_t* gt, const float* qual,
                           int32_t n_sites, const int32_t* cand_off , lcr_candidate* out, hipStream_t s,
                           lcr_candidate* h_cand , int32_t* h_off );
void launch_k2_import_check(const int64_t* pos0, const uint8_t* gt, int32_t n_sites, int32_t* bad , hipStream_t s);
void launch_k2_exon_check(const int32_t* iv_off, const int64_t* iv_start0, const int64_t* iv_end0, int32_t n_regions, int32_t* verdict, hipStream_t s);
void launch_k2_exon_build(const BatchView& b, const int32_t* iv_off, const int64_t* iv_start0, const int64_t* iv_end0, int32_t n_iv, uint32_t* plane , hipStream_t s);
void launch_k3_region_entries(const int64_t* row_ptr, const int32_t* row_region_off, int32_t ng, int64_t* region_e_off, hipStream_t s, int64_t* host_out = nullptr);
struct K3Hits {
  const int32_t* hit_cnt; const void* hit_list; const int32_t* ovf_cnt; const int32_t* ovf_list;
  const int32_t* keep; const int32_t* pos;
};
void launch_k3_count(const BatchView& b, const ReadBin* rbin, const lcr_candidate* cand, const int32_t* cand_region_off,
                     const int32_t* row_region_off, int32_t n_rows, int32_t* row_cnt, uint32_t* row_links, int32_t* tmp_col,
                     uint8_t* tmp_val, const K3Hits& hits, int list_blocks , hipStream_t s);
void launch_k3_fill(const BatchView& b, const ReadBin* rbin, const lcr_candidate* cand, const int32_t* cand_region_off,
                    const int32_t* row_region_off, int32_t n_rows, int32_t* row_cnt, const int64_t* row_ptr, const int32_t* tmp_col,
                    const uint8_t* tmp_val, int32_t* col, uint8_t* val, const K3Hits& hits, int list_blocks, hipStream_t s);
int launch_k3_inline();
void launch_k3_rows_offsets(const BatchView& b, const lcr_candidate* cand, const int32_t* cand_region_off, int32_t* region_rows, int32_t* row_region_off,
                            hipStream_t s, int32_t* host_rows = nullptr );
void launch_scan_i32_to_i64(DevBuf& tmp, const int32_t* in, int64_t* out_excl, int32_t n, hipStream_t s);

void launch_k5_span_window(const int32_t* ref_start, const int32_t* ref_end, int32_t n, int64_t contig_len, int32_t* out , hipStream_t s);
void launch_k5_span_diff(const int32_t* ref_start, const int32_t* ref_end, int32_t n, int64_t contig_len, int64_t lo , uint32_t* diff, hipStream_t s);
void launch_k5_bounds(bool write, const int32_t* ex, int64_t contig_len, uint32_t cap, int32_t n_blocks, int32_t* blk_cnt, const int32_t* blk_off,
                      int32_t* starts, int32_t* ends, uint32_t* imax, int32_t n_keys, uint32_t* n_trunc, hipStream_t s);

void launch_k6_count(const BatchView& b, const int32_t* row_region_off, const lcr_read_record* rec, uint32_t min_junctions,
                     int32_t* part_flag, int32_t* npair, hipStream_t s);
void launch_k6_sizes(const BatchView& b, const int32_t* part_off , const int32_t* pair_off , int32_t* tsz ,
                     int32_t* host_ctl , hipStream_t s);
size_t launch_k6_row_bytes();
void launch_k6_emit(const BatchView& b, const int32_t* row_region_off, const lcr_read_record* rec, const int32_t* part_flag,
                    const int32_t* part_off, const int32_t* pair_off, const int32_t* tbl_off , void* rows, uint64_t* keys,
                    uint64_t* tbl_key , uint32_t* tbl_cnt , hipStream_t s);
void launch_k6_flag(const uint64_t* tbl_key, const uint32_t* tbl_cnt, int32_t n_slots, uint32_t min_count, int32_t* flag, hipStream_t s);
void launch_k6_offsets(const int32_t* tbl_off, const int32_t* koff , int32_t ng, int32_t n_slots, int32_t* joff, int32_t* host_joff,
                       int32_t* host_ctl , hipStream_t s);
void launch_k6_place(const BatchView& b, const uint64_t* tbl_key, const uint32_t* tbl_cnt, const int32_t* flag, const int32_t* koff,
                     const int32_t* tbl_off, int32_t n_slots, const int32_t* joff, int32_t n_kept, uint64_t* ck, uint32_t* cc, int32_t* cgr,
                     lcr_junction* junc, hipStream_t s);
void launch_k6_tables(const BatchView& b, const int32_t* part_off, const void* rows, const uint64_t* keys, int32_t n_kept, lcr_junction* junc,
                      lcr_junction* host_junc , hipStream_t s);

void launch_k7_check(const int64_t* pos0, const uint8_t* pat, const uint8_t* mat, int32_t n_sites, int32_t* bad , hipStream_t s);
void launch_k7_pick(const int32_t* row_region_off, const lcr_read_record* rec, int32_t ng, lcr_ase_region* out,
                    lcr_ase_region* host_out , int32_t* row_tag , hipStream_t s);
void launch_k7_sites(const lcr_candidate* cand, int32_t n_cand, double min_phase_score, const int64_t* pos0, const uint8_t* pat,
                     const uint8_t* mat, int32_t n_sites, lcr_ase_region* ase, uint8_t* site , hipStream_t s);
void launch_k7_votes(const int32_t* row_tag, int32_t n_rows, const int64_t* row_ptr, const int32_t* col, const uint8_t* val, const uint8_t* site,
                     uint32_t min_baseq, lcr_ase_region* ase, hipStream_t s);
void launch_k7_export(const lcr_ase_region* ase, int32_t ng, lcr_ase_region* host_out , hipStream_t s);

struct K11Sites { const int64_t* pos0; const uint8_t* h1; const uint8_t* h2; const uint32_t* ps; int32_t n; };
struct K11Rows {
  int8_t* haplotag; uint8_t* assignment; uint32_t* phase_set;
  uint32_t* d_rec;
};
void launch_k11_check(const K11Sites& st, int32_t* bad , hipStream_t s);
void launch_k11_sites(lcr_candidate* cand, int32_t n_cand, const K11Sites& st, uint8_t* site , uint32_t* site_ps ,
                      lcr_haplotag_site* acc , hipStream_t s);
void launch_k11_rows(int32_t n_rows, const int64_t* row_ptr, const int32_t* col, const uint8_t* val, const uint8_t* site, const uint32_t* site_ps,
                     const PhaseLutDev& lut , uint32_t min_linkers, double cutoff, const K11Rows& out, lcr_haplotag_site* acc, hipStream_t s);
void launch_k11_finish(lcr_candidate* cand, int32_t n_cand, const uint8_t* site, const lcr_haplotag_site* acc, lcr_candidate* host_cand ,
                       lcr_haplotag_site* host_acc , hipStream_t s);

void launch_colseg_count(int32_t n_rows, const int64_t* row_ptr, const int32_t* col, int32_t n_cand, uint32_t* cnt , hipStream_t s);
void launch_k12_fill(int32_t n_rows, const int64_t* row_ptr, const int32_t* col, const uint8_t* val, const lcr_read_record* rec, uint32_t min_baseq,
                     int32_t n_cand, uint32_t* cnt , const int64_t* off , uint64_t* seg , hipStream_t s);
void launch_k12_sites(const lcr_candidate* cand, int32_t n_cand, const int64_t* off, const uint64_t* seg, lcr_site_count* out,
                      lcr_site_count* host_out , hipStream_t s);

struct K14Tables {
  int64_t tab[4 * 31];
  int64_t prior[3];
};
void launch_k14_fill(int32_t n_rows, const int64_t* row_ptr, const int32_t* col, const uint8_t* val, const lcr_read_record* rec, const lcr_candidate* cand,
                     int32_t n_cand, uint32_t* cnt , const int64_t* off , uint64_t* seg , hipStream_t s);
void launch_k14_sites(const lcr_candidate* cand, int32_t n_cand, const int64_t* off, const uint64_t* seg, const K14Tables& t, uint32_t min_baseq,
                      lcr_somatic_site* out, lcr_somatic_site* host_out , hipStream_t s);

void launch_k13_blocks(const BatchView& b, const int32_t* row_region_off, const lcr_read_record* rec, int64_t n_cols,
                       uint32_t* planes , hipStream_t s);
// ... 274 lines not shown
```

### longcallr_amd/csrc/lcr_pileup.hip

```cpp
#include "lcr_ctx.h"

namespace {

struct PilePools {
  int32_t n_blocks = 0;
  size_t pool_cap64 = 0, desc_cap64 = 0;
  size_t n_shards = 0;
  unsigned int pool_sub = 0, desc_sub = 0;
};

PilePools pile_size_pools(const lcr_ctx* c) {
  PilePools P;
  const int opb = launch_k0_opb();
  P.n_blocks = (int32_t)(((uint64_t)c->n_ops + opb - 1) / opb);
  P.desc_cap64 = (size_t)P.n_blocks * 128 + (size_t)c->bv.n_reads / 4 + 1024;
  P.pool_cap64 = (size_t)c->n_ops + (size_t)c->n_ops / 2 + (size_t)c->bv.n_reads + (size_t)c->n_bases / LCR_TILE + 8 * P.desc_cap64 + 1024;
  return P;
}

int pile_reserve_pools(lcr_ctx* c, PilePools& P) {
  const size_t nsh = P.n_shards = (size_t)launch_k0_acct_slots();
  const size_t pool_sub64 = (P.pool_cap64 + nsh - 1) / nsh + 256, desc_sub64 = (P.desc_cap64 + nsh - 1) / nsh + 64;
  if (pool_sub64 * nsh > 0xFFFFFFF0ull || desc_sub64 * nsh > 0x7FFFFFF0ull) { c->err = "batch too large for the 32-bit record pool: split it"; return LCR_E_ARG; }
  P.pool_sub = (unsigned int)pool_sub64; P.desc_sub = (unsigned int)desc_sub64;
  HIPCHK(c, c->k0_items.reserve(pool_sub64 * nsh * 8));
  HIPCHK(c, c->desc_tile.reserve(desc_sub64 * nsh * 4));
  HIPCHK(c, c->desc_val.reserve(desc_sub64 * nsh * 8));
  HIPCHK(c, c->chunks.reserve((pool_sub64 * nsh / 16 + desc_sub64 * nsh + 16) * 8));
  return LCR_OK;
}

int pile_reserve_scratch(lcr_ctx* c, const PileScratch& L) {
  const int nt = c->n_tiles;
  HIPCHK(c, c->k0_tile_fill.reserve(L.words * 4));
  c->bv.error_flag = &reinterpret_cast<K0Ctl*>(c->k0_tile_fill.as<int32_t>() + L.ctl)->error;
  HIPCHK(c, c->tile_order.reserve(std::max(nt, 1) * 4));
  HIPCHK(c, c->tile_nbase.reserve(std::max(nt, 1) * 4));
  HIPCHK(c, c->chunk_off.reserve(((size_t)nt + 2) * 4));
  HIPCHK(c, c->read_scan.reserve(std::max<size_t>(c->bv.n_reads, 1) * 8));
  HIPCHK(c, c->h_stage[0].reserve(64));
  return LCR_OK;
}

int pile_queue_k0(lcr_ctx* c, const PileScratch& L, const PilePools& P, bool& gated) {
  int32_t* const fill = c->k0_tile_fill.as<int32_t>();
  HIPCHK(c, lcr_fill_async(fill, 0, L.words * 4, c->stream));
  if (!gated) { HIPCHK(c, c->phase.gate_stream(c->stream)); gated = true; }
  Timer t(c, LCR_K_SPANS);
  launch_k0_ops(c->bv, c->read_bin.as<ReadBin>(), c->blk_first_read.as<int32_t>(), c->cig0, c->n_ops, c->dp.ont, c->dp.dist_to_end, c->n_tiles,
                fill, fill + L.nch, fill + L.ndiff, reinterpret_cast<K0Ctl*>(fill + L.ctl), (unsigned int*)(fill + L.acct), P.pool_sub, c->k0_items.as<unsigned long long>(),
                P.desc_sub, c->desc_tile.as<uint32_t>(), c->desc_val.p, c->read_scan.p, c->stream);
  return LCR_OK;
}

int pile_queue_tally(lcr_ctx* c, const PileScratch& L, const PilePools& P, bool fuse, bool lean) {
  BatchView& b = c->bv;
  const int nt = c->n_tiles;
  int32_t* const fill = c->k0_tile_fill.as<int32_t>();
  K0Ctl* const d_ctl = reinterpret_cast<K0Ctl*>(fill + L.ctl);
  { Timer t(c, LCR_K_PILEUP);
    if (nt > 0) {
      K0Ctl* h_ctl_dev = nullptr;
      HIPCHK(c, c->h_stage[0].dev(&h_ctl_dev));
      launch_k1_tiles_a(nt, fill, fill + L.ndiff, fill + L.nch, fill + L.tmp, (unsigned int*)(fill + L.acct), launch_k0_acct_slots(),
                        d_ctl, h_ctl_dev, c->tile_region.as<int32_t>(), c->tile_col0.as<int32_t>(), b.len, c->stream);
    } else HIPCHK(c, hipMemcpyAsync(c->h_stage[0].p, d_ctl, sizeof(K0Ctl), hipMemcpyDeviceToHost, c->stream));
    HIPCHK(c, hipEventRecord(c->ev_ctl, c->stream));
    if (nt > 0) launch_k1_tiles_b(nt, fill, fill + L.ndiff, fill + L.nch, fill + L.tmp, c->tile_nbase.as<int32_t>(), c->chunk_off.as<int32_t>(),
                                  c->tile_order.as<int32_t>(), fuse ? c->tile_count.as<int32_t>() : nullptr, c->stream);
    if (nt > 0 && c->n_ops > 0)
      launch_k0_desc_bin(d_ctl, (const unsigned int*)(fill + L.acct), P.desc_sub, c->desc_tile.as<uint32_t>(), c->desc_val.p, c->chunk_off.as<int32_t>(), fill + L.cur,
                         c->chunks.p, P.n_blocks / 8 + 1, c->stream);
    if (lean)
      launch_k1_pileup_lean(b, c->dp, c->tile_region.as<int32_t>(), c->tile_col0.as<int32_t>(), nt, c->n_cols, fill, c->chunk_off.as<int32_t>(),
                            c->chunks.p, c->k0_items.as<unsigned long long>(), c->tile_nbase.as<int32_t>(), c->tile_order.as<int32_t>(), fill + L.tmp,
                            c->stream, c->tile_count.as<int32_t>(), c->sv_stage.as<Survivor>(), c->sv_stage_key.p, c->sv_stage_cap);
    else
      launch_k1_pileup(b, c->dp, c->tile_region.as<int32_t>(), c->tile_col0.as<int32_t>(), nt, c->n_cols, fill, c->chunk_off.as<int32_t>(),
                       c->chunks.p, c->k0_items.as<unsigned long long>(), c->tile_nbase.as<int32_t>(), c->planes.as<uint32_t>(),
                       c->tile_order.as<int32_t>(), fill + L.tmp, c->stream, fuse ? c->flags.as<uint8_t>() : nullptr, fuse ? c->tile_count.as<int32_t>() : nullptr);
    if (!c->dp.ont && c->dp.dist_to_end > 0)
      launch_k1_zonefix(b, c->read_bin.as<ReadBin>(), c->dp.dist_to_end, c->dp.polya_len, c->n_cols, c->planes.as<uint32_t>(), c->stream); }
  HIPCHK(c, hipGetLastError());
  return LCR_OK;
}

int pile_read_verdict(lcr_ctx* c, K0Ctl* out, bool* retry) {
  HIPCHK(c, hipEventSynchronize(c->ev_ctl));
  HT("pile:ctl");
  *out = *c->h_stage[0].as<K0Ctl>();
  if (c->n_tiles == 0) out->empty_cols = 0;
  if (*c->h_order.as<int32_t>() != 0) { c->err = "the reads of a region must be sorted by position (lcr_reads.pos)"; return LCR_E_ARG; }
  if (out->error == 1) { c->err = "unknown CIGAR operation (reference panics: util.rs:944)"; return LCR_E_CIGAR; }
  if (out->error == 2) { c->err = "CIGAR inconsistent with l_seq / soft clips"; return LCR_E_CIGAR; }
  *retry = out->error != 0;
  return LCR_OK;
}

}

int planes_tally(lcr_ctx* c, bool with_filter) {
  if (c->planes_tallied && !with_filter) return LCR_OK;
  if (with_filter) HIPCHK(c, c->flags.reserve(std::max<size_t>(c->n_cols, 1)));
  launch_k1_pileup(c->bv, c->flt_dp, c->tile_region.as<int32_t>(), c->tile_col0.as<int32_t>(), c->n_tiles, c->n_cols, c->k0_tile_fill.as<int32_t>(),
                   c->chunk_off.as<int32_t>(), c->chunks.p, c->k0_items.as<unsigned long long>(), c->tile_nbase.as<int32_t>(), c->planes.as<uint32_t>(),
                   c->tile_order.as<int32_t>(), c->k0_tile_fill.as<int32_t>() + pile_scratch(c->n_tiles).tmp, c->stream,
                   with_filter ? c->flags.as<uint8_t>() : nullptr, with_filter ? c->tile_count.as<int32_t>() : nullptr);
  HIPCHK(c, hipGetLastError());
  c->planes_tallied = true;
  return LCR_OK;
}

int planes_materialise(lcr_ctx* c) {
  { int rc = planes_tally(c, false); if (rc) return rc; }
  if (c->planes_dense) return LCR_OK;
  launch_k1_empty_tiles(c->bv, c->tile_region.as<int32_t>(), c->tile_col0.as<int32_t>(), c->n_tiles, c->n_cols, c->tile_nbase.as<int32_t>(),
                        c->planes.as<uint32_t>(), c->tile_order.as<int32_t>(), c->k0_tile_fill.as<int32_t>() + pile_scratch(c->n_tiles).tmp, c->stream);
  HIPCHK(c, hipGetLastError());
  c->planes_dense = true;
  return LCR_OK;
}

int pile_staged_bytes(lcr_ctx* c, int64_t* bytes) {
  *bytes = 0;
  if (!c->pile_lean || c->stage < ST_PILED) return LCR_OK;
  if (c->sv_stage_n < 0) {
    int32_t n = 0;
    HIPCHK(c, hipSetDevice(c->device));
    HIPCHK(c, hipMemcpyAsync(&n, c->k0_tile_fill.as<int32_t>() + pile_scratch(c->n_tiles).tmp + K1_TMP_STAGED, 4, hipMemcpyDeviceToHost, c->stream));
    HIPCHK(c, hipStreamSynchronize(c->stream));
    c->sv_stage_n = std::min(n, c->sv_stage_cap);
  }
  *bytes = (int64_t)sizeof(Survivor) * c->sv_stage_n;
  return LCR_OK;
}

extern "C" {

int lcr_pileup(lcr_ctx* c, const lcr_params* p) {
  HT("pileup");
  if (!c || !p) return LCR_E_ARG;
  if (c->stage < ST_LOADED) { c->err = "lcr_pileup before lcr_load_batch"; return LCR_E_STATE; }
  if (p->polya_len == 0) { c->err = "polya_len must be >= 1"; return LCR_E_ARG; }
  if ((uint64_t)c->bv.n_reads * 2ull * p->dist_to_end > 0x7FFFFF00ull * (uint64_t)LCR_BLOCK) { c->err = "dist_to_end x reads too large for one launch; split the batch"; return LCR_E_ARG; }
  HIPCHK(c, hipSetDevice(c->device));
  if (c->sor_thr < 0.f) c->sor_thr = lcr_device_sor_threshold(c->stream);
  c->dp = to_dev(p, c->sor_thr);
  c->dp.dbg = 0;
  HIPCHK(c, c->planes.reserve(std::max<size_t>((size_t)c->n_cols * LCR_NPLANES, 1) * 4));
  rewind_to(c, ST_LOADED);
  if (c->dbg_poison_planes) HIPCHK(c, lcr_fill_async(c->planes.p, 0xA5, (size_t)c->n_cols * LCR_NPLANES * 4, c->stream));
  const int nt = c->n_tiles;
  PilePools P = pile_size_pools(c);
  const PileScratch L = pile_scratch(nt);
  int rc;
  if ((rc = pile_reserve_scratch(c, L))) return rc;
  const bool fuse = c->dbg_fuse_filter != 0 && c->dp.ont && nt > 0;
  const bool lean = fuse && c->sv_cap_guess > 0 && c->dbg_lean_planes != 0;
  if (fuse) HIPCHK(c, c->tile_count.reserve(std::max(nt, 1) * 4));
  if (fuse && !lean) HIPCHK(c, c->flags.reserve(std::max<size_t>(c->n_cols, 1)));
  if (lean) {
    c->sv_stage_cap = c->sv_cap_guess;
    HIPCHK(c, c->sv_stage.reserve((size_t)c->sv_stage_cap * sizeof(Survivor)));
    HIPCHK(c, c->sv_stage_key.reserve((size_t)c->sv_stage_cap * 8));
  }
  K0Ctl ctl{};
  bool gated = false;
  for (bool retry = true; retry;) {
    if ((rc = pile_reserve_pools(c, P))) return rc;
    if ((rc = pile_queue_k0(c, L, P, gated))) return rc;
    if ((rc = pile_queue_tally(c, L, P, fuse, lean))) return rc;
    if ((rc = pile_read_verdict(c, &ctl, &retry))) return rc;
    if (retry) {
      P.pool_cap64 = std::max<size_t>(P.pool_cap64 * 2, ((size_t)ctl.pool_top + 1024) * P.n_shards);
      P.desc_cap64 = std::max<size_t>(P.desc_cap64 * 2, ((size_t)ctl.desc_top + 1024) * P.n_shards);
    }
  }
  c->n_items = (int32_t)ctl.n_recs;
  const int64_t plane_cols = lean ? 0 : c->n_cols - (int64_t)ctl.empty_cols;
  c->pileup_bytes = c->n_bases + 8 * (int64_t)(int32_t)ctl.n_items + c->n_cols + 4 * LCR_NPLANES * plane_cols;
  c->stage_bytes = c->n_bases + 4 * c->n_cigar + 37 * (int64_t)c->bv.n_reads + c->n_cols + 4 * LCR_NPLANES * plane_cols;
  c->stage = ST_PILED;
  c->planes_tallied = !lean; c->sv_staged = c->pile_lean = lean; c->sv_stage_n = -1;
  c->flt_fused = fuse; c->flt_dp = c->dp; c->flt_mask_gen = c->mask_gen;
  c->pile_platform = p->platform; c->pile_dist_to_end = p->dist_to_end;
  return LCR_OK;
}

int lcr_get_columns(lcr_ctx* c, lcr_columns* out) {
  if (!c || !out) return LCR_E_ARG;
  if (c->stage < ST_PILED) { c->err = "lcr_get_columns before lcr_pileup"; return LCR_E_STATE; }
  HIPCHK(c, hipSetDevice(c->device));
  { int rc = planes_materialise(c); if (rc) return rc; }
  const size_t bytes = (size_t)c->n_cols * LCR_NPLANES * 4;
  HIPCHK(c, c->h_planes.reserve(std::max<size_t>(bytes, 1)));
  if (bytes) HIPCHK(c, hipMemcpyAsync(c->h_planes.p, c->planes.p, bytes, hipMemcpyDeviceToHost, c->stream));
  HIPCHK(c, hipStreamSynchronize(c->stream));
  out->n_cols = c->n_cols;
  out->planes = c->h_planes.as<uint32_t>();
  return LCR_OK;
}

}
```

Before: 6.843 billion.

## Fold single-base deletions and following insertions into match records

In the k0 op-expansion kernel, a match op that is immediately followed by an insertion, or by a one-base deletion, now carries a flag bit in its packed record, and the following indel record is dropped. The pileup tally kernel applies the folded indel counts from that flag, so fewer records are emitted, sorted and tallied. The record bit layout is narrowed to 8-bit column and length fields to make room for the flags, and a waves-per-EU occupancy hint is added to k0. This adds cross-lane shuffles and edge cases at tile and wave boundaries, plus a new debug switch and a record-count query.

```diff
diff --git a/include/lcr.h b/include/lcr.h
--- a/include/lcr.h
+++ b/include/lcr.h
@@ -429,6 +429,7 @@
 int lcr_kernel_ms(lcr_ctx*, int kernel, float* ms);
 int lcr_pileup_bytes(lcr_ctx*, int64_t* bytes);
 int lcr_pileup_stage_bytes(lcr_ctx*, int64_t* bytes);
+int lcr_pileup_records(lcr_ctx*, int64_t* items, int64_t* records);
 
 int lcr_release_cached_memory(void);
 int lcr_set_cache_limits(int64_t device_bytes, int64_t host_bytes);
diff --git a/longcallr_amd/_lib.py b/longcallr_amd/_lib.py
--- a/longcallr_amd/_lib.py
+++ b/longcallr_amd/_lib.py
@@ -11,7 +11,7 @@
     "lcr_ctx_sync", "lcr_ctx_set_lock_dir", "lcr_ctx_set_async_phase", "lcr_debug_set", "lcr_load_batch", "lcr_load_batch_async", "lcr_bind_batch",
     "lcr_host_alloc", "lcr_host_free", "lcr_host_register", "lcr_host_unregister", "lcr_pileup", "lcr_get_columns", "lcr_candidates",
     "lcr_get_candidates", "lcr_get_candidates_device", "lcr_fragments", "lcr_get_fragmat", "lcr_phase", "lcr_get_phase_result", "lcr_get_read_records_device", "lcr_collect_phase", "lcr_get_ld_blocks", "lcr_get_tie_census",
-    "lcr_enable_timing", "lcr_kernel_ms", "lcr_pileup_bytes", "lcr_pileup_stage_bytes", "lcr_discover_regions", "lcr_discover_regions_truncated", "lcr_version", "lcr_release_cached_memory", "lcr_set_cache_limits",
+    "lcr_enable_timing", "lcr_kernel_ms", "lcr_pileup_bytes", "lcr_pileup_stage_bytes", "lcr_pileup_records", "lcr_discover_regions", "lcr_discover_regions_truncated", "lcr_version", "lcr_release_cached_memory", "lcr_set_cache_limits",
     "lcr_bam_open", "lcr_bam_open_keep", "lcr_bam_close", "lcr_bam_last_error", "lcr_bam_refs", "lcr_bam_n_records", "lcr_bam_resident", "lcr_bam_spans", "lcr_bam_batch", "lcr_bam_write_phased", "lcr_bam_write_reads",
     "lcr_set_downsample", "lcr_set_downsample_rows", "lcr_get_downsample",
     "lcr_junctions", "lcr_get_junctions", "lcr_ase", "lcr_get_ase", "lcr_vcf_contig_alleles",
@@ -91,6 +91,7 @@
     l.lcr_kernel_ms.argtypes = [vp, i32, C.POINTER(C.c_float)]
     l.lcr_pileup_bytes.argtypes = [vp, C.POINTER(C.c_int64)]
     l.lcr_pileup_stage_bytes.argtypes = [vp, C.POINTER(C.c_int64)]
+    l.lcr_pileup_records.argtypes = [vp, C.POINTER(C.c_int64), C.POINTER(C.c_int64)]
     flt = C.POINTER(_abi.LcrReadFilter)
     l.lcr_bam_open.argtypes = [C.c_char_p, C.c_int32, C.POINTER(vp)]
     l.lcr_bam_open_keep.argtypes = [C.c_char_p, C.c_int32, C.c_int64, C.POINTER(vp)]
diff --git a/longcallr_amd/api.py b/longcallr_amd/api.py
--- a/longcallr_amd/api.py
+++ b/longcallr_amd/api.py
@@ -22,7 +22,7 @@
 
 _DEBUG_ENV = {"LCR_PHASE_PROF": "phase_prof", "LCR_GRID_MIN_ENTRIES": "grid_min_entries",
               "LCR_GRID_GENERIC": "grid_generic", "LCR_GRID_SPEC_LANES": "grid_spec_lanes", "LCR_GRID_SPEC_BATCH": "grid_spec_batch", "LCR_POST_HALF": "post_half", "LCR_ENUM_FORCE_BIG": "enum_force_big",
-              "LCR_ENUM_FORCE_STREAM": "enum_force_stream", "LCR_ENUM_ELIDE": "enum_elide", "LCR_HIST_TILES": "hist_tiles", "LCR_TIE_ARITH": "tie_arith", "LCR_CHAIN_TIES": "chain_ties", "LCR_K3_HITS": "k3_hits", "LCR_K3_LIST_BLOCKS": "k3_list_blocks", "LCR_FUSE_FILTER": "fuse_filter", "LCR_ASYNC_PHASE": "async_phase", "LCR_HOST_TRACE": "host_trace", "LCR_OWN_FILL": "own_fill", "LCR_REDO_LDS": "redo_lds", "LCR_SPEC_COMPACT": "spec_compact", "LCR_LEAN_PLANES": "lean_planes"}
+              "LCR_ENUM_FORCE_STREAM": "enum_force_stream", "LCR_ENUM_ELIDE": "enum_elide", "LCR_HIST_TILES": "hist_tiles", "LCR_TIE_ARITH": "tie_arith", "LCR_CHAIN_TIES": "chain_ties", "LCR_K3_HITS": "k3_hits", "LCR_K3_LIST_BLOCKS": "k3_list_blocks", "LCR_FUSE_FILTER": "fuse_filter", "LCR_ASYNC_PHASE": "async_phase", "LCR_HOST_TRACE": "host_trace", "LCR_OWN_FILL": "own_fill", "LCR_REDO_LDS": "redo_lds", "LCR_SPEC_COMPACT": "spec_compact", "LCR_LEAN_PLANES": "lean_planes", "LCR_FOLD_INDELS": "fold_indels"}
 
 
 class Engine:
@@ -546,6 +546,11 @@
         self._chk(self.lib.lcr_pileup_stage_bytes(self.h, C.byref(b)), "lcr_pileup_stage_bytes")
         return int(b.value)
 
+    def pileup_records(self):
+        items, recs = C.c_int64(), C.c_int64()
+        self._chk(self.lib.lcr_pileup_records(self.h, C.byref(items), C.byref(recs)), "lcr_pileup_records")
+        return int(items.value), int(recs.value)
+
 
 def host_register(*arrays):
     lib = _lib.load()
diff --git a/longcallr_amd/csrc/k0_ops.hip b/longcallr_amd/csrc/k0_ops.hip
--- a/longcallr_amd/csrc/k0_ops.hip
+++ b/longcallr_amd/csrc/k0_ops.hip
@@ -90,9 +90,9 @@
 }
 
 template <int OPT>
-__global__ void __launch_bounds__(K0_THREADS)
+__global__ void __launch_bounds__(K0_THREADS) __attribute__((amdgpu_waves_per_eu(7)))
 k0_ops(BatchView b, const ReadBin* __restrict__ rbin, const int32_t* __restrict__ blk_first_read, uint64_t cig0, uint32_t n_ops,
-       int ont, int D, int32_t n_tiles, int32_t* __restrict__ tile_fill, int32_t* __restrict__ tile_nchunks, int32_t* __restrict__ tile_ndiff,
+       int ont, int D, int fold, int32_t n_tiles, int32_t* __restrict__ tile_fill, int32_t* __restrict__ tile_nchunks, int32_t* __restrict__ tile_ndiff,
        K0Ctl* __restrict__ ctl, unsigned int* __restrict__ acct, unsigned int pool_sub, unsigned long long* __restrict__ recs,
        unsigned int desc_sub, uint32_t* __restrict__ desc_tile, uint2* __restrict__ desc_val, int2* __restrict__ read_scan) {
   constexpr int OPB = OPT * K0_THREADS, WOPS = OPT * 64;
@@ -138,7 +138,7 @@
     x.vec = h.vec; x.ftile = h.ftile; x.seq_off = h.seq_off; x.reb = h.reb; x.rel_pos = h.rel_pos;
     const int strand = h.flags & 1, ts = (h.flags >> 1) & 3;
     const uint32_t tscls = ts == 0 ? 0u : ((strand == 0) == (ts == 1) ? 1u : 2u);
-    x.hi = ((uint32_t)strand << 28) | (tscls << 29);
+    x.hi = ((uint32_t)strand << REC_HI_STRAND_SHIFT) | (tscls << REC_HI_TS_SHIFT);
     const uint64_t cb = h.cig_off - cig0;
     x.cend = (int32_t)min<int64_t>((int64_t)cb + h.n_cig - (int64_t)j0, INT_MAX);
     *cb_out = cb; *ncig_out = h.n_cig;
@@ -175,9 +175,11 @@
 
   if (K0_ABL == 1) return;
   int dr[OPT], dq[OPT], xr[OPT], xq[OPT], rid[OPT], mark[OPT];
+  unsigned int nxc;
   {
     bool bad_op = false;
     int tr = 0, tq = 0, tm = 0;
+    unsigned int selfc = 0u;
     const uint2 mk = *reinterpret_cast<const uint2*>(&ridh[OPT * tid]);
 #pragma unroll
     for (int k = 0; k < OPT; k++) {
@@ -190,6 +192,12 @@
       xr[k] = tr; xq[k] = tq;
       tr += dr[k]; tq += dq[k];
       tm = max(tm, mark[k]); rid[k] = tm;
+      if (fold && mark[k] == 0) selfc |= (op == 1 && len > 0 ? 1u : op == 2 && len == 1 ? 2u : 0u) << (2 * k);
+    }
+    {
+      unsigned int c0n = (unsigned int)__shfl_down((int)(selfc & 3u), 1, 64);
+      if (lane == 63) c0n = 0u;
+      nxc = (selfc >> 2) | (c0n << (2 * (OPT - 1)));
     }
     if (bad_op) atomicExch(&ctl->error, 1);
     const int ir = wave_incl_scan(tr), iq = wave_incl_scan(tq), im = wave_incl_max(tm);
@@ -236,9 +244,15 @@
     int kd = ((m || d || isn) && len > 0 && ee > aa) ? (m ? 1 : d ? 2 : 4) : 0;
     if (ins && len > 0 && rs >= 1 && rs < H.vec) { kd = 3; aa = rs - 1; ee = rs; }
     kind[k] = kd; a[k] = aa; e[k] = ee; tb[k] = H.ftile;
+    unsigned int fl = 0u;
+    if (kd == 1 && ee == rs + len && ee < H.vec && p + 1 < H.cend) {
+      const unsigned int cn = (nxc >> (2 * k)) & 3u;
+      if (cn == 1u) fl = REC_HI_F_INS;
+      else if (cn == 2u && ((unsigned int)ee % (unsigned int)LCR_TILE) != 0u) fl = REC_HI_F_DEL;
+    }
     if (kd == 1) {
       const unsigned long long o0 = H.seq_off + (unsigned long long)(long long)(qs - rs);
-      rlo[k] = (unsigned int)o0; rhi[k] = ((unsigned int)(o0 >> 32) & 0xffu) | H.hi;
+      rlo[k] = (unsigned int)o0; rhi[k] = ((unsigned int)(o0 >> 32) & 0xffu) | H.hi | fl;
     } else {
       rlo[k] = kd == 2 ? (unsigned int)REC_KIND_D : kd == 3 ? (unsigned int)REC_KIND_I : (unsigned int)REC_KIND_N;
       rhi[k] = 0xffu;
@@ -254,15 +268,24 @@
     }
   }
 
+  {
+    constexpr unsigned int FM = REC_HI_F_INS | REC_HI_F_DEL;
+    unsigned int fp = (unsigned int)__shfl_up((int)(kind[OPT - 1] == 1 ? rhi[OPT - 1] & FM : 0u), 1, 64);
+    if (lane == 0) fp = 0u;
+#pragma unroll
+    for (int k = OPT - 1; k >= 0; k--) if ((k == 0 ? fp : (kind[k - 1] == 1 ? rhi[k - 1] & FM : 0u)) != 0u) kind[k] = 0;
+  }
+
   if (K0_ABL == 3) { int x = 0; for (int k = 0; k < OPT; k++) x += a[k] + e[k] + tb[k] + kind[k] + (int)rlo[k] + (int)rhi[k]; if (x == 0x7fffffff) ctl->error = 9; return; }
   auto make_rec = [&](int k, int t) -> unsigned long long {
     const int c0 = (t - tb[k]) * LCR_TILE;
     const int c_lo = max(a[k], c0), c_hi = min(e[k], c0 + LCR_TILE);
-    unsigned int lo = rlo[k], hi = rhi[k] | ((unsigned int)(c_lo - c0) << 8) | ((unsigned int)(c_hi - c_lo - 1) << 18);
+    unsigned int lo = rlo[k], hi = rhi[k] | ((unsigned int)(c_lo - c0) << REC_HI_COL_SHIFT) | ((unsigned int)(c_hi - c_lo - 1) << REC_HI_LEN_SHIFT);
     if (kind[k] == 1) {
       const unsigned int s = lo + (unsigned int)c_lo;
       hi = (hi & ~0xffu) | (((hi & 0xffu) + (s < lo ? 1u : 0u)) & 0xffu);
       lo = s;
+      if (c_hi != e[k]) hi &= ~(REC_HI_F_INS | REC_HI_F_DEL);
     }
     return ((unsigned long long)hi << 32) | lo;
   };
@@ -432,13 +455,13 @@
                      chunk_off, cursor, (uint2*)sorted);
 }
 
-void launch_k0_ops(const BatchView& b, const ReadBin* rb, const int32_t* blk_first_read, uint64_t cig0, uint32_t n_ops, int ont, int D,
+void launch_k0_ops(const BatchView& b, const ReadBin* rb, const int32_t* blk_first_read, uint64_t cig0, uint32_t n_ops, int ont, int D, int fold,
                    int32_t n_tiles, int32_t* tile_fill, int32_t* tile_nchunks, int32_t* tile_ndiff, K0Ctl* ctl, unsigned int* acct,
                    unsigned int pool_sub, unsigned long long* recs, unsigned int desc_sub, uint32_t* desc_tile, void* desc_val, void* read_scan,
                    hipStream_t s) {
   if (b.n_reads == 0) return;
   if (n_ops == 0) { hipLaunchKernelGGL(k0_empty_reads, dim3((b.n_reads + LCR_BLOCK - 1) / LCR_BLOCK), dim3(LCR_BLOCK), 0, s, b, rb, ctl); return; }
   const int opb = launch_k0_opb();
-  hipLaunchKernelGGL(k0_ops<K0_OPT>, dim3((n_ops + opb - 1) / opb), dim3(K0_THREADS), 0, s, b, rb, blk_first_read, cig0, n_ops, ont, D, n_tiles,
+  hipLaunchKernelGGL(k0_ops<K0_OPT>, dim3((n_ops + opb - 1) / opb), dim3(K0_THREADS), 0, s, b, rb, blk_first_read, cig0, n_ops, ont, D, fold, n_tiles,
                      tile_fill, tile_nchunks, tile_ndiff, ctl, acct, pool_sub, recs, desc_sub, desc_tile, (uint2*)desc_val, (int2*)read_scan);
 }
diff --git a/longcallr_amd/csrc/k1_pileup.hip b/longcallr_amd/csrc/k1_pileup.hip
--- a/longcallr_amd/csrc/k1_pileup.hip
+++ b/longcallr_amd/csrc/k1_pileup.hip
@@ -281,20 +281,20 @@
       const int slot = tid * K1_RPB + x;
       const unsigned long long rec = rec_cur[x];
       const bool hasrec = (has_cur >> x) & 1;
-      const unsigned long long off = rec & REC_OFF_MASK;
-      const int col0 = (int)((rec >> 40) & 1023u), len = (int)((rec >> 50) & 1023u) + 1;
+      const unsigned long long off = rec_off(rec);
+      const int col0 = rec_col(rec), len = rec_len(rec);
       int npieces = 0;
       if (hasrec) {
         if (off == REC_KIND_D) {
           atomicAdd(&pl[P_DIFF_D * TSTRIDE + col0], 1u);
           atomicAdd(&pl[P_DIFF_D * TSTRIDE + col0 + len], 0xFFFFFFFFu);
         } else if (off == REC_KIND_I) {
-          atomicAdd(&pl[P_NI * TSTRIDE + col0], 1u);
+          if (!LEAN) atomicAdd(&pl[P_NI * TSTRIDE + col0], 1u);
         } else if (off == REC_KIND_N) {
           atomicAdd(&pl[P_DIFF_N * TSTRIDE + col0], 1u);
           atomicAdd(&pl[P_DIFF_N * TSTRIDE + col0 + len], 0xFFFFFFFFu);
         } else {
-          const int strand = (int)((rec >> 60) & 1u), tscls = (int)((rec >> 61) & 3u);
+          const int strand = rec_strand(rec), tscls = rec_tscls(rec);
           uint32_t* dp = pl + (strand ? P_DIFF_DEPTH_R : P_DIFF_DEPTH_F) * TSTRIDE;
           atomicAdd(&dp[col0], 1u);
           atomicAdd(&dp[col0 + len], 0xFFFFFFFFu);
@@ -303,6 +303,11 @@
             atomicAdd(&tp[col0], 1u);
             atomicAdd(&tp[col0 + len], 0xFFFFFFFFu);
           }
+          if (rec_f_del(rec)) {
+            atomicAdd(&pl[P_DIFF_D * TSTRIDE + col0 + len], 1u);
+            atomicAdd(&pl[P_DIFF_D * TSTRIDE + col0 + len + 1], 0xFFFFFFFFu);
+          }
+          if (!LEAN && rec_f_ins(rec)) atomicAdd(&pl[P_NI * TSTRIDE + col0 + len - 1], 1u);
           npieces = (len + 15) >> 4;
         }
       }
@@ -334,10 +339,9 @@
       if (pstride == 1) lo = pown[p];
       else { lo = pown[p / pstride]; while (pstart[lo + 1] <= p) lo++; }
       const unsigned long long rc = rec_s[lo];
-      const uint32_t rhi = (uint32_t)(rc >> 32);
-      const long long soff = (long long)(rc & REC_OFF_MASK);
-      const int scol = (int)((rhi >> 8) & 1023u), slen = (int)((rhi >> 18) & 1023u) + 1;
-      q.strand = (int)((rhi >> 28) & 1u);
+      const long long soff = (long long)rec_off(rc);
+      const int scol = rec_col(rc), slen = rec_len(rc);
+      q.strand = rec_strand(rc);
       const int d16 = 16 * (p - pstart[lo]);
       const long long A = soff + d16;
       q.k_lo = 0; q.k_hi = min(16, slen - d16);
diff --git a/longcallr_amd/csrc/k2_candidates.hip b/longcallr_amd/csrc/k2_candidates.hip
--- a/longcallr_amd/csrc/k2_candidates.hip
+++ b/longcallr_amd/csrc/k2_candidates.hip
@@ -331,9 +331,9 @@
       const unsigned long long rec = nx;
       nx = nx2;
       nx2 = fetch(j + 2 * (HT_BLOCK / HT_LANES));
-      const unsigned long long off = rec & REC_OFF_MASK;
-      const bool live = off < REC_KIND_N;
-      const int col0 = (int)((rec >> 40) & 1023u), len = (int)((rec >> 50) & 1023u) + 1;
+      const unsigned long long off = rec_off(rec);
+      const bool live = rec_is_m(rec);
+      const int col0 = rec_col(rec), len = rec_len(rec);
       const int d_lo = max(0, c_lo - col0), d_hi = live ? min(len - 1, c_hi - col0) : -1;
       auto tally = [&](int dd, bool in, uint32_t base, uint32_t qual) {
         const uint32_t slot = slot_of[min(col0 + max(dd, 0), LCR_TILE - 1)];
diff --git a/longcallr_amd/csrc/lcr_api.hip b/longcallr_amd/csrc/lcr_api.hip
--- a/longcallr_amd/csrc/lcr_api.hip
+++ b/longcallr_amd/csrc/lcr_api.hip
@@ -232,6 +232,13 @@
   const int rc = pile_staged_bytes(c, &staged);
   *bytes = c->pileup_bytes + staged;
   return rc;
+}
+
+int lcr_pileup_records(lcr_ctx* c, int64_t* items, int64_t* records) {
+  if (!c || !items || !records) return LCR_E_ARG;
+  if (c->stage < ST_PILED) { c->err = "lcr_pileup_records before lcr_pileup"; return LCR_E_STATE; }
+  *items = c->pile_items; *records = c->pile_recs;
+  return LCR_OK;
 }
 
 int lcr_pileup_stage_bytes(lcr_ctx* c, int64_t* bytes) {
@@ -500,6 +507,7 @@
   else if (k == "fuse_filter") c->dbg_fuse_filter = value != 0;
   else if (k == "spec_compact") c->dbg_spec_compact = value != 0;
   else if (k == "lean_planes") c->dbg_lean_planes = value != 0;
+  else if (k == "fold_indels") c->dbg_fold_indels = value != 0;
   else if (k == "poison_planes") c->dbg_poison_planes = value != 0;
   else if (k == "iso_hash_bits") c->dbg_iso_hash_bits = (int)std::max<int64_t>(0, std::min<int64_t>(value, 64));
   else if (k == "ends_hash_bits") c->dbg_ends_hash_bits = (int)std::max<int64_t>(0, std::min<int64_t>(value, 32));
diff --git a/longcallr_amd/csrc/lcr_ctx.h b/longcallr_amd/csrc/lcr_ctx.h
--- a/longcallr_amd/csrc/lcr_ctx.h
+++ b/longcallr_amd/csrc/lcr_ctx.h
@@ -79,7 +79,8 @@
   DevBuf blk_first_read, read_scan, cig_compact, cig_off_new, cig_new_off32;
   uint64_t cig0 = 0;
   uint32_t n_ops = 0;
-  int64_t n_items = 0;
+  int64_t pile_items = 0, pile_recs = 0;
+  int dbg_fold_indels = 1;
 
   bool planes_dense = false;
   bool planes_tallied = false;
diff --git a/longcallr_amd/csrc/lcr_dev.h b/longcallr_amd/csrc/lcr_dev.h
--- a/longcallr_amd/csrc/lcr_dev.h
+++ b/longcallr_amd/csrc/lcr_dev.h
@@ -64,10 +64,33 @@
   int32_t dbg;
 };
 
+static_assert(LCR_TILE <= 256, "a record keeps its tile column and its length - 1 in 8 bits each");
 #define REC_OFF_MASK 0xFFFFFFFFFFull
 #define REC_KIND_D 0xFFFFFFFFFFull
 #define REC_KIND_I 0xFFFFFFFFFEull
 #define REC_KIND_N 0xFFFFFFFFFDull
+#define REC_HI_COL_SHIFT 8
+#define REC_HI_LEN_SHIFT 16
+#define REC_HI_F_INS (1u << 24)
+#define REC_HI_F_DEL (1u << 25)
+#define REC_HI_STRAND_SHIFT 28
+#define REC_HI_TS_SHIFT 29
+#define REC_F_INS ((unsigned long long)REC_HI_F_INS << 32)
+#define REC_F_DEL ((unsigned long long)REC_HI_F_DEL << 32)
+#ifdef __HIPCC__
+__device__ __forceinline__ unsigned long long rec_off(unsigned long long rec) { return rec & REC_OFF_MASK; }
+__device__ __forceinline__ int rec_col(unsigned long long rec) { return (int)((uint32_t)(rec >> 40) & 255u); }
+__device__ __forceinline__ int rec_len(unsigned long long rec) { return (int)((uint32_t)(rec >> 48) & 255u) + 1; }
+__device__ __forceinline__ int rec_strand(unsigned long long rec) { return (int)((uint32_t)(rec >> 60) & 1u); }
+__device__ __forceinline__ int rec_tscls(unsigned long long rec) { return (int)((uint32_t)(rec >> 61) & 3u); }
+__device__ __forceinline__ bool rec_f_ins(unsigned long long rec) { return (rec & REC_F_INS) != 0; }
+__device__ __forceinline__ bool rec_f_del(unsigned long long rec) { return (rec & REC_F_DEL) != 0; }
+__device__ __forceinline__ bool rec_is_m(unsigned long long rec) { return rec_off(rec) < REC_KIND_N; }
+__device__ __forceinline__ int rec_kind(unsigned long long rec) {
+  const unsigned long long off = rec_off(rec);
+  return off == REC_KIND_D ? 2 : off == REC_KIND_I ? 3 : off == REC_KIND_N ? 4 : 1;
+}
+#endif
 
 struct Survivor {
   int64_t gcol;
@@ -175,6 +198,7 @@
 int launch_k0_opb();
 void launch_k0_block_reads(const ReadBin* rbin, int32_t nr, uint64_t cig0, int32_t opb, int32_t n_blocks, int32_t* blk_first_read, hipStream_t s);
 void launch_k0_ops(const BatchView& b, const ReadBin* rb, const int32_t* blk_first_read, uint64_t cig0, uint32_t n_ops, int ont, int D,
+                   int fold ,
                    int32_t n_tiles, int32_t* tile_fill, int32_t* tile_nchunks, int32_t* tile_ndiff, K0Ctl* ctl, unsigned int* acct ,
                    unsigned int pool_sub , unsigned long long* recs, unsigned int desc_sub, uint32_t* desc_tile, void* desc_val ,
                    void* read_scan , hipStream_t s);
diff --git a/longcallr_amd/csrc/lcr_pileup.hip b/longcallr_amd/csrc/lcr_pileup.hip
--- a/longcallr_amd/csrc/lcr_pileup.hip
+++ b/longcallr_amd/csrc/lcr_pileup.hip
@@ -47,7 +47,7 @@
   HIPCHK(c, lcr_fill_async(fill, 0, L.words * 4, c->stream));
   if (!gated) { HIPCHK(c, c->phase.gate_stream(c->stream)); gated = true; }
   Timer t(c, LCR_K_SPANS);
-  launch_k0_ops(c->bv, c->read_bin.as<ReadBin>(), c->blk_first_read.as<int32_t>(), c->cig0, c->n_ops, c->dp.ont, c->dp.dist_to_end, c->n_tiles,
+  launch_k0_ops(c->bv, c->read_bin.as<ReadBin>(), c->blk_first_read.as<int32_t>(), c->cig0, c->n_ops, c->dp.ont, c->dp.dist_to_end, c->dbg_fold_indels, c->n_tiles,
                 fill, fill + L.nch, fill + L.ndiff, reinterpret_cast<K0Ctl*>(fill + L.ctl), (unsigned int*)(fill + L.acct), P.pool_sub, c->k0_items.as<unsigned long long>(),
                 P.desc_sub, c->desc_tile.as<uint32_t>(), c->desc_val.p, c->read_scan.p, c->stream);
   return LCR_OK;
@@ -176,7 +176,7 @@
       P.desc_cap64 = std::max<size_t>(P.desc_cap64 * 2, ((size_t)ctl.desc_top + 1024) * P.n_shards);
     }
   }
-  c->n_items = (int32_t)ctl.n_recs;
+  c->pile_items = (int64_t)ctl.n_items; c->pile_recs = (int64_t)ctl.n_recs;
   const int64_t plane_cols = lean ? 0 : c->n_cols - (int64_t)ctl.empty_cols;
   c->pileup_bytes = c->n_bases + 8 * (int64_t)(int32_t)ctl.n_items + c->n_cols + 4 * LCR_NPLANES * plane_cols;
   c->stage_bytes = c->n_bases + 4 * c->n_cigar + 37 * (int64_t)c->bv.n_reads + c->n_cols + 4 * LCR_NPLANES * plane_cols;
```

Measured after the change: 7.043 billion (median of 6 runs). +2.9%, better.
